# zengjianping/openpose

Measured on AMD Instinct MI355X. Metric: frames/sec whole-node, BODY_25 -1x368 @1280x720, 1/2/4/8 GPU + CPU ref, higher is better.
Workload: dtype fp16

## Files before the change

include/opk.h:

```cpp
#ifndef OPK_H
#define OPK_H

#include <stddef.h>
#include <stdint.h>

#ifdef __cplusplus
extern "C" {
#endif

#define OPK_OK 0
#define OPK_ERR_ARG 1
#define OPK_ERR_HIP 2
#define OPK_ERR_STATE 3
#define OPK_ERR_UNSUPPORTED 4

#define OPK_BODY_25 0
#define OPK_COCO_18 1
#define OPK_MPI_15 2
#define OPK_MPI_15_4 3
#define OPK_BODY_19 4
#define OPK_BODY_19_X2 5
#define OPK_BODY_19N 6
#define OPK_BODY_25E 7
#define OPK_CAR_12 8
#define OPK_BODY_25D 9
#define OPK_BODY_23 10
#define OPK_CAR_22 11
#define OPK_BODY_19E 12
#define OPK_BODY_25B 13
#define OPK_BODY_135 14

#define OPK_CONNECT_CPU 0
#define OPK_CONNECT_GPU 1

const char* opk_last_error(void);
int opk_version(void);

typedef struct opk_ctx opk_ctx;
int opk_ctx_create(int device, void* hip_stream ,
                   opk_ctx** out);
int opk_ctx_create_private_stream(int device, opk_ctx** out);
int opk_ctx_destroy(opk_ctx* ctx);
int opk_ctx_stream(opk_ctx* ctx, void** hip_stream);
int opk_sync(opk_ctx* ctx);
int opk_malloc(opk_ctx* ctx, void** dev, size_t bytes);
int opk_free(opk_ctx* ctx, void* dev);
int opk_memset(opk_ctx* ctx, void* dev, int value, size_t bytes);
int opk_memcpy_h2d(opk_ctx* ctx, void* dev_dst, const void* host_src, size_t bytes);
int opk_memcpy_d2h(opk_ctx* ctx, void* host_dst, const void* dev_src, size_t bytes);
#define OPK_F32 0
#define OPK_F64 1
#define OPK_U8 2
int opk_convert(opk_ctx* ctx, void* dst_dev, int dst_type, const void* src_dev, int src_type,
                size_t count);

int opk_resize_and_merge(opk_ctx* ctx, float* target_dev, const float* const* sources_dev,
                         int num_sources, const int target_size[4], const int* source_sizes,
                         const float* scale_ratios);

int opk_nms(opk_ctx* ctx, float* target_dev, int* kernel_scratch_dev, const float* source_dev,
            float threshold, const int target_size[4], const int source_size[4],
            float offset_x, float offset_y);

#define OPK_MAPS_CPU 0
#define OPK_MAPS_CUDA 1
int opk_resize_and_merge_semantics(opk_ctx* ctx, float* target_dev, const float* const* sources_dev,
                                   int num_sources, const int target_size[4],
                                   const int* source_sizes, const float* scale_ratios,
                                   int semantics);
int opk_nms_semantics(opk_ctx* ctx, float* target_dev, int* kernel_scratch_dev,
                      const float* source_dev, float threshold, const int target_size[4],
                      const int source_size[4], float offset_x, float offset_y, int semantics);

int opk_paf_scores(opk_ctx* ctx, float* pair_scores_dev, const float* heat_dev,
                   const float* peaks_dev, int num_frames, int pose_model, int heat_channels,
                   int heat_h, int heat_w, int max_peaks, float inter_threshold,
                   float inter_min_above_threshold, float default_nms_threshold);

int opk_connect_body_parts(opk_ctx* ctx, float* keypoints_host, float* scores_host,
                           int max_people, int* num_people, const float* heat_dev,
                           const float* peaks_dev, int pose_model, int heat_channels, int heat_h,
                           int heat_w, int max_peaks, float inter_min_above_threshold,
                           float inter_threshold, int min_subset_cnt, float min_subset_score,
                           float default_nms_threshold, float scale_factor,
                           int maximize_positives);

int opk_assemble_people(float* keypoints_host, float* scores_host, int max_people,
                        int* num_people, const float* pair_scores_host,
                        const float* peaks_host, int pose_model, int max_peaks,
                        int min_subset_cnt, float min_subset_score, float scale_factor,
                        int maximize_positives);

int opk_assemble_people_semantics(float* keypoints_host, float* scores_host, int max_people,
                                  int* num_people, const float* pair_scores_host,
                                  const float* peaks_host, int pose_model, int max_peaks,
                                  int min_subset_cnt, float min_subset_score, float scale_factor,
                                  int maximize_positives, int semantics);
int opk_connect_body_parts_semantics(opk_ctx* ctx, float* keypoints_host, float* scores_host,
                                     int max_people, int* num_people, const float* heat_dev,
                                     const float* peaks_dev, int pose_model, int heat_channels,
                                     int heat_h, int heat_w, int max_peaks,
                                     float inter_min_above_threshold, float inter_threshold,
                                     int min_subset_cnt, float min_subset_score,
                                     float default_nms_threshold, float scale_factor,
                                     int maximize_positives, int semantics);

int opk_scale_keypoints(float* keypoints_host, int people, int parts, int scale_mode,
                        double scale_input_to_output, double scale_net_to_output, int producer_w,
                        int producer_h);
int opk_keep_top_n_people(const float* keypoints_host, int people, int parts,
                          const float* scores_host, int max_people, float* out_keypoints_host,
                          int* out_index_host, int* out_people);

typedef struct opk_json_keypoints {
    const char* name;
    const float* data;
    int ndims, people, parts, dims;
} opk_json_keypoints;
int opk_people_json(const opk_json_keypoints* arrays, int n_arrays, const float* candidates_host,
                    const int* candidate_counts_host, int n_parts, int human_readable,
                    char* out_host, size_t capacity, size_t* len);
int opk_save_people_json(const char* path, const opk_json_keypoints* arrays, int n_arrays,
                         const float* candidates_host, const int* candidate_counts_host,
                         int n_parts, int human_readable);

int opk_pose_model_info(int pose_model, int* parts, int* bkg, int* npairs, int* heat_channels,
                        int* pairs, int* map_idx);
int opk_pose_default_thresholds(int pose_model, int maximize_positives, float* nms_threshold,
                                float* inter_threshold);

int opk_scale_and_size(int in_w, int in_h, int net_w, int net_h, float dynamic_behavior,
                       int scale_number, double scale_gap, double* scales, int* net_sizes);
int opk_cvmat_to_input(opk_ctx* ctx, float* input_dev, const uint8_t* frames_dev, int n, int width,
                       int height, size_t step, double scale, int net_w, int net_h, int normalize);

int opk_dev_set(const char* key, int value, int reset);

typedef struct opk_net opk_net;
int opk_net_create(opk_ctx* ctx, const char* prototxt, const char* caffemodel, opk_net** out);
int opk_net_load_caffemodel(opk_net* net, const char* caffemodel, int* convs_loaded);
int opk_caffemodel_blob(const char* caffemodel, const char* layer, int index, float* data,
                        size_t capacity, int64_t* shape, int* ndim);
int opk_net_destroy(opk_net* net);
int opk_net_num_convs(opk_net* net);
int opk_net_conv_info(opk_net* net, int index, char* name, int* cin, int* cout, int* kernel,
                      int* act);
int opk_net_set_conv(opk_net* net, const char* name, const float* weights_host,
                     const float* bias_host, const float* slope_host);
int opk_net_forward(opk_net* net, const float* input_dev, int n, int h, int w);
int opk_net_flops_per_frame(opk_net* net, int h, int w, double* flops);
#define OPK_PRECISION_FP16 0
#define OPK_PRECISION_SPLIT 1
int opk_net_set_precision(opk_net* net, int precision);
int opk_net_set_precision_schedule(opk_net* net, const int* precisions, int count);
int opk_net_conv_precision(opk_net* net, int index);
int opk_net_set_small_batch(opk_net* net, int enable);
int opk_net_small_batch(opk_net* net);
int opk_net_conv_plan(opk_net* net, int index, int n, int h, int w, int cus,
                      int* bm, int* bn, int* workgroups, int* small );
int opk_net_conv_kernels(opk_net* net, int index, int n, int h, int w, int cus,
                         char* buf, size_t size, size_t* needed);
int opk_net_set_timing(opk_net* net, int enable);
int opk_net_read_timing(opk_net* net, int* forwards, double* total_ms);
int opk_net_output(opk_net* net, float** output_dev, int shape[4]);
int opk_net_blob(opk_net* net, const char* name, int frame0, int nframes, float* host_out,
                 int shape[4]);
int opk_net_blob_planes(opk_net* net, const char* name, int frame0, int nframes, float* hi_host,
                        float* lo_host, int shape[4], int* has_lo);
int opk_net_launch_log(opk_net* net, char* buf, size_t size, size_t* needed);

typedef struct opk_pose opk_pose;
#define OPK_PROP_NMS_THRESHOLD 0
#define OPK_PROP_INTER_MIN_ABOVE_THRESHOLD 1
#define OPK_PROP_INTER_THRESHOLD 2
#define OPK_PROP_MIN_SUBSET_CNT 3
#define OPK_PROP_MIN_SUBSET_SCORE 4
int opk_pose_create(opk_ctx* ctx, opk_net* net ,
                    int maximize_positives, opk_pose** out);
int opk_pose_create_model(opk_ctx* ctx, opk_net* net, int pose_model, int maximize_positives,
                          int semantics, opk_pose** out);
int opk_pose_destroy(opk_pose* pose);
int opk_pose_set_property(opk_pose* pose, int property, double value);
int opk_pose_set_map_semantics(opk_pose* pose, int semantics);
int opk_pose_set_upsampling_ratio(opk_pose* pose, float ratio);
int opk_pose_forward(opk_pose* pose, const float* frames_dev, int n, int net_h, int net_w,
                     int producer_w, int producer_h);
int opk_pose_forward_net_output(opk_pose* pose, const float* net_output_dev, int n, int out_h,
                                int out_w, int net_h, int net_w, int producer_w, int producer_h);
int opk_pose_submit(opk_pose* pose, const float* frames_dev, int n, int net_h, int net_w,
                    int producer_w, int producer_h);
int opk_pose_submit_net_output(opk_pose* pose, const float* net_output_dev, int n, int out_h,
                               int out_w, int net_h, int net_w, int producer_w, int producer_h);
int opk_pose_collect(opk_pose* pose, int* frames);
int opk_pose_submit_multi(opk_pose* pose, const float* const* frames_dev, const int* net_hw,
                          int num_scales, int n, int producer_w, int producer_h);
int opk_pose_forward_multi(opk_pose* pose, const float* const* frames_dev, const int* net_hw,
                           int num_scales, int n, int producer_w, int producer_h);
int opk_pose_set_input(opk_pose* pose, int net_w, int net_h, float dynamic_behavior,
                       int scale_number, double scale_gap);
int opk_pose_submit_frames(opk_pose* pose, const uint8_t* frames_dev, int n, int width,
                           int height, size_t step);
int opk_pose_forward_frames(opk_pose* pose, const uint8_t* frames_dev, int n, int width,
                            int height, size_t step);
int opk_pose_net_input(opk_pose* pose, int scale, const float** input_dev, int* net_w,
                       int* net_h);
int opk_pose_pending(opk_pose* pose);
int opk_pose_set_overlay(opk_pose* pose, const float* overlay_dev);
int opk_pose_num_people(opk_pose* pose, int frame);
int opk_pose_keypoints(opk_pose* pose, int frame, float* keypoints_host, float* scores_host,
                       int max_people);
int opk_pose_set_timing(opk_pose* pose, int enable);
int opk_pose_read_timing(opk_pose* pose, int* batches, double* total_ms);
int opk_pose_read_collect_times(opk_pose* pose, int* collects, double* wait_ms, double* assembly_ms,
                                int* workers);
int opk_pose_records(opk_pose* pose, float* records_host, size_t capacity, size_t* used);
int opk_pose_heatmaps(opk_pose* pose, float** heat_dev, int shape[4]);
int opk_pose_heatmap_size(opk_pose* pose, int shape[4]);
int opk_pose_peaks(opk_pose* pose, float** peaks_dev, int shape[4]);
float opk_pose_scale_net_to_output(opk_pose* pose);
#define OPK_HEATMAP_PARTS 1
#define OPK_HEATMAP_BACKGROUND 2
#define OPK_HEATMAP_PAFS 4
int opk_pose_heatmaps_copy(opk_pose* pose, int types, int scale_mode, float* dst_dev,
                           int shape[4]);
int opk_pose_heatmaps_copy_range(opk_pose* pose, int types, int scale_mode, int frame0, int nframes,
                                 void* dst_dev, int dst_type, int shape[4]);
int opk_pose_candidates(opk_pose* pose, int frame, float* candidates_host, int* counts_host);


int opk_face_detect(int pose_model, const float* keypoints_host, int people, int parts,
                    float* rects_host);
int opk_hand_detect(int pose_model, const float* keypoints_host, int people, int parts,
                    float* rects_host);

typedef struct opk_extractor opk_extractor;
#define OPK_EXTRACT_FACE 0
#define OPK_EXTRACT_HAND 1
int opk_extractor_create(opk_ctx* ctx, opk_net* net, int kind, int net_w, int net_h,
                         opk_extractor** out);
int opk_extractor_destroy(opk_extractor* ex);
int opk_extractor_set_scales(opk_extractor* ex, int number, float range);
int opk_extractor_set_max_batch(opk_extractor* ex, int max_batch);
int opk_extractor_parts(opk_extractor* ex);
int opk_extractor_set_heatmaps(opk_extractor* ex, int scale_mode);
int opk_extractor_heatmaps(opk_extractor* ex, const float** heatmaps_dev, int shape[5]);
int opk_extractor_forward(opk_extractor* ex, const uint8_t* frames_dev, int nframes, int width,
                          int height, size_t step, const float* rects_host,
                          const int* frame_of_host, int people, float* keypoints_host);
int opk_extractor_crop_count(opk_extractor* ex);
int opk_extractor_crop(opk_extractor* ex, int i, double* matrix_host, const float** input_dev);

int opk_pose_attach_extractor(opk_pose* pose, opk_extractor* ex);
int opk_pose_detach_extractor(opk_pose* pose, int kind);
int opk_pose_part_rectangles(opk_pose* pose, int kind, int frame, float* rects_host);
int opk_pose_part_keypoints(opk_pose* pose, int kind, int frame, float* keypoints_host,
                            int max_people);
int opk_pose_read_part_times(opk_pose* pose, int kind, int* batches, int* crops, double* host_ms,
                             double* wait_ms);

int opk_probe_peaks(opk_ctx* ctx, double* mfma_random_tflops, double* mfma_zero_tflops,
                    double* hbm_read_gbs);

int opk_render_pose_keypoints(opk_ctx* ctx, float* frame_dev, int pose_model, int people,
                              unsigned width, unsigned height, const float* pose_dev,
                              float render_threshold, int googly_eyes, int blend_original,
                              float alpha);
int opk_render_face_keypoints(opk_ctx* ctx, float* frame_dev, unsigned width, unsigned height,
                              const float* face_dev, int people, float render_threshold,
                              float alpha);
int opk_render_hand_keypoints(opk_ctx* ctx, float* frame_dev, unsigned width, unsigned height,
                              const float* hands_dev, int hands, float render_threshold,
                              float alpha);
int opk_render_pose_heat_map(opk_ctx* ctx, float* frame_dev, unsigned width, unsigned height,
                             const float* heat_dev, int heat_w, int heat_h,
                             float scale_to_keep_ratio, unsigned part, float alpha);
int opk_render_pose_heat_maps(opk_ctx* ctx, float* frame_dev, int pose_model, unsigned width,
                              unsigned height, const float* heat_dev, int heat_w, int heat_h,
                              float scale_to_keep_ratio, float alpha);
int opk_render_pose_paf(opk_ctx* ctx, float* frame_dev, int pose_model, unsigned width,
                        unsigned height, const float* heat_dev, int heat_w, int heat_h,
                        float scale_to_keep_ratio, int part, float alpha);
int opk_render_pose_pafs(opk_ctx* ctx, float* frame_dev, int pose_model, unsigned width,
                         unsigned height, const float* heat_dev, int heat_w, int heat_h,
                         float scale_to_keep_ratio, float alpha);
int opk_render_pose_distance(opk_ctx* ctx, float* frame_dev, unsigned width, unsigned height,
                             const float* heat_dev, int heat_w, int heat_h,
                             float scale_to_keep_ratio, unsigned part, float alpha);

#define OPK_CAST_CPU 0
#define OPK_CAST_CUDA 1
int opk_cvmat_to_output(opk_ctx* ctx, float* output_dev, const uint8_t* frames_dev, int n,
                        int width, int height, size_t step, double scale, int out_w, int out_h);
int opk_output_to_cvmat(opk_ctx* ctx, uint8_t* dst_dev, size_t dst_step, const float* output_dev,
                        int n, int w, int h, int cast);

#define OPK_LAYER_POSE 0
#define OPK_LAYER_FACE 1
#define OPK_LAYER_HAND 2
typedef struct opk_render_layer {
    int kind;
    int pose_model;
    const float* keypoints_dev;
// ... 53 lines not shown
```

openpose_amd/_lib.py:

```python
import ctypes
import os

_HERE = os.path.dirname(os.path.abspath(__file__))
LIB_PATH = os.path.join(_HERE, "libopk_hip.so")
if os.environ.get("OPK_LIB_PATH"):
    LIB_PATH = os.environ["OPK_LIB_PATH"]

_c = ctypes
_p = _c.c_void_p
_i = _c.c_int
_f = _c.c_float
_d = _c.c_double
_ip = _c.POINTER(_c.c_int)
_fp = _c.POINTER(_c.c_float)

_SIGS = {
    "opk_last_error": (_c.c_char_p, []),
    "opk_version": (_i, []),
    "opk_dev_set": (_i, [_c.c_char_p, _i, _i]),
    "opk_ctx_create": (_i, [_i, _p, _c.POINTER(_p)]),
    "opk_ctx_create_private_stream": (_i, [_i, _c.POINTER(_p)]),
    "opk_ctx_destroy": (_i, [_p]),
    "opk_ctx_stream": (_i, [_p, _c.POINTER(_p)]),
    "opk_sync": (_i, [_p]),
    "opk_malloc": (_i, [_p, _c.POINTER(_p), _c.c_size_t]),
    "opk_free": (_i, [_p, _p]),
    "opk_memset": (_i, [_p, _p, _i, _c.c_size_t]),
    "opk_convert": (_i, [_p, _p, _i, _p, _i, _c.c_size_t]),
    "opk_memcpy_h2d": (_i, [_p, _p, _p, _c.c_size_t]),
    "opk_memcpy_d2h": (_i, [_p, _p, _p, _c.c_size_t]),
    "opk_probe_peaks": (_i, [_p, _c.POINTER(_d), _c.POINTER(_d), _c.POINTER(_d)]),
    "opk_render_pose_keypoints": (_i, [_p, _p, _i, _i, _c.c_uint, _c.c_uint, _p, _f, _i, _i, _f]),
    "opk_render_face_keypoints": (_i, [_p, _p, _c.c_uint, _c.c_uint, _p, _i, _f, _f]),
    "opk_render_hand_keypoints": (_i, [_p, _p, _c.c_uint, _c.c_uint, _p, _i, _f, _f]),
    "opk_render_pose_heat_map": (_i, [_p, _p, _c.c_uint, _c.c_uint, _p, _i, _i, _f, _c.c_uint, _f]),
    "opk_render_pose_heat_maps": (_i, [_p, _p, _i, _c.c_uint, _c.c_uint, _p, _i, _i, _f, _f]),
    "opk_render_pose_paf": (_i, [_p, _p, _i, _c.c_uint, _c.c_uint, _p, _i, _i, _f, _i, _f]),
    "opk_render_pose_pafs": (_i, [_p, _p, _i, _c.c_uint, _c.c_uint, _p, _i, _i, _f, _f]),
    "opk_render_pose_distance": (_i, [_p, _p, _c.c_uint, _c.c_uint, _p, _i, _i, _f, _c.c_uint, _f]),
    "opk_resize_and_merge": (_i, [_p, _p, _c.POINTER(_p), _i, _ip, _ip, _fp]),
    "opk_nms": (_i, [_p, _p, _p, _p, _f, _ip, _ip, _f, _f]),
    "opk_nms_semantics": (_i, [_p, _p, _p, _p, _f, _ip, _ip, _f, _f, _i]),
    "opk_pose_set_map_semantics": (_i, [_p, _i]),
    "opk_resize_and_merge_semantics": (_i, [_p, _p, _c.POINTER(_p), _i, _ip, _ip, _fp, _i]),
    "opk_paf_scores": (_i, [_p, _p, _p, _p, _i, _i, _i, _i, _i, _i, _f, _f, _f]),
    "opk_connect_body_parts": (_i, [_p, _p, _p, _i, _ip, _p, _p, _i, _i, _i, _i, _i, _f, _f, _i,
                                    _f, _f, _f, _i]),
    "opk_assemble_people": (_i, [_p, _p, _i, _ip, _p, _p, _i, _i, _i, _f, _f, _i]),
    "opk_connect_body_parts_semantics": (_i, [_p, _p, _p, _i, _ip, _p, _p, _i, _i, _i, _i, _i, _f,
                                              _f, _i, _f, _f, _f, _i, _i]),
    "opk_assemble_people_semantics": (_i, [_p, _p, _i, _ip, _p, _p, _i, _i, _i, _f, _f, _i, _i]),
    "opk_pose_model_info": (_i, [_i, _ip, _ip, _ip, _ip, _p, _p]),
    "opk_pose_default_thresholds": (_i, [_i, _i, _fp, _fp]),
    "opk_net_create": (_i, [_p, _c.c_char_p, _c.c_char_p, _c.POINTER(_p)]),
    "opk_net_destroy": (_i, [_p]),
    "opk_net_num_convs": (_i, [_p]),
    "opk_net_conv_info": (_i, [_p, _i, _c.c_char_p, _ip, _ip, _ip, _ip]),
    "opk_net_set_conv": (_i, [_p, _c.c_char_p, _p, _p, _p]),
    "opk_net_forward": (_i, [_p, _p, _i, _i, _i]),
    "opk_net_flops_per_frame": (_i, [_p, _i, _i, _c.POINTER(_d)]),
    "opk_net_output": (_i, [_p, _c.POINTER(_p), _ip]),
    "opk_net_blob": (_i, [_p, _c.c_char_p, _i, _i, _p, _ip]),
    "opk_net_launch_log": (_i, [_p, _c.c_char_p, _c.c_size_t, _c.POINTER(_c.c_size_t)]),
    "opk_pose_create": (_i, [_p, _p, _i, _c.POINTER(_p)]),
    "opk_pose_create_model": (_i, [_p, _p, _i, _i, _i, _c.POINTER(_p)]),
    "opk_pose_destroy": (_i, [_p]),
    "opk_pose_set_property": (_i, [_p, _i, _d]),
    "opk_pose_forward": (_i, [_p, _p, _i, _i, _i, _i, _i]),
    "opk_pose_forward_net_output": (_i, [_p, _p, _i, _i, _i, _i, _i, _i, _i]),
    "opk_pose_set_upsampling_ratio": (_i, [_p, _f]),
    "opk_pose_heatmap_size": (_i, [_p, _ip]),
    "opk_pose_set_overlay": (_i, [_p, _p]),
    "opk_pose_submit": (_i, [_p, _p, _i, _i, _i, _i, _i]),
    "opk_pose_submit_net_output": (_i, [_p, _p, _i, _i, _i, _i, _i, _i, _i]),
    "opk_pose_collect": (_i, [_p, _ip]),
    "opk_pose_submit_multi": (_i, [_p, _c.POINTER(_p), _ip, _i, _i, _i, _i]),
    "opk_pose_forward_multi": (_i, [_p, _c.POINTER(_p), _ip, _i, _i, _i, _i]),
    "opk_pose_pending": (_i, [_p]),
    "opk_pose_num_people": (_i, [_p, _i]),
    "opk_pose_keypoints": (_i, [_p, _i, _p, _p, _i]),
    "opk_pose_set_timing": (_i, [_p, _i]),
    "opk_pose_read_timing": (_i, [_p, _ip, _c.POINTER(_d)]),
    "opk_pose_read_collect_times": (_i, [_p, _ip, _c.POINTER(_d), _c.POINTER(_d), _ip]),
    "opk_net_set_precision": (_i, [_p, _i]),
    "opk_net_set_precision_schedule": (_i, [_p, _ip, _i]),
    "opk_net_conv_precision": (_i, [_p, _i]),
    "opk_net_blob_planes": (_i, [_p, _c.c_char_p, _i, _i, _p, _p, _ip, _ip]),
    "opk_net_set_small_batch": (_i, [_p, _i]),
    "opk_net_small_batch": (_i, [_p]),
    "opk_net_conv_plan": (_i, [_p, _i, _i, _i, _i, _i, _ip, _ip, _ip, _ip]),
    "opk_net_conv_kernels": (_i, [_p, _i, _i, _i, _i, _i, _c.c_char_p, _c.c_size_t, _c.POINTER(_c.c_size_t)]),
    "opk_pose_records":(_i, [_p, _p, _c.c_size_t, _c.POINTER(_c.c_size_t)]),
    "opk_pose_heatmaps": (_i, [_p, _c.POINTER(_p), _ip]),
    "opk_pose_peaks": (_i, [_p, _c.POINTER(_p), _ip]),
    "opk_pose_scale_net_to_output": (_f, [_p]),
    "opk_net_load_caffemodel": (_i, [_p, _c.c_char_p, _ip]),
    "opk_caffemodel_blob": (_i, [_c.c_char_p, _c.c_char_p, _i, _p, _c.c_size_t, _p, _ip]),
    "opk_net_set_timing": (_i, [_p, _i]),
    "opk_net_read_timing": (_i, [_p, _ip, _c.POINTER(_d)]),
    "opk_pose_heatmaps_copy": (_i, [_p, _i, _i, _p, _ip]),
    "opk_pose_heatmaps_copy_range": (_i, [_p, _i, _i, _i, _i, _p, _i, _ip]),
    "opk_pose_candidates": (_i, [_p, _i, _p, _ip]),
    "opk_scale_keypoints": (_i, [_p, _i, _i, _i, _d, _d, _i, _i]),
    "opk_keep_top_n_people": (_i, [_p, _i, _i, _p, _i, _p, _p, _ip]),
    "opk_people_json": (_i, [_p, _i, _p, _p, _i, _i, _p, ctypes.c_size_t, _p]),
    "opk_save_people_json": (_i, [ctypes.c_char_p, _p, _i, _p, _p, _i, _i]),
    "opk_face_detect": (_i, [_i, _p, _i, _i, _p]),
    "opk_hand_detect": (_i, [_i, _p, _i, _i, _p]),
    "opk_extractor_create": (_i, [_p, _p, _i, _i, _i, _c.POINTER(_p)]),
    "opk_extractor_destroy": (_i, [_p]),
    "opk_extractor_set_scales": (_i, [_p, _i, _f]),
    "opk_extractor_set_max_batch": (_i, [_p, _i]),
    "opk_extractor_set_heatmaps": (_i, [_p, _i]),
    "opk_extractor_heatmaps": (_i, [_p, _p, _ip]),
    "opk_extractor_parts": (_i, [_p]),
    "opk_extractor_forward": (_i, [_p, _p, _i, _i, _i, _c.c_size_t, _p, _p, _i, _p]),
    "opk_extractor_crop_count": (_i, [_p]),
    "opk_extractor_crop": (_i, [_p, _i, _p, _c.POINTER(_p)]),
    "opk_pose_attach_extractor": (_i, [_p, _p]),
    "opk_pose_detach_extractor": (_i, [_p, _i]),
    "opk_pose_part_rectangles": (_i, [_p, _i, _i, _p]),
    "opk_pose_part_keypoints": (_i, [_p, _i, _i, _p, _i]),
    "opk_pose_read_part_times": (_i, [_p, _i, _ip, _ip, _c.POINTER(_d), _c.POINTER(_d)]),
    "opk_pose_render_frames_parts": (_i, [_p, _p, _c.c_size_t, _i, _i, _p, _i, _i, _i, _c.c_size_t,
                                          _d, _f, _f, _i, _i, _i, _f, _f, _f, _f]),
    "opk_scale_and_size": (_i, [_i, _i, _i, _i, _f, _i, _d, _c.POINTER(_d), _ip]),
    "opk_cvmat_to_input": (_i, [_p, _p, _p, _i, _i, _i, _c.c_size_t, _d, _i, _i, _i]),
    "opk_pose_set_input": (_i, [_p, _i, _i, _f, _i, _d]),
    "opk_pose_submit_frames": (_i, [_p, _p, _i, _i, _i, _c.c_size_t]),
    "opk_pose_forward_frames": (_i, [_p, _p, _i, _i, _i, _c.c_size_t]),
    "opk_pose_net_input": (_i, [_p, _i, _c.POINTER(_p), _ip, _ip]),
    "opk_cvmat_to_output": (_i, [_p, _p, _p, _i, _i, _i, _c.c_size_t, _d, _i, _i]),
    "opk_output_to_cvmat": (_i, [_p, _p, _c.c_size_t, _p, _i, _i, _i, _i]),
    "opk_render_frames": (_i, [_p, _p, _c.c_size_t, _i, _i, _p, _i, _i, _i, _c.c_size_t, _d, _p, _i,
                               _i, _i]),
    "opk_pose_render_frames": (_i, [_p, _p, _c.c_size_t, _i, _i, _p, _i, _i, _i, _c.c_size_t, _d,
                                    _f, _f, _i, _i, _i]),
    "opk_render_frames_heat": (_i, [_p, _p, _c.c_size_t, _i, _i, _p, _i, _i, _i, _c.c_size_t, _d, _p,
                                    _i, _i, _i, _p]),
    "opk_render_element": (_i, [_i, _i, _ip, _ip]),
    "opk_pose_render_frames_element": (_i, [_p, _p, _c.c_size_t, _i, _i, _p, _i, _i, _i,
                                            _c.c_size_t, _d, _i, _f, _f, _f, _i, _i, _i]),
}


class RenderHeatStruct(ctypes.Structure):
    _fields_ = [("kind", _i), ("pose_model", _i), ("channel", _i), ("heat_dev", _p),
                ("channels", _i), ("heat_w", _i), ("heat_h", _i), ("scale_to_keep_ratio", _f),
                ("alpha", _f)]


class RenderLayerStruct(ctypes.Structure):
    _fields_ = [("kind", _i), ("pose_model", _i), ("keypoints_dev", _p), ("counts_host", _ip),
                ("render_threshold", _f), ("alpha", _f), ("googly_eyes", _i)]


_LIB = None


class OpkError(RuntimeError):
    pass


def load():
    global _LIB
    if _LIB is None:
        if not os.path.exists(LIB_PATH):
            raise OpkError("libopk_hip.so not built (run `python -m openpose_amd.build`); the "
                           "product has no fallback path")
        L = ctypes.CDLL(LIB_PATH)
        for name, (res, args) in _SIGS.items():
            fn = getattr(L, name, None)
            if fn is None:
                continue
            fn.restype = res
            fn.argtypes = args
        _LIB = L
    return _LIB


def exported_symbols():
    return list(_SIGS)


def check(rc):
    if rc != 0:
        raise OpkError("opk error %d: %s" % (rc, load().opk_last_error().decode()))
    return rc


def int4(v):
    return (ctypes.c_int * 4)(*[int(x) for x in v])
```

openpose_amd/api.py:

```python
import atexit
import ctypes
import weakref

import numpy as np
import torch

from . import _lib
from ._lib import OpkError, check, int4
from .pose_tables import (BODY_25, CONNECT_CPU, CONNECT_GPU, CONNECT_INTER_MIN_ABOVE_THRESHOLD,
                          CONNECT_INTER_THRESHOLD,
                          CONNECT_MIN_SUBSET_CNT, CONNECT_MIN_SUBSET_SCORE, NMS_THRESHOLD)

MAPS_CPU, MAPS_CUDA = 0, 1
PRECISION_FP16, PRECISION_SPLIT = 0, 1
CAST_CPU, CAST_CUDA = 0, 1
LAYER_POSE, LAYER_FACE, LAYER_HAND = 0, 1, 2
_LAYER_THRESHOLD = {LAYER_POSE: 0.05, LAYER_FACE: 0.4, LAYER_HAND: 0.2}


class RenderLayer:

    def __init__(self, kind, keypoints, counts, threshold=None, alpha=0.6, pose_model=BODY_25,
                 googly_eyes=False):
        self.kind, self.keypoints, self.counts = kind, keypoints, list(counts)
        self.threshold = _LAYER_THRESHOLD[kind] if threshold is None else threshold
        self.alpha, self.pose_model, self.googly_eyes = alpha, pose_model, googly_eyes


HEAT_NONE, HEAT_PART, HEAT_PARTS, HEAT_PAF, HEAT_PAFS, HEAT_DISTANCE = 0, 1, 2, 3, 4, 5


class RenderHeat:

    def __init__(self, kind, heat, scale, channel=0, alpha=0.7, pose_model=BODY_25):
        self.kind, self.heat, self.scale, self.channel = kind, heat, scale, channel
        self.alpha, self.pose_model = alpha, pose_model


def render_element(pose_model, element):
    kind, channel = ctypes.c_int(0), ctypes.c_int(0)
    check(_lib.load().opk_render_element(pose_model, element, ctypes.byref(kind),
                                         ctypes.byref(channel)))
    return kind.value, channel.value


def _row_bytes(t, n, h, w):
    assert t.dtype == torch.uint8 and t.is_contiguous() and t.shape[0] == n and t.shape[1] == h
    step = t.shape[2] * 3 if t.dim() == 4 else t.shape[2]
    assert (t.dim() == 3 or t.shape[3] == 3) and step >= w * 3
    return step


def _ptr(t):
    if t is None:
        return None
    assert t.is_cuda and t.is_contiguous(), "device tensors must be contiguous CUDA tensors"
    return ctypes.c_void_p(t.data_ptr())


_LIVE = {"pose": weakref.WeakSet(), "extractor": weakref.WeakSet(), "net": weakref.WeakSet(),
         "ctx": weakref.WeakSet()}


@atexit.register
def _close_live():
    for kind in ("pose", "extractor", "net", "ctx"):
        for obj in list(_LIVE[kind]):
            try:
                obj.close()
            except Exception:
                pass


class dev_switches:

    def __init__(self, **kv):
        self.kv = kv

    def __enter__(self):
        L = _lib.load()
        for k, v in self.kv.items():
            check(L.opk_dev_set(k.encode(), int(v), 0))
        return self

    def __exit__(self, *exc):
        L = _lib.load()
        for k in self.kv:
            L.opk_dev_set(k.encode(), 0, 1)
        return False


class Context:

    def __init__(self, device=0, stream=None):
        self.L = _lib.load()
        self.device = device
        torch.cuda.set_device(device)
        s = stream if stream is not None else torch.cuda.current_stream(device)
        self.torch_stream = s
        h = ctypes.c_void_p()
        check(self.L.opk_ctx_create(device, ctypes.c_void_p(s.cuda_stream), ctypes.byref(h)))
        self.h = h
        _LIVE["ctx"].add(self)

    def close(self):
        if self.h:
            self.L.opk_ctx_destroy(self.h)
            self.h = None

    def __del__(self):
        try:
            self.close()
        except Exception:
            pass

    def sync(self):
        check(self.L.opk_sync(self.h))

    @classmethod
    def host_only(cls):
        self = cls.__new__(cls)
        self.L = _lib.load()
        self.device = -1
        self.torch_stream = None
        h = ctypes.c_void_p()
        check(self.L.opk_ctx_create(-1, None, ctypes.byref(h)))
        self.h = h
        _LIVE["ctx"].add(self)
        return self

    def convert(self, dst, src):
        kinds = {torch.float32: 0, torch.float64: 1}
        assert dst.numel() == src.numel() and dst.dtype in kinds and src.dtype in kinds
        assert dst.is_contiguous() and src.is_contiguous()
        check(self.L.opk_convert(self.h, _ptr(dst), kinds[dst.dtype], _ptr(src), kinds[src.dtype],
                                 src.numel()))

    def resize_and_merge(self, target, sources, semantics=MAPS_CPU, scale_ratios=None):
        n = len(sources)
        ptrs = (ctypes.c_void_p * n)(*[s.data_ptr() for s in sources])
        sizes = (ctypes.c_int * (4 * n))(*[int(v) for s in sources for v in s.shape])
        ratios = None if scale_ratios is None else (ctypes.c_float * n)(*[float(r) for r in scale_ratios])
        check(self.L.opk_resize_and_merge_semantics(self.h, _ptr(target), ptrs, n,
                                                    int4(target.shape), sizes, ratios, semantics))

    def cvmat_to_input(self, net_input, frames, scale, normalize=1):
        n, h, w, c = frames.shape
        assert c == 3 and frames.dtype == torch.uint8
        assert net_input.shape[0] == n and net_input.shape[1] == 3
        check(self.L.opk_cvmat_to_input(self.h, _ptr(net_input), _ptr(frames), n, w, h, w * 3,
                                        float(scale), net_input.shape[3], net_input.shape[2],
                                        normalize))

    def nms(self, peaks, heat, threshold=NMS_THRESHOLD, offset=(0.0, 0.0), semantics=MAPS_CPU):
        check(self.L.opk_nms_semantics(self.h, _ptr(peaks), None, _ptr(heat), threshold,
                                       int4(peaks.shape), int4(heat.shape), offset[0], offset[1],
                                       semantics))

    def probe_peaks(self):
        r, z, h = ctypes.c_double(), ctypes.c_double(), ctypes.c_double()
        check(self.L.opk_probe_peaks(self.h, ctypes.byref(r), ctypes.byref(z), ctypes.byref(h)))
        return {"mfma_fp16_random_tflops": round(r.value, 1), "mfma_fp16_zero_tflops": round(z.value, 1),
                "hbm_read_gbs": round(h.value, 1)}

    def render_pose_keypoints(self, frame, pose, pose_model=BODY_25, threshold=0.05,
                              googly_eyes=False, blend_original=True, alpha=0.6):
        h, w = frame.shape[:2]
        people = 0 if pose is None else pose.shape[0]
        check(self.L.opk_render_pose_keypoints(self.h, _ptr(frame), pose_model, people, w, h,
                                               None if pose is None else _ptr(pose), threshold,
                                               int(googly_eyes), int(blend_original), alpha))

    def render_face_keypoints(self, frame, face, threshold=0.4, alpha=0.6):
        h, w = frame.shape[:2]
        check(self.L.opk_render_face_keypoints(self.h, _ptr(frame), w, h, _ptr(face), face.shape[0],
                                               threshold, alpha))

    def render_hand_keypoints(self, frame, hands, threshold=0.2, alpha=0.6):
        h, w = frame.shape[:2]
        check(self.L.opk_render_hand_keypoints(self.h, _ptr(frame), w, h, _ptr(hands),
                                               hands.shape[0], threshold, alpha))

    def render_heat_map(self, frame, heat, scale, part, alpha=0.7, distance=False):
        h, w = frame.shape[:2]
        fn = self.L.opk_render_pose_distance if distance else self.L.opk_render_pose_heat_map
        check(fn(self.h, _ptr(frame), w, h, _ptr(heat), heat.shape[-1], heat.shape[-2], scale,
                 part, alpha))

    def render_heat_maps(self, frame, heat, scale, pose_model=BODY_25, alpha=0.7):
        h, w = frame.shape[:2]
        check(self.L.opk_render_pose_heat_maps(self.h, _ptr(frame), pose_model, w, h, _ptr(heat),
                                               heat.shape[-1], heat.shape[-2], scale, alpha))

    def render_pafs(self, frame, heat, scale, part=None, pose_model=BODY_25, alpha=0.7):
        h, w = frame.shape[:2]
        if part is None:
            check(self.L.opk_render_pose_pafs(self.h, _ptr(frame), pose_model, w, h, _ptr(heat),
                                              heat.shape[-1], heat.shape[-2], scale, alpha))
        else:
            check(self.L.opk_render_pose_paf(self.h, _ptr(frame), pose_model, w, h, _ptr(heat),
                                             heat.shape[-1], heat.shape[-2], scale, part, alpha))

    def cvmat_to_output(self, frames, scale=1.0, out_size=None):
        n, h, w, c = frames.shape
        assert c == 3 and frames.dtype == torch.uint8
        ow, oh = out_size if out_size is not None else (w, h)
        out = torch.empty((n, max(oh, 0), max(ow, 0), 3), dtype=torch.float32, device=frames.device)
        check(self.L.opk_cvmat_to_output(self.h, _ptr(out), _ptr(frames), n, w, h, w * 3,
                                         float(scale), ow, oh))
        return out

    def output_to_cvmat(self, output, cast=CAST_CPU, out=None):
        n, h, w, c = output.shape
        assert c == 3 and output.dtype == torch.float32
        if out is None:
            out = torch.empty((n, h, w, 3), dtype=torch.uint8, device=output.device)
        check(self.L.opk_output_to_cvmat(self.h, _ptr(out), _row_bytes(out, n, h, w), _ptr(output),
                                         n, w, h, cast))
        return out

    def render_frames(self, frames, layers, scale=1.0, out_size=None, blend_original=True,
                      cast=CAST_CPU, out=None, heat=None):
        n, h, w, c = frames.shape
        assert c == 3 and frames.dtype == torch.uint8
        ow, oh = out_size if out_size is not None else (w, h)
        if out is None:
            out = torch.empty((n, max(oh, 0), max(ow, 0), 3), dtype=torch.uint8,
                              device=frames.device)
        arr = (_lib.RenderLayerStruct * max(len(layers), 1))()
        keep = []
        for s, l in zip(arr, layers):
            assert len(l.counts) == n, "one count per frame"
            counts = (ctypes.c_int * max(n, 1))(*[int(v) for v in l.counts])
            keep.append(counts)
            parts = {LAYER_FACE: 70, LAYER_HAND: 21}.get(l.kind)
            if parts is None and l.kind == LAYER_POSE and 0 <= l.pose_model <= 14:
                parts = pose_model_info(l.pose_model)["parts"]
            if l.keypoints is None:
                assert sum(l.counts) == 0, "keypoints missing"
            elif parts is not None:
                assert l.keypoints.dtype == torch.float32
                assert tuple(l.keypoints.shape) == (sum(l.counts), parts, 3), "keypoints shape"
            s.kind, s.pose_model = l.kind, l.pose_model
            s.keypoints_dev = None if l.keypoints is None else _ptr(l.keypoints)
            s.counts_host = counts
            s.render_threshold, s.alpha, s.googly_eyes = l.threshold, l.alpha, int(l.googly_eyes)
        if heat is None:
            check(self.L.opk_render_frames(self.h, _ptr(out), _row_bytes(out, n, oh, ow), ow, oh,
                                           _ptr(frames), n, w, h, w * 3, float(scale), arr,
                                           len(layers), int(blend_original), cast))
            return out
        hs = _lib.RenderHeatStruct()
        hs.kind, hs.pose_model, hs.channel = heat.kind, heat.pose_model, heat.channel
        if heat.heat is not None:
            assert heat.heat.dtype == torch.float32 and heat.heat.dim() == 4
            assert heat.heat.shape[0] == n, "one heat stack per frame"
            hs.heat_dev = _ptr(heat.heat)
            hs.channels, hs.heat_h, hs.heat_w = heat.heat.shape[1:]
        hs.scale_to_keep_ratio, hs.alpha = heat.scale, heat.alpha
        check(self.L.opk_render_frames_heat(self.h, _ptr(out), _row_bytes(out, n, oh, ow), ow, oh,
                                            _ptr(frames), n, w, h, w * 3, float(scale), arr,
                                            len(layers), int(blend_original), cast,
                                            ctypes.byref(hs)))
        return out

    def paf_scores(self, scores, heat, peaks, pose_model=BODY_25, inter_th=CONNECT_INTER_THRESHOLD,
                   inter_min_above=CONNECT_INTER_MIN_ABOVE_THRESHOLD, nms_th=NMS_THRESHOLD):
        n, c, h, w = heat.shape
        check(self.L.opk_paf_scores(self.h, _ptr(scores), _ptr(heat), _ptr(peaks), n, pose_model, c,
                                    h, w, peaks.shape[2] - 1, inter_th, inter_min_above, nms_th))

    def connect_body_parts(self, heat, peaks, pose_model=BODY_25, scale=1.0, max_people=512,
                           inter_min_above=CONNECT_INTER_MIN_ABOVE_THRESHOLD,
                           inter_th=CONNECT_INTER_THRESHOLD, min_subset_cnt=CONNECT_MIN_SUBSET_CNT,
                           min_subset_score=CONNECT_MIN_SUBSET_SCORE, nms_th=NMS_THRESHOLD,
                           maximize_positives=False, semantics=CONNECT_CPU):
        c, h, w = heat.shape[-3:]
        parts = peaks.shape[-3]
        kp = np.zeros((max_people, parts, 3), np.float32)
        ks = np.zeros(max_people, np.float32)
        n = ctypes.c_int()
        check(self.L.opk_connect_body_parts_semantics(
            self.h, kp.ctypes.data_as(ctypes.c_void_p), ks.ctypes.data_as(ctypes.c_void_p),
            max_people, ctypes.byref(n), _ptr(heat), _ptr(peaks), pose_model, c, h, w,
            peaks.shape[-2] - 1, inter_min_above, inter_th, min_subset_cnt, min_subset_score,
            nms_th, scale, int(maximize_positives), semantics))
        k = min(n.value, max_people)
        return kp[:k].copy(), ks[:k].copy()


def scale_and_size(input_size, net_resolution=(-1, 368), dynamic_behavior=1.0, scale_number=1,
                   scale_gap=0.25):
    L = _lib.load()
    scales = (ctypes.c_double * scale_number)()
    sizes = (ctypes.c_int * (2 * scale_number))()
    check(L.opk_scale_and_size(input_size[0], input_size[1], net_resolution[0], net_resolution[1],
                               float(dynamic_behavior), scale_number, float(scale_gap), scales,
                               sizes))
    return list(scales), [(sizes[2 * i], sizes[2 * i + 1]) for i in range(scale_number)]


def scale_keypoints(keypoints, scale_mode, scale_input_to_output=1.0, scale_net_to_output=1.0,
                    producer_size=(1, 1)):
    kp = np.ascontiguousarray(keypoints, np.float32).copy()
    check(_lib.load().opk_scale_keypoints(kp.ctypes.data_as(ctypes.c_void_p), kp.shape[0],
# ... 29 lines not shown
        a = np.ascontiguousarray(a if a is not None else np.zeros(0), np.float32)
        keep.append(a)
        shape = a.shape if a.size else ()
        if len(shape) not in (0, 1, 3):
            shape = (None,) * 2
        dims = list(shape) + [0] * (3 - len(shape))
        arr[i] = _JsonKeypoints(name.encode(), a.ctypes.data if a.size else None, len(shape),
                                dims[0] or 0, dims[1] or 0, dims[2] or 0)
    cands = candidates or []
    counts = np.array([len(c) for c in cands], np.int32)
    flat = np.ascontiguousarray(
        np.concatenate([np.asarray(c, np.float32).reshape(-1, 3) for c in cands])
        if cands and counts.sum() else np.zeros((0, 3)), np.float32)
    keep += [counts, flat]
    return arr, keep, (flat.ctypes.data if flat.size else None,
                       counts.ctypes.data if counts.size else None, len(cands))


def people_json(keypoint_vector, candidates=None, human_readable=False):
    L = _lib.load()
    arr, keep, (cp, cc, nparts) = _json_args(keypoint_vector, candidates)
    n = ctypes.c_size_t()
    check(L.opk_people_json(arr, len(keypoint_vector), cp, cc, nparts, int(human_readable), None,
                            0, ctypes.byref(n)))
    buf = ctypes.create_string_buffer(n.value + 1)
    check(L.opk_people_json(arr, len(keypoint_vector), cp, cc, nparts, int(human_readable), buf,
                            n.value + 1, ctypes.byref(n)))
    del keep
    return buf.raw[:n.value].decode()


def save_people_json(path, keypoint_vector, candidates=None, human_readable=False):
    L = _lib.load()
    arr, keep, (cp, cc, nparts) = _json_args(keypoint_vector, candidates)
    check(L.opk_save_people_json(path.encode(), arr, len(keypoint_vector), cp, cc, nparts,
                                 int(human_readable)))
    del keep


def datum_keypoint_vector(pose_keypoints, face_keypoints=None, hand_keypoints=(None, None)):
    pk = np.asarray(pose_keypoints, np.float32)
    ids = np.full(pk.shape[0], -1, np.float32) if pk.size else None
    return [(ids, "person_id"), (pk, "pose_keypoints_2d"), (face_keypoints, "face_keypoints_2d"),
            (hand_keypoints[0], "hand_left_keypoints_2d"),
            (hand_keypoints[1], "hand_right_keypoints_2d"), (None, "pose_keypoints_3d"),
            (None, "face_keypoints_3d"), (None, "hand_left_keypoints_3d"),
            (None, "hand_right_keypoints_3d")]


def caffemodel_blob(path, layer, index):
    L = _lib.load()
    shape = (ctypes.c_int64 * 8)()
    nd = ctypes.c_int()
    check(L.opk_caffemodel_blob(path.encode(), layer.encode(), index, None, 0, shape,
                                ctypes.byref(nd)))
    dims = tuple(shape[i] for i in range(nd.value))
    out = np.empty(int(np.prod(dims)) if dims else 0, np.float32)
    check(L.opk_caffemodel_blob(path.encode(), layer.encode(), index,
                                out.ctypes.data_as(ctypes.c_void_p), out.size, shape,
                                ctypes.byref(nd)))
    return dims, out.reshape(dims)


def pose_model_info(pose_model):
    L = _lib.load()
    parts, bkg, npairs, hc = (ctypes.c_int() for _ in range(4))
    check(L.opk_pose_model_info(pose_model, ctypes.byref(parts), ctypes.byref(bkg),
                                ctypes.byref(npairs), ctypes.byref(hc), None, None))
    pairs = np.zeros(2 * npairs.value, np.int32)
    nmap = hc.value - parts.value - bkg.value
    mi = np.zeros(max(nmap, 1), np.int32)
    check(L.opk_pose_model_info(pose_model, None, None, None, None,
                                pairs.ctypes.data_as(ctypes.c_void_p),
                                mi.ctypes.data_as(ctypes.c_void_p)))
    nms, inter = ctypes.c_float(), ctypes.c_float()
    check(L.opk_pose_default_thresholds(pose_model, 0, ctypes.byref(nms), ctypes.byref(inter)))
    return dict(id=pose_model, parts=parts.value, bkg=bool(bkg.value), pairs=pairs.tolist(),
                map_idx=mi[:nmap].tolist(), heat_channels=hc.value, nms_threshold=nms.value,
                inter_threshold=inter.value)


def assemble_people(pair_scores, peaks, pose_model=BODY_25, scale=1.0, max_people=512,
                    min_subset_cnt=CONNECT_MIN_SUBSET_CNT, min_subset_score=CONNECT_MIN_SUBSET_SCORE,
                    maximize_positives=False, semantics=CONNECT_CPU):
    L = _lib.load()
    pair_scores = np.ascontiguousarray(pair_scores, np.float32)
    peaks = np.ascontiguousarray(peaks, np.float32)
    parts = peaks.shape[0]
    kp = np.zeros((max_people, parts, 3), np.float32)
    ks = np.zeros(max_people, np.float32)
    n = ctypes.c_int()
    check(L.opk_assemble_people_semantics(kp.ctypes.data_as(ctypes.c_void_p),
                                          ks.ctypes.data_as(ctypes.c_void_p), max_people,
                                          ctypes.byref(n),
                                          pair_scores.ctypes.data_as(ctypes.c_void_p),
                                          peaks.ctypes.data_as(ctypes.c_void_p), pose_model,
                                          peaks.shape[1] - 1, min_subset_cnt, min_subset_score,
                                          scale, int(maximize_positives), semantics))
    k = min(n.value, max_people)
    return kp[:k].copy(), ks[:k].copy()


class Net:

    def __init__(self, ctx, prototxt="builtin:BODY_25", caffemodel=None):
        self.ctx = ctx
        self.L = ctx.L
        h = ctypes.c_void_p()
        check(self.L.opk_net_create(ctx.h, prototxt.encode(),
                                    caffemodel.encode() if caffemodel else None, ctypes.byref(h)))
        self.h = h
        _LIVE["net"].add(self)

    def close(self):
        if self.h:
            self.L.opk_net_destroy(self.h)
            self.h = None

    def __del__(self):
        try:
            self.close()
        except Exception:
            pass

    def convs(self):
        out = []
        name = ctypes.create_string_buffer(64)
        cin, cout, k, act = ctypes.c_int(), ctypes.c_int(), ctypes.c_int(), ctypes.c_int()
        for i in range(self.L.opk_net_num_convs(self.h)):
            check(self.L.opk_net_conv_info(self.h, i, name, ctypes.byref(cin), ctypes.byref(cout),
                                           ctypes.byref(k), ctypes.byref(act)))
            out.append(dict(name=name.value.decode(), cin=cin.value, num_output=cout.value,
                            kernel_size=k.value, act=act.value))
        return out

    def set_params(self, params):
        for c in self.convs():
            w, b, s = params[c["name"]]
            w = np.ascontiguousarray(w, np.float32)
            b = np.ascontiguousarray(b, np.float32)
            sp = None
            if s is not None:
                s = np.ascontiguousarray(s, np.float32)
                sp = s.ctypes.data_as(ctypes.c_void_p)
            check(self.L.opk_net_set_conv(self.h, c["name"].encode(),
                                          w.ctypes.data_as(ctypes.c_void_p),
                                          b.ctypes.data_as(ctypes.c_void_p), sp))

    def forward(self, x):
        n, c, h, w = x.shape
        check(self.L.opk_net_forward(self.h, _ptr(x), n, h, w))
        return self.output()

    def load_caffemodel(self, path):
        n = ctypes.c_int()
        check(self.L.opk_net_load_caffemodel(self.h, path.encode(), ctypes.byref(n)))
        return n.value

    def set_precision(self, precision):
        check(self.L.opk_net_set_precision(self.h, int(precision)))

    def set_precision_schedule(self, schedule):
        convs = self.convs()
        if callable(schedule):
            sched = [schedule(dict(c, index=i)) for i, c in enumerate(convs)]
        elif isinstance(schedule, dict):
            names = {c["name"] for c in convs}
            unknown = sorted(set(schedule) - names)
            if unknown:
                raise OpkError("precision schedule: no convolution named " + ", ".join(unknown))
            cur = self.precision_schedule()
            sched = [schedule.get(c["name"], cur[i]) for i, c in enumerate(convs)]
        else:
            sched = list(schedule)
        arr = (ctypes.c_int * max(1, len(sched)))(*[int(p) for p in sched])
        check(self.L.opk_net_set_precision_schedule(self.h, arr, len(sched)))

    def precision_schedule(self):
        return [self.L.opk_net_conv_precision(self.h, i)
                for i in range(self.L.opk_net_num_convs(self.h))]

    def set_small_batch(self, on=True):
        check(self.L.opk_net_set_small_batch(self.h, int(bool(on))))

    @property
    def small_batch(self):
        return self.L.opk_net_small_batch(self.h) == 1

    def conv_plan(self, index, n, h, w, cus):
        v = [ctypes.c_int() for _ in range(4)]
        check(self.L.opk_net_conv_plan(self.h, index, n, h, w, cus, *[ctypes.byref(x) for x in v]))
        return dict(bm=v[0].value, bn=v[1].value, workgroups=v[2].value, small=v[3].value)

    def conv_kernels(self, index, n, h, w, cus):
        need = ctypes.c_size_t()
        check(self.L.opk_net_conv_kernels(self.h, index, n, h, w, cus, None, 0, ctypes.byref(need)))
        buf = ctypes.create_string_buffer(need.value)
        check(self.L.opk_net_conv_kernels(self.h, index, n, h, w, cus, buf, need.value, ctypes.byref(need)))
        return buf.value.decode().splitlines()

    def set_timing(self, on=True):
        check(self.L.opk_net_set_timing(self.h, int(on)))

    def read_timing(self):
        n, ms = ctypes.c_int(), ctypes.c_double()
        check(self.L.opk_net_read_timing(self.h, ctypes.byref(n), ctypes.byref(ms)))
        return n.value, ms.value

    def flops_per_frame(self, h, w):
        f = ctypes.c_double()
        check(self.L.opk_net_flops_per_frame(self.h, h, w, ctypes.byref(f)))
        return f.value

    def output(self):
        p = ctypes.c_void_p()
        shape = (ctypes.c_int * 4)()
        check(self.L.opk_net_output(self.h, ctypes.byref(p), shape))
        return p.value, tuple(shape)

    def output_numpy(self):
        p, shape = self.output()
        out = np.empty(shape, np.float32)
        check(self.L.opk_memcpy_d2h(self.ctx.h, out.ctypes.data_as(ctypes.c_void_p),
                                    ctypes.c_void_p(p), out.nbytes))
        return out

    def blob(self, name, frames=None):
        shape = (ctypes.c_int * 4)()
        f0, nf = frames if frames is not None else (0, self.output()[1][0])
        check(self.L.opk_net_blob(self.h, name.encode(), f0, nf, None, shape))
        out = np.empty(tuple(shape), np.float32)
        check(self.L.opk_net_blob(self.h, name.encode(), f0, nf,
                                  out.ctypes.data_as(ctypes.c_void_p), shape))
        return out

    def blob_planes(self, name, frames=None):
        shape = (ctypes.c_int * 4)()
        has = ctypes.c_int()
        f0, nf = frames if frames is not None else (0, self.output()[1][0])
        check(self.L.opk_net_blob_planes(self.h, name.encode(), f0, nf, None, None, shape,
                                         ctypes.byref(has)))
        hi = np.empty(tuple(shape), np.float32)
        lo = np.empty(tuple(shape), np.float32)
        check(self.L.opk_net_blob_planes(self.h, name.encode(), f0, nf,
                                         hi.ctypes.data_as(ctypes.c_void_p),
                                         lo.ctypes.data_as(ctypes.c_void_p), shape, ctypes.byref(has)))
        return hi, lo, bool(has.value)

    def launch_log(self):
        need = ctypes.c_size_t()
        check(self.L.opk_net_launch_log(self.h, None, 0, ctypes.byref(need)))
        buf = ctypes.create_string_buffer(need.value)
        check(self.L.opk_net_launch_log(self.h, buf, need.value, ctypes.byref(need)))
        return [tuple(line.split("\t", 1)) for line in buf.value.decode().splitlines()]


class PoseExtractor:

    def __init__(self, ctx, net=None, maximize_positives=False, pose_model=BODY_25,
                 semantics=CONNECT_CPU):
        self.ctx = ctx
        self.L = ctx.L
        h = ctypes.c_void_p()
        check(self.L.opk_pose_create_model(ctx.h, net.h if net is not None else None, pose_model,
                                           int(maximize_positives), semantics, ctypes.byref(h)))
        self.h = h
        _LIVE["pose"].add(self)
        self.net = net
        self.parts = pose_model_info(pose_model)["parts"]
        self.pose_model = pose_model
        self._attached = {}

    def close(self):
        if self.h:
            self.L.opk_pose_destroy(self.h)
            self.h = None
            self._attached = {}

    def attach(self, face=None, hands=None):
        for ex, kind in ((face, FACE), (hands, HAND)):
            if ex is None:
                continue
            if ex.kind != kind:
                raise ValueError("face wants a FACE extractor, hands a HAND extractor")
            check(self.L.opk_pose_attach_extractor(self.h, ex.h))
            self._attached[kind] = ex

    def detach(self, kind):
        check(self.L.opk_pose_detach_extractor(self.h, kind))
        self._attached.pop(kind, None)

    def _part_rectangles(self, kind, frame):
        n = max(self.num_people(frame), 0)
        out = np.zeros((n, 2 if kind == HAND else 1, 4), np.float32)
        check(self.L.opk_pose_part_rectangles(self.h, kind, frame,
                                              out.ctypes.data_as(ctypes.c_void_p)))
        return out

    def _part_keypoints(self, kind, frame):
        n = max(self.num_people(frame), 0)
        parts = self._attached[kind].parts if kind in self._attached else (21 if kind == HAND else 70)
        out = np.zeros((2 if kind == HAND else 1, n, parts, 3), np.float32)
        check(self.L.opk_pose_part_keypoints(self.h, kind, frame,
                                             out.ctypes.data_as(ctypes.c_void_p), n))
        return out

# ... 352 lines not shown
```

openpose_amd/csrc/host/api_net.cpp:

```cpp
#include <cstring>
#include <memory>
#include <string>

#include "../../../include/opk.h"
#include "net.h"
#include "caffemodel.h"
#include "extract.h"
#include "input.h"
#include "pose.h"

namespace opk {
template <class F>
static int guarded_net(F&& f)
{
    try {
        f();
        return OPK_OK;
    } catch (const Error& e) {
        set_error(e.what());
        return e.code;
    } catch (const std::exception& e) {
        set_error(e.what());
        return OPK_ERR_STATE;
    }
}
}

struct opk_ctx : opk::Context {};
struct opk_net {
    opk_ctx* ctx;
    std::unique_ptr<opk::NetHip> net;
};
struct opk_pose {
    opk_ctx* ctx;
    std::unique_ptr<opk::PoseHip> pose;
};

using opk::guarded_net;

extern "C" {

int opk_net_create(opk_ctx* ctx, const char* prototxt, const char* caffemodel, opk_net** out)
{
    return guarded_net([&] {
        OPK_CHECK_ARG(ctx && prototxt && out, "NULL argument");
        const std::string p(prototxt);
        std::vector<opk::LayerDesc> layers =
            p.rfind("builtin:", 0) == 0 ? opk::builtin_graph(p) : opk::load_prototxt(p);
        auto n = std::make_unique<opk_net>(opk_net{ctx, std::make_unique<opk::NetHip>(ctx, std::move(layers))});
        if (caffemodel && caffemodel[0]) {
            OPK_CHECK_ARG(ctx->device >= 0, "weights need a device context");
            n->net->load_caffemodel(caffemodel);
        }
        *out = n.release();
    });
}

int opk_net_destroy(opk_net* net)
{
    return guarded_net([&] {
        if (!net) return;
        if (net->ctx->device >= 0) net->ctx->bind();
        delete net;
    });
}

int opk_net_num_convs(opk_net* net)
{
    if (!net) return -1;
    return (int)net->net->convs().size();
}

int opk_net_conv_info(opk_net* net, int i, char* name, int* cin, int* cout, int* k, int* act)
{
    return guarded_net([&] {
        OPK_CHECK_ARG(net && i >= 0 && i < (int)net->net->convs().size(), "bad index");
        const auto& c = net->net->convs()[i];
        if (name) {
            std::strncpy(name, c.name.c_str(), 63);
            name[63] = 0;
        }
        if (cin) *cin = c.cin;
        if (cout) *cout = c.cout;
        if (k) *k = c.k;
        if (act) *act = c.act;
    });
}

int opk_net_set_conv(opk_net* net, const char* name, const float* w, const float* b,
                     const float* slope)
{
    return guarded_net([&] {
        OPK_CHECK_ARG(net && name, "NULL argument");
        net->net->set_conv(name, w, b, slope);
    });
}

int opk_net_forward(opk_net* net, const float* input, int n, int h, int w)
{
    return guarded_net([&] {
        OPK_CHECK_ARG(net, "NULL net");
        net->net->forward(input, n, h, w);
    });
}

int opk_net_flops_per_frame(opk_net* net, int h, int w, double* flops)
{
    return guarded_net([&] {
        OPK_CHECK_ARG(net && flops && h > 0 && w > 0, "bad argument");
        *flops = net->net->flops_per_frame(h, w);
    });
}

int opk_net_output(opk_net* net, float** out, int shape[4])
{
    return guarded_net([&] {
        OPK_CHECK_ARG(net && out && shape, "NULL argument");
        *out = net->net->output();
        shape[0] = net->net->frames();
        shape[1] = net->net->out_channels();
        shape[2] = net->net->out_h();
        shape[3] = net->net->out_w();
    });
}

int opk_net_blob(opk_net* net, const char* name, int frame0, int nframes, float* host_out,
                 int shape[4])
{
    return guarded_net([&] {
        OPK_CHECK_ARG(net && name && shape, "NULL argument");
        net->net->blob(name, frame0, nframes, host_out, shape);
    });
}

int opk_net_blob_planes(opk_net* net, const char* name, int frame0, int nframes, float* hi_host,
                        float* lo_host, int shape[4], int* has_lo)
{
    return guarded_net([&] {
        OPK_CHECK_ARG(net && name && shape && has_lo, "NULL argument");
        net->net->blob_planes(name, frame0, nframes, hi_host, lo_host, shape, has_lo);
    });
}

int opk_net_launch_log(opk_net* net, char* buf, size_t size, size_t* needed)
{
    return guarded_net([&] {
        OPK_CHECK_ARG(net && needed, "NULL argument");
        std::string text;
        for (const auto& l : net->net->launches()) text += l + "\n";
        *needed = text.size() + 1;
        if (buf && size >= *needed) std::memcpy(buf, text.c_str(), text.size() + 1);
    });
}

int opk_pose_create(opk_ctx* ctx, opk_net* net, int maxpos, opk_pose** out)
{
    return guarded_net([&] {
        OPK_CHECK_ARG(ctx && out, "NULL argument");
        *out = new opk_pose{ctx, std::make_unique<opk::PoseHip>(ctx, net ? net->net.get() : nullptr,
                                                                maxpos != 0)};
    });
}

int opk_pose_create_model(opk_ctx* ctx, opk_net* net, int pose_model, int maxpos, int semantics,
                          opk_pose** out)
{
    return guarded_net([&] {
        OPK_CHECK_ARG(ctx && out, "NULL argument");
        *out = new opk_pose{ctx, std::make_unique<opk::PoseHip>(ctx, net ? net->net.get() : nullptr,
                                                                maxpos != 0, pose_model, semantics)};
    });
}

int opk_pose_destroy(opk_pose* p)
{
    return guarded_net([&] {
        if (!p) return;
        if (p->ctx->device >= 0) p->ctx->bind();
        delete p;
    });
}

int opk_pose_set_map_semantics(opk_pose* p, int semantics)
{
    return guarded_net([&] {
        OPK_CHECK_ARG(p, "NULL pose");
        p->pose->set_map_semantics(semantics);
    });
}

int opk_pose_set_property(opk_pose* p, int prop, double v)
{
    return guarded_net([&] {
        OPK_CHECK_ARG(p, "NULL pose");
        p->pose->set_property(prop, v);
    });
}

int opk_pose_forward(opk_pose* p, const float* frames, int n, int net_h, int net_w, int pw, int ph)
{
    return guarded_net([&] {
        OPK_CHECK_ARG(p, "NULL pose");
        p->pose->forward(frames, n, net_h, net_w, pw, ph);
    });
}

int opk_pose_forward_net_output(opk_pose* p, const float* out, int n, int oh, int ow, int net_h,
                                int net_w, int pw, int ph)
{
    return guarded_net([&] {
        OPK_CHECK_ARG(p, "NULL pose");
        p->pose->forward_net_output(out, n, oh, ow, net_h, net_w, pw, ph);
    });
}

int opk_pose_submit(opk_pose* p, const float* frames, int n, int net_h, int net_w, int pw, int ph)
{
    return guarded_net([&] {
        OPK_CHECK_ARG(p, "NULL pose");
        p->pose->submit(frames, n, net_h, net_w, pw, ph);
    });
}

int opk_pose_submit_multi(opk_pose* p, const float* const* frames, const int* net_hw, int nscales,
                          int n, int pw, int ph)
{
    return guarded_net([&] {
        OPK_CHECK_ARG(p, "NULL pose");
        p->pose->submit_multi(frames, net_hw, nscales, n, pw, ph);
    });
}

int opk_pose_forward_multi(opk_pose* p, const float* const* frames, const int* net_hw,
                           int nscales, int n, int pw, int ph)
{
    return guarded_net([&] {
        OPK_CHECK_ARG(p, "NULL pose");
        OPK_CHECK_ARG(p->pose->pending() == 0, "batches in flight: collect them first");
        p->pose->submit_multi(frames, net_hw, nscales, n, pw, ph);
        p->pose->collect();
    });
}

int opk_pose_submit_net_output(opk_pose* p, const float* out, int n, int oh, int ow, int net_h,
                               int net_w, int pw, int ph)
{
    return guarded_net([&] {
        OPK_CHECK_ARG(p, "NULL pose");
        p->pose->submit_net_output(out, n, oh, ow, net_h, net_w, pw, ph);
    });
}

int opk_pose_collect(opk_pose* p, int* frames)
{
    return guarded_net([&] {
        OPK_CHECK_ARG(p, "NULL pose");
// ... 89 lines not shown
    });
}

int opk_pose_heatmaps(opk_pose* p, float** heat, int shape[4])
{
    return guarded_net([&] {
        OPK_CHECK_ARG(p && heat && shape, "NULL argument");
        *heat = p->pose->heatmaps(shape);
    });
}

int opk_pose_heatmap_size(opk_pose* p, int shape[4])
{
    return guarded_net([&] {
        OPK_CHECK_ARG(p && shape, "NULL argument");
        p->pose->heatmap_size(shape);
    });
}

int opk_pose_peaks(opk_pose* p, float** peaks, int shape[4])
{
    return guarded_net([&] {
        OPK_CHECK_ARG(p && peaks && shape, "NULL argument");
        *peaks = p->pose->peaks(shape);
    });
}

int opk_net_load_caffemodel(opk_net* net, const char* caffemodel, int* loaded)
{
    return guarded_net([&] {
        OPK_CHECK_ARG(net && caffemodel, "NULL argument");
        OPK_CHECK_ARG(net->ctx->device >= 0, "weights need a device context");
        const int n = net->net->load_caffemodel(caffemodel);
        if (loaded) *loaded = n;
    });
}

int opk_caffemodel_blob(const char* caffemodel, const char* layer, int index, float* data,
                        size_t capacity, int64_t* shape, int* ndim)
{
    return guarded_net([&] {
        OPK_CHECK_ARG(caffemodel && layer && ndim, "NULL argument");
        const auto layers = opk::load_caffemodel(caffemodel);
        for (const auto& L : layers) {
            if (L.name != layer) continue;
            OPK_CHECK_ARG(index >= 0 && index < (int)L.blobs.size(), "no such blob");
            const auto& b = L.blobs[index];
            OPK_CHECK_ARG(b.shape.size() <= 8, "blob rank > 8");
            *ndim = (int)b.shape.size();
            if (shape) for (size_t i = 0; i < b.shape.size(); ++i) shape[i] = b.shape[i];
            if (data) {
                OPK_CHECK_ARG(capacity >= b.data.size(), "capacity too small");
                std::memcpy(data, b.data.data(), b.data.size() * sizeof(float));
            }
            return;
        }
        throw opk::Error(1, std::string("layer ") + layer + " has no blobs in " + caffemodel);
    });
}

int opk_net_set_precision(opk_net* net, int precision)
{
    return guarded_net([&] {
        OPK_CHECK_ARG(net, "NULL net");
        net->net->set_precision(precision);
    });
}

int opk_net_set_precision_schedule(opk_net* net, const int* precisions, int count)
{
    return guarded_net([&] {
        OPK_CHECK_ARG(net, "NULL net");
        net->net->set_precision_schedule(precisions, count);
    });
}

int opk_net_conv_precision(opk_net* net, int index)
{
    if (!net) return -1;
    return net->net->conv_precision(index);
}

int opk_net_set_small_batch(opk_net* net, int enable)
{
    return guarded_net([&] {
        OPK_CHECK_ARG(net, "NULL net");
        OPK_CHECK_ARG(enable == 0 || enable == 1, "small batch: 0 or 1");
        net->net->set_small_batch(enable == 1);
    });
}

int opk_net_small_batch(opk_net* net)
{
    if (!net) return -1;
    return net->net->small_batch() ? 1 : 0;
}

int opk_net_conv_plan(opk_net* net, int index, int n, int h, int w, int cus, int* bm, int* bn,
                      int* workgroups, int* small)
{
    return guarded_net([&] {
        OPK_CHECK_ARG(net, "NULL net");
        net->net->conv_plan(index, n, h, w, cus, bm, bn, workgroups, small);
    });
}

int opk_net_conv_kernels(opk_net* net, int index, int n, int h, int w, int cus, char* buf, size_t size,
                         size_t* needed)
{
    return guarded_net([&] {
        OPK_CHECK_ARG(net && needed, "NULL argument");
        std::string text;
        for (const auto& k : net->net->conv_kernels(index, n, h, w, cus)) text += k + "\n";
        *needed = text.size() + 1;
        if (buf && size >= *needed) std::memcpy(buf, text.c_str(), text.size() + 1);
    });
}

int opk_net_set_timing(opk_net* net, int enable)
{
    return guarded_net([&] {
        OPK_CHECK_ARG(net, "NULL net");
        net->net->set_timing(enable != 0);
    });
}

int opk_net_read_timing(opk_net* net, int* forwards, double* total_ms)
{
    return guarded_net([&] {
        OPK_CHECK_ARG(net, "NULL net");
        net->net->read_timing(forwards, total_ms);
    });
}

int opk_scale_and_size(int in_w, int in_h, int net_w, int net_h, float dynamic_behavior,
                       int scale_number, double scale_gap, double* scales, int* net_sizes)
{
    return guarded_net([&] {
        OPK_CHECK_ARG(scales && net_sizes, "NULL output");
        opk::scale_and_size(in_w, in_h, net_w, net_h, dynamic_behavior, scale_number, scale_gap,
                            scales, net_sizes);
    });
}

int opk_cvmat_to_input(opk_ctx* ctx, float* input_dev, const uint8_t* frames_dev, int n, int width,
                       int height, size_t step, double scale, int net_w, int net_h, int normalize)
{
    return guarded_net([&] {
        OPK_CHECK_ARG(ctx, "NULL context");
        OPK_CHECK_ARG(normalize == 0 || normalize == 1,
                      "normalize: 0 (none) or 1 (VGG); DenseNet (2) is not supported");
        opk::cvmat_to_input(ctx, input_dev, frames_dev, n, width, height, step, scale, net_w, net_h,
                            normalize);
    });
}

int opk_pose_set_input(opk_pose* p, int net_w, int net_h, float dynamic_behavior, int scale_number,
                       double scale_gap)
{
    return guarded_net([&] {
        OPK_CHECK_ARG(p, "NULL pose");
        p->pose->set_input(net_w, net_h, dynamic_behavior, scale_number, scale_gap);
    });
}

int opk_pose_submit_frames(opk_pose* p, const uint8_t* frames, int n, int width, int height,
                           size_t step)
{
    return guarded_net([&] {
        OPK_CHECK_ARG(p, "NULL pose");
        p->pose->submit_frames(frames, n, width, height, step);
    });
}

int opk_pose_forward_frames(opk_pose* p, const uint8_t* frames, int n, int width, int height,
                            size_t step)
{
    return guarded_net([&] {
        OPK_CHECK_ARG(p, "NULL pose");
        p->pose->forward_frames(frames, n, width, height, step);
    });
}

int opk_pose_render_frames(opk_pose* p, uint8_t* dst, size_t dst_step, int out_w, int out_h,
                           const uint8_t* frames, int n, int width, int height, size_t step,
                           double scale, float threshold, float alpha, int googly_eyes,
                           int blend_original, int cast)
{
    return guarded_net([&] {
        OPK_CHECK_ARG(p, "NULL pose");
        std::vector<int> counts;
        opk_render_layer layer{};
        const opk::PoseHip& pose = *p->pose;
        if (pose.frames() == 0) throw opk::Error(OPK_ERR_STATE, "no collected batch to render");
        if (n != pose.frames())
            throw opk::Error(OPK_ERR_STATE, "the collected batch has " +
                                                std::to_string(pose.frames()) + " frames, not " +
                                                std::to_string(n));
        const int parts = opk::pose_model(pose.model()).parts;
        std::vector<float> kp;
        for (int f = 0; f < n; ++f) {
            const int people = pose.num_people(f);
            counts.push_back(people);
            const auto& k = pose.keypoints(f);
            kp.insert(kp.end(), k.begin(), k.begin() + (size_t)people * parts * 3);
        }
        const float s = (float)scale;
        if (s != 1.f)
            for (size_t i = 0; i < kp.size(); i += 3) {
                kp[i] *= s;
                kp[i + 1] *= s;
            }
        layer.kind = OPK_LAYER_POSE;
        layer.pose_model = pose.model();
        layer.counts_host = counts.data();
        layer.render_threshold = threshold;
        layer.alpha = alpha;
        layer.googly_eyes = googly_eyes;
        opk::render_frames(p->ctx, dst, dst_step, out_w, out_h, frames, n, width, height, step,
                           scale, &layer, 1, blend_original, cast, kp.data(), kp.size());
    });
}

int opk_pose_render_frames_element(opk_pose* p, uint8_t* dst, size_t dst_step, int out_w,
                                   int out_h, const uint8_t* frames, int n, int width, int height,
                                   size_t step, double scale, int element, float threshold,
                                   float alpha_keypoint, float alpha_heatmap, int googly_eyes,
                                   int blend_original, int cast)
{
    if (element == 0)
        return opk_pose_render_frames(p, dst, dst_step, out_w, out_h, frames, n, width, height,
                                      step, scale, threshold, alpha_keypoint, googly_eyes,
                                      blend_original, cast);
    return guarded_net([&] {
        OPK_CHECK_ARG(p, "NULL pose");
        const opk::PoseHip& pose = *p->pose;
        opk_render_heat heat{};
        heat.pose_model = pose.model();
        opk::render_element(pose.model(), element, &heat.kind, &heat.channel);
        if (pose.frames() == 0) throw opk::Error(OPK_ERR_STATE, "no collected batch to render");
        if (n != pose.frames())
            throw opk::Error(OPK_ERR_STATE, "the collected batch has " +
                                                std::to_string(pose.frames()) + " frames, not " +
                                                std::to_string(n));
        const opk::HeatMap& lazy = pose.lazy_heat();
        heat.scale_to_keep_ratio = pose.scale_net_to_output() * (float)scale;
        heat.alpha = blend_original ? alpha_heatmap : 1.f;
        opk::render_frames(p->ctx, dst, dst_step, out_w, out_h, frames, n, width, height, step,
                           scale, nullptr, 0, 1, cast, nullptr, 0, &heat, &lazy);
    });
}

int opk_pose_net_input(opk_pose* p, int scale, const float** input_dev, int* net_w, int* net_h)
{
    return guarded_net([&] {
        OPK_CHECK_ARG(p && input_dev, "NULL argument");
        *input_dev = p->pose->net_input(scale, net_w, net_h);
    });
}

int opk_pose_heatmaps_copy(opk_pose* p, int types, int scale_mode, float* dst_dev, int shape[4])
{
    return guarded_net([&] {
        OPK_CHECK_ARG(p && shape, "NULL argument");
        p->pose->heatmaps_copy(types, scale_mode, dst_dev, shape);
    });
}

int opk_pose_heatmaps_copy_range(opk_pose* p, int types, int scale_mode, int frame0, int nframes,
                                 void* dst_dev, int dst_type, int shape[4])
{
    return guarded_net([&] {
        OPK_CHECK_ARG(p && shape, "NULL argument");
        p->pose->heatmaps_copy_range(types, scale_mode, frame0, nframes, dst_dev, dst_type, shape);
    });
}

int opk_pose_candidates(opk_pose* p, int frame, float* candidates_host, int* counts_host)
{
    return guarded_net([&] {
        OPK_CHECK_ARG(p, "NULL pose");
        p->pose->candidates(frame, candidates_host, counts_host);
    });
}

float opk_pose_scale_net_to_output(opk_pose* p) { return p ? p->pose->scale_net_to_output() : 0.f; }

}

struct opk_extractor {
    opk_ctx* ctx;
    std::unique_ptr<opk::KeypointExtractor> ex;
};

extern "C" {

int opk_face_detect(int pose_model, const float* keypoints, int people, int parts, float* rects)
{
    return guarded_net([&] {
        OPK_CHECK_ARG(people == 0 || rects, "NULL rectangles");
        opk::detect_faces(pose_model, keypoints, people, parts, reinterpret_cast<opk::Rect*>(rects));
    });
}

int opk_hand_detect(int pose_model, const float* keypoints, int people, int parts, float* rects)
{
// ... 212 lines not shown
```

openpose_amd/csrc/host/input.cpp:

```cpp
#include "input.h"

#include <cmath>
#include <cstring>
#include <vector>

#include "../common.h"
#include "../kernels/kernels.h"
#include "context.h"

namespace opk {

namespace {
constexpr int kInterBits = 5, kInterTab = 1 << kInterBits;
constexpr int kAbBits = 10, kAbScale = 1 << kAbBits;
constexpr int kCoefScale = 1 << 15;

int round_half_even(double v) { return (int)std::lrint(v); }
int round_half_even(float v) { return (int)std::lrintf(v); }

int positive_round(float v) { return (int)(v + 0.5f); }
int positive_round(double v) { return (int)(v + 0.5f); }
}

void scale_and_size(int in_w, int in_h, int net_w, int net_h, float dyn, int scale_number,
                    double scale_gap, double* scales, int* sizes)
{
    OPK_CHECK_ARG(in_w > 0 && in_h > 0, "Wrong input element (empty cvInputData).");
    OPK_CHECK_ARG(scale_number >= 1, "scale_number must be >= 1");
    if (net_w <= 0 || net_h <= 0) {
        OPK_CHECK_ARG(net_w > 0 || net_h > 0,
                      "Only 1 of the dimensions of net input resolution can be <= 0.");
        if (dyn > 0) {
            if (net_w <= 0)
                net_w = 16 * positive_round(1 / 16.f * std::min(net_h * dyn * 16.f / 9.f,
                                                                 net_h * in_w / (float)in_h));
            else
                net_h = 16 * positive_round(1 / 16.f * std::min(net_w * dyn * 9.f / 16.f,
                                                                 net_w * in_h / (float)in_w));
        } else {
            if (net_w <= 0)
                net_w = 16 * positive_round(1 / 16.f * net_h * in_w / (float)in_h);
            else
                net_h = 16 * positive_round(1 / 16.f * net_w * in_h / (float)in_w);
        }
    }
    for (int i = 0; i < scale_number; ++i) {
        const double cur = 1. - i * scale_gap;
        OPK_CHECK_ARG(cur >= 0. && cur <= 1.,
                      "All scales must be in the range [0, 1], i.e., 0 <= 1-scale_number*scale_gap <= 1");
        const int tw = std::min(net_w, std::max(1, positive_round(net_w * cur) / 16 * 16));
        const int th = std::min(net_h, std::max(1, positive_round(net_h * cur) / 16 * 16));
        const double rw = (tw - 1) / (double)(in_w - 1), rh = (th - 1) / (double)(in_h - 1);
        scales[i] = rw < rh ? rw : rh;
        sizes[2 * i] = tw;
        sizes[2 * i + 1] = th;
    }
}

void warp_weight_table(bool cubic, short* itab )
{
    const int k = cubic ? 4 : 2;
    float t1[kInterTab * 4];
    for (int i = 0; i < kInterTab; ++i) {
        const float x = i * (1.f / kInterTab);
        float* c = t1 + i * k;
        if (cubic) {
            const float A = -0.75f;
            c[0] = ((A * (x + 1) - 5 * A) * (x + 1) + 8 * A) * (x + 1) - 4 * A;
            c[1] = ((A + 2) * x - (A + 3)) * x * x + 1;
            c[2] = ((A + 2) * (1 - x) - (A + 3)) * (1 - x) * (1 - x) + 1;
            c[3] = 1.f - c[0] - c[1] - c[2];
        } else {
            c[0] = 1.f - x;
            c[1] = x;
        }
    }
    for (int i = 0; i < kInterTab; ++i)
        for (int j = 0; j < kInterTab; ++j) {
            short* w = itab + (i * kInterTab + j) * k * k;
            int isum = 0;
            for (int a = 0; a < k; ++a)
                for (int b = 0; b < k; ++b) {
                    const float v = t1[i * k + a] * t1[j * k + b];
                    const int r = round_half_even(v * kCoefScale);
                    w[a * k + b] = (short)std::min(32767, std::max(-32768, r));
                    isum += w[a * k + b];
                }
            if (isum == kCoefScale) continue;
            const int diff = isum - kCoefScale, h = k / 2;
            int lo = h * k + h, hi = h * k + h;
            for (int a = h; a < h + 2; ++a)
                for (int b = h; b < h + 2; ++b) {
                    const int e = a * k + b;
                    if (w[e] < w[lo]) lo = e;
                    else if (w[e] > w[hi]) hi = e;
                }
            if (diff < 0) w[hi] = (short)(w[hi] - diff);
            else w[lo] = (short)(w[lo] - diff);
        }
}

void warp_axis_table(double scale, int d, bool cubic, int* tab)
{
    double D = scale * scale;
    D = D != 0 ? 1. / D : 0;
    const double m = scale * D;
    const int x0 = round_half_even(0.0 * kAbScale) + kAbScale / kInterTab / 2;
    for (int x = 0; x < d; ++x) {
        const int X = (x0 + round_half_even(m * x * kAbScale)) >> (kAbBits - kInterBits);
        tab[2 * x] = (X >> kInterBits) - (cubic ? 1 : 0);
        tab[2 * x + 1] = X & (kInterTab - 1);
    }
}

const short* Context::warp_weight_table(bool cubic)
{
    DevBuf& b = warp_weights[cubic ? 1 : 0];
    if (!b.ptr) {
        const int k = cubic ? 4 : 2;
        std::vector<short> host((size_t)(kInterTab * kInterTab + 1) * k * k);
        opk::warp_weight_table(cubic, host.data());
        const size_t bytes = (size_t)kInterTab * kInterTab * k * k * sizeof(short);
        b.get(bytes);
        OPK_HIP(hipMemcpyAsync(b.ptr, host.data(), bytes,
                               hipMemcpyHostToDevice, stream));
        OPK_HIP(hipStreamSynchronize(stream));
    }
    return static_cast<const short*>(b.ptr);
}

const Context::WarpAxes& Context::warp_axis_tables(double scale, int dw, int dh)
{
    uint64_t bits;
    std::memcpy(&bits, &scale, sizeof bits);
    const auto key = std::make_tuple(bits, dw, dh);
    auto it = warp_axes.find(key);
    if (it != warp_axes.end()) return *it->second;
    const bool cubic = scale > 1.;
    std::vector<int> host(2 * (size_t)(dw + dh));
    warp_axis_table(scale, dw, cubic, host.data());
    warp_axis_table(scale, dh, cubic, host.data() + 2 * dw);
    auto t = std::make_unique<WarpAxes>();
    int* dev = static_cast<int*>(t->buf.get(host.size() * sizeof(int)));
    OPK_HIP(hipMemcpyAsync(dev, host.data(), host.size() * sizeof(int), hipMemcpyHostToDevice,
                           stream));
    OPK_HIP(hipStreamSynchronize(stream));
    t->x = dev;
    t->y = dev + 2 * dw;
    auto& ref = *t;
    warp_axes.emplace(key, std::move(t));
    return ref;
}

void cvmat_to_input(Context* ctx, float* dst, const uint8_t* src, int n, int sw, int sh,
                    size_t step, double scale, int dw, int dh, int normalize, hipStream_t stream)
{
    OPK_CHECK_ARG(dst && src, "NULL buffer");
    OPK_CHECK_ARG(n > 0 && sw > 0 && sh > 0 && dw > 0 && dh > 0, "empty frame or net input");
    OPK_CHECK_ARG(scale > 0 && std::isfinite(scale), "scale must be positive");
    ctx->bind();
    const bool cubic = scale > 1.;
    const short* w = ctx->warp_weight_table(cubic);
    const auto& ax = ctx->warp_axis_tables(scale, dw, dh);
    launch_cvmat_to_input(dst, src, n, sh, sw, step ? step : (size_t)sw * 3, dh, dw, ax.x, ax.y, w,
                          cubic ? 4 : 2, normalize, stream ? stream : ctx->stream);
}

}
```

openpose_amd/csrc/host/input.h:

```cpp
#pragma once
#include <hip/hip_runtime.h>
#include <cstddef>
#include <cstdint>

namespace opk {

struct Context;

void scale_and_size(int in_w, int in_h, int net_w, int net_h, float dyn, int scale_number,
                    double scale_gap, double* scales, int* sizes);

void warp_weight_table(bool cubic, short* itab);
void warp_axis_table(double scale, int d, bool cubic, int* tab );

void cvmat_to_input(Context* ctx, float* dst, const uint8_t* src, int n, int sw, int sh,
                    size_t step, double scale, int dw, int dh, int normalize, hipStream_t stream = nullptr);

}
```

openpose_amd/csrc/host/net.cpp:

```cpp
#include "net.h"

#include "caffemodel.h"

#include <algorithm>
#include <cmath>
#include <cstdlib>
#include <set>

namespace opk {

namespace {
int round_up(int v, int m) { return (v + m - 1) / m * m; }
int pick_bn(int cout)
{
    if (cout <= 32) return 32;
    if (cout <= 64) return 64;
    if (cout <= 96) return 96;
    return 128;
}
}

NetHip::NetHip(Context* ctx, std::vector<LayerDesc> layers, const std::string& output_blob)
    : ctx_(ctx), output_blob_(output_blob)
{
// ... 597 lines not shown
    S.h = h;
    S.w = w;
    const std::vector<int>& lh_ = S.lh;
    const std::vector<int>& lw_ = S.lw;
    std::vector<uint16_t*>& ptr = S.base;
    ptr.assign(bufs_.size(), nullptr);
    S.base_lo.assign(bufs_.size(), nullptr);
    for (size_t i = 0; i < bufs_.size(); ++i) {
        S.mem.push_back(std::make_unique<DevBuf>());
        S.mem_lo.push_back(std::make_unique<DevBuf>());
        if ((int)i == image_buf_) continue;
        bool head_buf = false;
        for (size_t hi = 0; hi < heads_.size(); ++hi)
            head_buf = head_buf || (S.headfused[hi] && heads_[hi].buf == (int)i);
        if (head_buf) continue;
        if (S.fused1 && ((int)i == fuse1_.abuf || (int)i == fuse1_.bbuf))
            continue;
        bool pooled_away = false;
        for (size_t q = 0; q < pools_.size(); ++q)
            pooled_away = pooled_away || (S.poolfused[q] && pools_[q].in_buf == (int)i);
        if (pooled_away) continue;
        const int L = bufs_[i].level, B = border_;
        const size_t head = (size_t)B * (lw_[L] + 2 * B) + B + 64;
        const size_t pos = head + (size_t)n * (lh_[L] + 2 * B) * (lw_[L] + 2 * B) + kConvGuardTail;
        const size_t bytes = pos * bufs_[i].cs * 2;
        OPK_CHECK_ARG(pos * bufs_[i].cs < (size_t)1 << 31, "activation buffer exceeds 2^31 elements");
        uint16_t* raw = static_cast<uint16_t*>(S.mem.back()->get(bytes));
        OPK_HIP(hipMemsetAsync(raw, 0, bytes, zero_stream ? zero_stream : ctx_->stream));
        ptr[i] = raw + head * bufs_[i].cs;
        if (S.twin[i]) {
            uint16_t* rl = static_cast<uint16_t*>(S.mem_lo.back()->get(bytes));
            OPK_HIP(hipMemsetAsync(rl, 0, bytes, zero_stream ? zero_stream : ctx_->stream));
            S.base_lo[i] = rl + head * bufs_[i].cs;
        }
    }
    const size_t out_bytes = (size_t)n * out_c_ * lh_[out_level_] * lw_[out_level_] * 4;
    S.out32 = static_cast<float*>(S.out_mem.get(out_bytes));
    void* sink = sink_.get(kConv3SinkBytes);
    S.args.assign(convs_.size(), ConvArgs{});
    S.use3.assign(convs_.size(), 0);
    for (size_t ci = 0; ci < convs_.size(); ++ci) {
        const ConvPlan& c = convs_[ci];
        ConvArgs& a = S.args[ci];
        const int H = lh_[c.level], W = lw_[c.level], Wp = W + 2 * border_;
        a.in = ptr[c.in.buf];
        a.in_cs = bufs_[c.in.buf].cs;
        a.in_coff = c.in.coff;
        a.cin_pad = c.cin_pad;
        a.ntaps = c.ntaps;
        if (a.ntaps == 9)
            for (int t = 0; t < 9; ++t) a.tapoff[t] = (t / 3) * Wp + (t % 3);
        else if (a.ntaps == 1)
            a.tapoff[0] = Wp + 1;
        a.border = border_;
        a.ksteps = c.ksteps;
        const bool use3 = !c.from_image;
        S.use3[ci] = use3;
        OPK_CHECK_ARG(use3 || c.w.ptr != nullptr, c.info.name + ": weights not set");
        if (use3) {
            a.sw = S.conv[ci].sw;
            a.nstrips = S.conv[ci].nstrips;
            a.small = S.conv[ci].family == Conv3Family::conv3s;
            a.sink = sink;
            a.cus = cus;
        }
        a.w = static_cast<const uint16_t*>(use3 ? c.w3.ptr : c.w.ptr);
        a.bias = static_cast<const float*>(c.bias.ptr);
        a.slope = static_cast<const float*>(c.slope.ptr);
        a.act = c.info.act;
        a.actmax = dev_switch("EPI_MAX", 1) != 0;
        a.frames = n;
        a.H = H;
        a.W = W;
        a.M = n * H * Wp;
        a.cout = c.info.cout;
        a.ndst = (int)c.outs.size();
        for (size_t d = 0; d < c.outs.size(); ++d) {
            a.dst[d] = ptr[c.outs[d].buf];
            a.dst_cs[d] = bufs_[c.outs[d].buf].cs;
            a.dst_coff[d] = c.outs[d].coff;
            a.dst_lo[d] = S.csplit[ci] ? S.base_lo[c.outs[d].buf] : nullptr;
        }
        a.split = S.csplit[ci] ? 1 : 0;
        a.wscale = S.csplit[ci] ? c.wscale : 1.f;
        a.in_lo = S.csplit[ci] && use3 && !S.query[ci].xhi ? S.base_lo[c.in.buf] : nullptr;
        for (size_t q = 0; q < pools_.size(); ++q)
            if (S.poolfused[q] && pool_conv_[q] == (int)ci) {
                a.pool = 1;
                a.ndst = 1;
                a.dst[0] = ptr[pools_[q].out_buf];
                a.dst_lo[0] = S.csplit[ci] ? S.base_lo[pools_[q].out_buf] : nullptr;
                a.dst_cs[0] = bufs_[pools_[q].out_buf].cs;
                a.dst_coff[0] = 0;
            }
        if (c.out32_coff >= 0) {
            OPK_CHECK_ARG(c.level == out_level_, c.info.name + ": output at another resolution");
            a.out32 = S.out32;
            a.out32_c = out_c_;
            a.out32_coff = c.out32_coff;
        }
    }
    return &S;
}

void NetHip::forward(const float* input, int n, int h, int w)
{
    forward_on(input, n, h, w, ctx_->stream, true);
}

float* NetHip::select_output(int n, int h, int w, bool alternate)
{
    OPK_CHECK_ARG(n > 0 && h > 0 && w > 0, "empty input");
    ctx_->bind();
    ShapePlan& S = *shape_plan(n, h, w, ctx_->stream);
    if (alternate) {
        if (!S.out32_alt) {
            const size_t bytes = (size_t)n * out_c_ * S.lh[out_level_] * S.lw[out_level_] * 4;
            S.out32_alt = static_cast<float*>(S.out_mem_alt.get(bytes));
        }
        S.alt = !S.alt;
    }
    return S.out();
}

void NetHip::note_reader(const float* out, hipEvent_t ev)
{
    for (auto& r : readers_)
        if (r.first == out) {
            r.second = ev;
            return;
        }
    readers_.emplace_back(out, ev);
}

void NetHip::forget_reader_events(const hipEvent_t* evs, int n)
{
    for (size_t i = readers_.size(); i-- > 0;)
        for (int k = 0; k < n; ++k)
            if (readers_[i].second == evs[k]) {
                readers_.erase(readers_.begin() + (long)i);
                break;
            }
}

void NetHip::prepare(int n, int h, int w)
{
    OPK_CHECK_ARG(n > 0 && h > 0 && w > 0, "empty input");
    ctx_->bind();
    (void)shape_plan(n, h, w, ctx_->stream);
}

void NetHip::forward_on(const float* input, int n, int h, int w, hipStream_t st, bool timed)
{
    OPK_CHECK_ARG(input && n > 0 && h > 0 && w > 0, "empty input");
    OPK_CHECK_ARG(ready(), "weights not loaded for every convolution");
    ctx_->bind();
    ShapePlan& S = *shape_plan(n, h, w, st);
    cur_ = &S;
    for (const auto& r : readers_)
        if (r.first == S.out()) OPK_HIP(hipStreamWaitEvent(st, r.second, 0));
    if (timed) timer_.begin(st);
    forward_launches(S, input, n, h, w, st);
    if (timed) timer_.end(st);
}

void NetHip::blob(const std::string& name, int f0, int nf, float* host, int shape[4]) const
{
    read_planes(name, f0, nf, nullptr, nullptr, host, shape, nullptr);
}

void NetHip::blob_planes(const std::string& name, int f0, int nf, float* hi, float* lo, int shape[4],
                         int* has_lo) const
{
    read_planes(name, f0, nf, hi, lo, nullptr, shape, has_lo);
}

void NetHip::read_planes(const std::string& name, int f0, int nf, float* hi, float* lo, float* sum,
                         int shape[4], int* has_lo) const
{
    OPK_CHECK_ARG(cur_ != nullptr, "no forward yet");
    const auto it = blob_loc_.find(name);
    OPK_CHECK_ARG(it != blob_loc_.end(), "no blob named " + name);
    const BlobLoc& L = it->second;
    const ShapePlan& S = *cur_;
    OPK_CHECK_ARG(f0 >= 0 && nf > 0 && f0 + nf <= S.n, "frames out of range");
    const int H = S.lh[L.level], W = S.lw[L.level];
    if (shape) {
        shape[0] = nf; shape[1] = L.ch; shape[2] = H; shape[3] = W;
    }
    const bool twin = !L.out32 && S.base_lo[L.buf] != nullptr;
    if (has_lo) *has_lo = twin ? 1 : 0;
    if (!hi && !lo && !sum) return;
    ctx_->bind();
    OPK_HIP(hipStreamSynchronize(ctx_->stream));
    const size_t hw = (size_t)H * W;
    if (L.out32) {
        OPK_CHECK_ARG(L.level == out_level_, name + ": not at the output resolution");
        for (float* host : {hi, sum})
            for (int f = 0; f < nf && host; ++f)
                OPK_HIP(hipMemcpy(host + (size_t)f * L.ch * hw,
                                  S.out() + ((size_t)(f0 + f) * out_c_ + L.coff) * hw,
                                  (size_t)L.ch * hw * 4, hipMemcpyDeviceToHost));
        if (lo) std::fill(lo, lo + (size_t)nf * L.ch * hw, 0.f);
        return;
    }
    OPK_CHECK_ARG(S.base[L.buf] != nullptr,
                  name + ": kept on chip by a fused kernel (not materialised at this shape)");
    const int B = border_, Wp = W + 2 * B, Hp = H + 2 * B, cs = bufs_[L.buf].cs;
    const size_t frame_elems = (size_t)Hp * Wp * cs;
    std::vector<uint16_t> raw(frame_elems * nf), rlo(twin ? frame_elems * nf : 0);
    OPK_HIP(hipMemcpy(raw.data(), S.base[L.buf] + (size_t)f0 * frame_elems, raw.size() * 2,
                      hipMemcpyDeviceToHost));
    if (twin)
        OPK_HIP(hipMemcpy(rlo.data(), S.base_lo[L.buf] + (size_t)f0 * frame_elems, rlo.size() * 2,
                          hipMemcpyDeviceToHost));
    for (int f = 0; f < nf; ++f)
        for (int y = 0; y < H; ++y)
            for (int x = 0; x < W; ++x) {
                const size_t at = f * frame_elems + ((size_t)(y + B) * Wp + x + B) * cs + L.coff;
                const uint16_t* src = raw.data() + at;
                for (int c = 0; c < L.ch; ++c) {
                    const size_t o = ((size_t)f * L.ch + c) * hw + (size_t)y * W + x;
                    const float vh = (float)__builtin_bit_cast(_Float16, src[c]);
                    const float vl = twin ? (float)__builtin_bit_cast(_Float16, rlo[at + c]) : 0.f;
                    if (hi) hi[o] = vh;
                    if (lo) lo[o] = vl;
                    if (sum) sum[o] = vh + vl;
                }
            }
}

void NetHip::forward_launches(ShapePlan& S, const float* input, int n, int h, int w, hipStream_t st)
{
    const bool logging = dev_switch("LAUNCH_LOG", 0) != 0;
    if (logging) {
        log_.lines.clear();
        attach_launch_log(&log_);
    }
    struct Detach {
        bool on;
        ~Detach() { if (on) attach_launch_log(nullptr); }
    } detach{logging};
    forward_steps(S, input, n, h, w, st);
}

static void launch_conv3_frames(const ConvArgs& a, hipStream_t st)
{
    const int B = a.border > 0 ? a.border : 1;
    Conv3Query q = conv3_query(a);
    const int run = conv3_run_frames(q);
    if (run == a.frames) {
        launch_conv3(a, st);
        return;
    }
    const size_t frame_pos = (size_t)(a.H + 2 * B) * (a.W + 2 * B);
    const size_t dst_pos = a.pool ? (size_t)(a.H / 2 + 2 * B) * (a.W / 2 + 2 * B) : frame_pos;
    for (int f0 = 0; f0 < a.frames; f0 += run) {
        ConvArgs b = a;
        b.frames = std::min(run, a.frames - f0);
        q.frames = b.frames;
        const Conv3Plan pb = conv3_plan(q);
        b.sw = pb.sw;
        b.nstrips = pb.nstrips;
        b.M = b.frames * a.H * (a.W + 2 * B);
        b.in = a.in + f0 * frame_pos * a.in_cs;
        if (a.in_lo) b.in_lo = a.in_lo + f0 * frame_pos * a.in_cs;
        for (int d = 0; d < a.ndst; ++d) {
            b.dst[d] = a.dst[d] + f0 * dst_pos * a.dst_cs[d];
            if (a.dst_lo[d]) b.dst_lo[d] = a.dst_lo[d] + f0 * dst_pos * a.dst_cs[d];
        }
        if (a.out32) b.out32 = a.out32 + (size_t)f0 * a.out32_c * a.H * a.W;
        launch_conv3(b, st);
    }
}

void NetHip::forward_steps(ShapePlan& S, const float* input, int n, int h, int w, hipStream_t st)
{
    LaunchLog* log = launch_log();
    float* const out32 = S.out();
    const std::vector<uint16_t*>& ptr = S.base;
    const std::vector<int>& lh_ = S.lh;
    const std::vector<int>& lw_ = S.lw;
    size_t first = 0;
    if (S.fused1) {
        const ConvPlan& a = convs_[fuse1_.a];
        const ConvPlan& b = convs_[fuse1_.b];
        const PoolPlan& p = pools_[fuse1_.p];
        Conv1FusedArgs fa{};
        fa.img = input;
        fa.frames = n;
        fa.H = h;
        fa.W = w;
        fa.w1 = static_cast<const uint16_t*>(a.w.ptr);
        fa.b1 = static_cast<const float*>(a.bias.ptr);
        fa.s1 = static_cast<const float*>(a.slope.ptr);
        fa.act1 = a.info.act;
        fa.w2 = static_cast<const uint16_t*>(b.w3.ptr);
        fa.b2 = static_cast<const float*>(b.bias.ptr);
        fa.s2 = static_cast<const float*>(b.slope.ptr);
        fa.act2 = b.info.act;
        fa.out = ptr[p.out_buf];
        fa.out_cs = bufs_[p.out_buf].cs;
        fa.out_coff = 0;
        fa.OH = lh_[1];
        fa.OW = lw_[1];
        fa.actmax = a.slope01 && b.slope01 && dev_switch("EPI_MAX", 1) != 0;
        if (log) log->layer = a.info.name + "+" + b.info.name + "+pool";
        launch_conv1_fused(fa, std::min(cus_, std::max(1, dev_switch("GRID_CUS", cus_))), st);
        first = 3;
    }
    for (size_t si = first; si < steps_.size(); ++si) {
        const Step& s = steps_[si];
        if (s.conv) {
            const ConvPlan& c = convs_[s.idx];
            const ConvArgs& a = S.args[s.idx];
            if (c.head >= 0 && S.headfused[c.head] && heads_[c.head].step == (int)si) {
                const FuseHead& fh = heads_[c.head];
                const ConvPlan& cb = convs_[fh.b];
                const ConvArgs& b = S.args[fh.b];
                HeadArgs h{};
                h.in = a.in;
                h.in_cs = a.in_cs;
                h.in_coff = a.in_coff;
                h.cin_pad = a.cin_pad;
                h.w6 = static_cast<const uint16_t*>(c.wh.ptr);
                h.b6 = a.bias;
                h.s6 = a.slope;
                h.act6 = a.act;
                h.actmax = a.actmax && c.slope01;
                h.w7 = static_cast<const uint16_t*>(cb.wh.ptr);
                h.b7 = b.bias;
                h.n1 = c.info.cout;
                h.n2 = cb.info.cout;
                h.frames = n;
                h.H = a.H;
                h.W = a.W;
                h.ndst = b.ndst;
                for (int d = 0; d < b.ndst; ++d) {
                    h.dst[d] = b.dst[d];
                    h.dst_cs[d] = b.dst_cs[d];
                    h.dst_coff[d] = b.dst_coff[d];
                }
                h.out32 = b.out32 ? out32 : nullptr;
                h.out32_c = b.out32_c;
                h.out32_coff = b.out32_coff;
                h.cus = dev_switch("HEAD_PERSIST", 1) != 0 ? a.cus : 0;
                if (S.csplit[s.idx]) {
                    h.split = 1;
                    h.in_lo = a.in_lo;
                    for (int d = 0; d < b.ndst; ++d) h.dst_lo[d] = b.dst_lo[d];
                    h.wscale6 = a.wscale;
                    h.wscale7 = b.wscale;
                }
                if (log) log->layer = c.info.name + "+" + cb.info.name;
                launch_conv_head(h, st);
                ++si;
                continue;
            }
            if (log) log->layer = c.info.name + (a.pool ? "+pool" : "");
            if (c.from_image) {
                ConvArgs ai = a;
                if (ai.out32) ai.out32 = out32;
                launch_conv_image(ai, input, st);
            } else {
                ConvArgs a3 = a;
                a3.actmax = a.actmax && c.slope01;
                if (a3.out32) a3.out32 = out32;
                launch_conv3_frames(a3, st);
            }
        } else {
            if (S.poolfused[s.idx]) continue;
            const PoolPlan& p = pools_[s.idx];
            const int L = p.level_in;
            if (log) log->layer = "pool";
            if (S.twin[p.in_buf])
                launch_maxpool2_split(ptr[p.out_buf], S.base_lo[p.out_buf], ptr[p.in_buf],
                                      S.base_lo[p.in_buf], n, lh_[L], lw_[L], bufs_[p.in_buf].cs,
                                      lh_[L + 1], lw_[L + 1], st, border_);
            else
                launch_maxpool2(ptr[p.out_buf], ptr[p.in_buf], n, lh_[L], lw_[L],
                                bufs_[p.in_buf].cs, lh_[L + 1], lw_[L + 1], st, border_);
        }
    }
}

int NetHip::load_caffemodel(const std::string& path)
{
    const std::vector<CaffeLayer> layers = opk::load_caffemodel(path);
    std::map<std::string, const CaffeLayer*> by_name;
    for (const auto& L : layers) by_name[L.name] = &L;
    int loaded = 0;
    for (const ConvInfo& c : info_) {
        auto it = by_name.find(c.name);
        if (it == by_name.end()) continue;
        const auto& blobs = it->second->blobs;
        OPK_CHECK_ARG(blobs.size() == 2, c.name + ": expected weights and bias blobs, got " +
                                             std::to_string(blobs.size()));
        const std::vector<int64_t> wshape{c.cout, c.cin, c.k, c.k}, bshape{c.cout};
        OPK_CHECK_ARG(blob_shape_is(blobs[0], wshape), "Cannot copy param 0 weights from layer '" +
                                                           c.name + "'; shape mismatch.");
        OPK_CHECK_ARG(blob_shape_is(blobs[1], bshape), "Cannot copy param 1 weights from layer '" +
                                                           c.name + "'; shape mismatch.");
        const float* slope = nullptr;
        if (c.act == 2) {
            auto pt = by_name.find(c.act_layer);
            OPK_CHECK_ARG(pt != by_name.end() && pt->second->blobs.size() == 1 &&
                              blob_shape_is(pt->second->blobs[0], bshape),
                          c.act_layer + ": PReLU slopes missing or of the wrong shape");
            slope = pt->second->blobs[0].data.data();
        }
        set_conv(c.name, blobs[0].data.data(), blobs[1].data.data(), slope);
        ++loaded;
    }
    return loaded;
}

NetHip::~NetHip() = default;

void NetHip::set_timing(bool on)
{
    timer_.on = on;
}

void NetHip::read_timing(int* count, double* total_ms)
{
    timer_.read(count, total_ms);
}

}
```

openpose_amd/csrc/host/net.h:

```cpp
#pragma once
#include <map>
#include <memory>
#include <string>
#include <vector>

#include "../kernels/conv.h"
#include "context.h"
#include "graph.h"

namespace opk {

class NetHip {
public:
    NetHip(Context* ctx, std::vector<LayerDesc> layers, const std::string& output_blob = "net_output");

    struct ConvInfo {
        std::string name;
        int cin, cout, k, act;
        std::string act_layer;
    };
    const std::vector<ConvInfo>& convs() const { return info_; }
    void set_conv(const std::string& name, const float* w, const float* b, const float* slope);
    static constexpr int kPrecisionFp16 = 0, kPrecisionSplit = 1;
    void set_precision(int precision);
    void set_precision_schedule(const int* precisions, int count);
    int conv_precision(int index) const;
    void set_small_batch(bool on);
    bool small_batch() const { return small_batch_; }
    void conv_plan(int index, int n, int h, int w, int cus, int* bm, int* bn, int* workgroups,
                   int* small) const;
    std::vector<std::string> conv_kernels(int index, int n, int h, int w, int cus) const;
    bool ready() const;
    int load_caffemodel(const std::string& path);

    void forward(const float* input, int n, int h, int w);
    void forward_on(const float* input, int n, int h, int w, hipStream_t stream, bool timed);
    void prepare(int n, int h, int w);
    void time_begin(hipStream_t s) { timer_.begin(s); }
    void time_end(hipStream_t s) { timer_.end(s); }
    float* output() const { return cur_ ? cur_->out() : nullptr; }
    float* select_output(int n, int h, int w, bool alternate);
    std::weak_ptr<void> liveness() const { return alive_; }
    void note_reader(const float* out, hipEvent_t ev);
    void forget_reader_events(const hipEvent_t* evs, int n);
    int out_channels() const { return out_c_; }
    int out_h() const { return cur_ ? cur_->lh[out_level_] : 0; }
    int out_w() const { return cur_ ? cur_->lw[out_level_] : 0; }
    int frames() const { return cur_ ? cur_->n : 0; }
    static constexpr int kMaxShapes = 8;
    double flops_per_frame(int h, int w) const;
    int border() const { return border_; }
    ~NetHip();

    void set_timing(bool on);
    void read_timing(int* count, double* total_ms);

    void blob(const std::string& name, int f0, int nf, float* host, int shape[4]) const;
    void blob_planes(const std::string& name, int f0, int nf, float* hi, float* lo, int shape[4],
                     int* has_lo) const;
    const std::vector<std::string>& launches() const { return log_.lines; }

private:
    struct Placement { int buf; int coff; };
    struct BufSpec { int level; int cs; };
    struct ConvPlan {
        ConvInfo info;
        std::string in_blob;
        int level = 0;
        bool from_image = false;
        Placement in{};
        int cin_pad = 0, ntaps = 9, ksteps = 0, bn = 128, cout_pad = 0;
        std::vector<Placement> outs;
        int out32_coff = -1;
        DevBuf w, bias, slope;
        DevBuf w3;
        DevBuf wh;
        int head = -1;
        bool loaded = false;
        bool slope01 = true;
        float wscale = 1.f;
        int precision = kPrecisionFp16;
        std::vector<float> hw, hb, hs;
    };
    bool fused1_at(int h, int w) const;
    void read_planes(const std::string& name, int f0, int nf, float* hi, float* lo, float* sum,
                     int shape[4], int* has_lo) const;
    void pack(ConvPlan& c);
    struct PoolPlan { int in_buf, out_buf, level_in, channels; };
    struct Step { bool conv; int idx; };

    struct Dispatch {
        std::vector<int> lh, lw;
        std::vector<char> csplit;
        std::vector<char> twin;
        bool fused1 = false;
        std::vector<char> headfused;
        std::vector<char> poolfused;
        std::vector<Conv3Query> query;
        std::vector<Conv3Plan> conv;
    };
    Dispatch dispatch(int n, int h, int w, int cus) const;

    struct ShapePlan : Dispatch {
        int n = 0, h = 0, w = 0;
        std::vector<std::unique_ptr<DevBuf>> mem;
        std::vector<uint16_t*> base;
        std::vector<std::unique_ptr<DevBuf>> mem_lo;
        std::vector<uint16_t*> base_lo;
        DevBuf out_mem, out_mem_alt;
        float* out32 = nullptr;
        float* out32_alt = nullptr;
        bool alt = false;
        float* out() const { return alt ? out32_alt : out32; }
        std::vector<ConvArgs> args;
        std::vector<char> use3;
    };

    void plan(const std::vector<LayerDesc>& layers);
    void forward_launches(ShapePlan& S, const float* input, int n, int h, int w, hipStream_t st);
    void forward_steps(ShapePlan& S, const float* input, int n, int h, int w, hipStream_t st);
    ShapePlan* shape_plan(int n, int h, int w, hipStream_t zero_stream = nullptr);

    Context* ctx_;
    std::string output_blob_;
    std::vector<ConvInfo> info_;
    std::vector<ConvPlan> convs_;
    std::map<std::string, int> conv_by_name_;
    std::vector<PoolPlan> pools_;
    std::vector<Step> steps_;
    std::vector<BufSpec> bufs_;
    int out_level_ = 0, out_c_ = 0, nlevels_ = 1;
    int image_buf_ = -1;
    struct Fuse1 { int a = -1, b = -1, p = -1, abuf = -1, bbuf = -1; };
    Fuse1 fuse1_;
    struct FuseHead { int a = -1, b = -1, step = -1, buf = -1; };
    std::vector<FuseHead> heads_;
    std::vector<int> pool_conv_;
    int cus_ = 256;
    bool small_batch_ = false;
    int border_ = 1;

    struct BlobLoc { int buf = -1, coff = 0, ch = 0, level = 0; bool out32 = false; };
    std::map<std::string, BlobLoc> blob_loc_;
    LaunchLog log_;

    std::vector<std::unique_ptr<ShapePlan>> shapes_;
    ShapePlan* cur_ = nullptr;
    std::vector<std::pair<const float*, hipEvent_t>> readers_;
    std::shared_ptr<int> alive_ = std::make_shared<int>(0);
    DevBuf sink_;
    EventTimer timer_;
};

}
```

openpose_amd/csrc/host/pose.cpp:

```cpp
#include "pose.h"

#include <sched.h>

#include <algorithm>
#include <chrono>
#include <cmath>
#include <cstring>
#include <exception>
#include <string>
#include <thread>

#include "../../../include/opk.h"
#include "input.h"
#include "maps.h"

namespace opk {

double resize_scale_factor(int iw, int ih, int tw, int th)
{
    const double rw = (tw - 1) / (double)(iw - 1);
    const double rh = (th - 1) / (double)(ih - 1);
    return rw < rh ? rw : rh;
}

// ... 181 lines not shown
{
    OPK_CHECK_ARG(last_ >= 0, "no collected batch");
    OPK_CHECK_ARG(frame >= 0 && frame < n_, "bad frame");
    const PoseModelInfo& m = pose_model(model_);
    const size_t area = (size_t)(kMaxPeaks + 1) * 3;
    const float* p = static_cast<const float*>(slots_[last_].hpeaks.ptr) + (size_t)frame * m.parts * area;
    for (int part = 0; part < m.parts; ++part) {
        const float* pp = p + part * area;
        const int count = (int)std::round(pp[0]);
        if (counts) counts[part] = count;
        if (!out) continue;
        for (int c = 0; c < count; ++c) {
            float* o = out + ((size_t)part * kMaxPeaks + c) * 3;
            o[0] = pp[3 + 3 * c] * scale_net_to_output_;
            o[1] = pp[3 + 3 * c + 1] * scale_net_to_output_;
            o[2] = pp[3 + 3 * c + 2];
        }
    }
}

float* PoseHip::peaks(int shape[4]) const
{
    OPK_CHECK_ARG(last_ >= 0, "no collected batch");
    shape[0] = n_; shape[1] = pose_model(model_).parts; shape[2] = kMaxPeaks + 1; shape[3] = 3;
    return static_cast<float*>(slots_[last_].peaks.ptr);
}

void PoseHip::forward(const float* frames, int n, int net_h, int net_w, int prod_w, int prod_h)
{
    OPK_CHECK_ARG(count_ == 0, "batches in flight: collect them first");
    submit(frames, n, net_h, net_w, prod_w, prod_h);
    collect();
}

void PoseHip::forward_net_output(const float* net_out, int n, int oh, int ow, int net_h,
                                 int net_w, int prod_w, int prod_h)
{
    OPK_CHECK_ARG(count_ == 0, "batches in flight: collect them first");
    submit_net_output(net_out, n, oh, ow, net_h, net_w, prod_w, prod_h);
    collect();
}

void PoseHip::need_frames() const
{
    if (any_attached() && !cur_raw_.ptr)
        throw Error(3, "face / hand extraction needs the frames: with an extractor attached only "
                       "submit_frames / forward_frames are accepted");
}

void PoseHip::attach_extractor(KeypointExtractor* ex)
{
    OPK_CHECK_ARG(ex != nullptr, "NULL extractor");
    OPK_CHECK_ARG(ex->context() == ctx_, "the extractor and the pose extractor must share one context");
    OPK_CHECK_ARG(ex->net() != net_, "the extractor's net must not be the pose net");
    const int kind = ex->kind();
    if (kind == KeypointExtractor::kFace) detect_faces(model_, nullptr, 0, 0, nullptr);
    else detect_hands(model_, nullptr, 0, 0, nullptr);
    if (count_ != 0) throw Error(3, "batches in flight: collect them before attaching");
    if (attached(kind))
        throw Error(3, std::string("a ") + (kind == KeypointExtractor::kFace ? "face" : "hand") +
                           " extractor is already attached: detach it first");
    part_[kind] = Part{};
    part_[kind].ex = ex;
    part_[kind].alive = ex->liveness();
    part_[kind].parts = ex->parts();
    parts_valid_ = false;
}

void PoseHip::detach_extractor(int kind)
{
    OPK_CHECK_ARG(kind == KeypointExtractor::kFace || kind == KeypointExtractor::kHand,
                  "kind: face (0) or hand (1)");
    if (count_ != 0) throw Error(3, "batches in flight: collect them before detaching");
    part_[kind] = Part{};
}

const Rect* PoseHip::part_rectangles(int kind, int f) const
{
    OPK_CHECK_ARG(kind == KeypointExtractor::kFace || kind == KeypointExtractor::kHand,
                  "kind: face (0) or hand (1)");
    if (!attached(kind)) throw Error(3, "no such extractor attached");
    if (!parts_valid_) throw Error(3, "no collected batch with face / hand results");
    OPK_CHECK_ARG(f >= 0 && f < n_, "bad frame");
    return part_[kind].rects.data() + (size_t)part_first_[f] * (kind == KeypointExtractor::kHand ? 2 : 1);
}

const float* PoseHip::part_keypoints(int kind, int f, int* first, int* total, int* parts) const
{
    (void)part_rectangles(kind, f);
    *first = part_first_[f];
    *total = part_first_[n_];
    *parts = part_[kind].parts;
    return part_[kind].kp.data();
}

void PoseHip::read_part_times(int kind, int* batches, int* crops, double* host_ms, double* wait_ms)
{
    OPK_CHECK_ARG(kind == KeypointExtractor::kFace || kind == KeypointExtractor::kHand,
                  "kind: face (0) or hand (1)");
    Part& p = part_[kind];
    if (!attached(kind)) throw Error(3, "no such extractor attached");
    if (batches) *batches = p.batches;
    if (crops) *crops = p.crops;
    if (host_ms) *host_ms = p.host_ms;
    if (wait_ms) *wait_ms = p.wait_ms;
    p.batches = p.crops = 0;
    p.host_ms = p.wait_ms = 0.;
}

void PoseHip::run_parts(const Slot& sl)
{
    parts_valid_ = false;
    if (!any_attached()) return;
    if (!sl.raw.ptr) throw Error(3, "face / hand extraction needs the frames of the collected batch");
    const int n = sl.n;
    const int parts = pose_model(model_).parts;
    part_first_.assign(n + 1, 0);
    for (int f = 0; f < n; ++f) part_first_[f + 1] = part_first_[f] + people_[f];
    const int total = part_first_[n];
    std::vector<int> frame_of(total);
    for (int f = 0; f < n; ++f)
        std::fill(frame_of.begin() + part_first_[f], frame_of.begin() + part_first_[f + 1], f);
    for (int kind = 0; kind < 2; ++kind) {
        Part& p = part_[kind];
        if (!attached(kind)) continue;
        const auto t0 = std::chrono::steady_clock::now();
        const int per = kind == KeypointExtractor::kHand ? 2 : 1;
        p.rects.assign((size_t)total * per, Rect{0.f, 0.f, 0.f, 0.f});
        for (int f = 0; f < n; ++f) {
            Rect* r = p.rects.data() + (size_t)part_first_[f] * per;
            if (kind == KeypointExtractor::kFace) detect_faces(model_, kp_[f].data(), people_[f], parts, r);
            else detect_hands(model_, kp_[f].data(), people_[f], parts, r);
        }
        p.kp.assign((size_t)per * total * p.ex->parts() * 3, 0.f);
        const double rect_ms =
            std::chrono::duration<double, std::milli>(std::chrono::steady_clock::now() - t0).count();
        p.ex->extract(sl.raw.ptr, sl.raw.n, sl.raw.w, sl.raw.h, sl.raw.step, p.rects.data(),
                      frame_of.data(), total, p.kp.data(), true);
        ++p.batches;
        p.crops += p.ex->crops();
        p.host_ms += rect_ms + p.ex->last_host_ms();
        p.wait_ms += p.ex->last_wait_ms();
    }
    parts_valid_ = true;
}

void PoseHip::submit(const float* frames, int n, int net_h, int net_w, int prod_w, int prod_h)
{
    need_frames();
    OPK_CHECK_ARG(net_ != nullptr, "no network: use forward_net_output (poseNetOutput path)");
    OPK_CHECK_ARG(count_ < 2, "two batches already in flight: collect first");
    ctx_->bind();
    next_output(n, net_h, net_w, true);
    live_net()->forward(frames, n, net_h, net_w);
    const NetOutput o{live_net()->output(), live_net()->out_h(), live_net()->out_w()};
    submit_outputs(&o, 1, n, net_h, net_w, prod_w, prod_h, true);
}

hipStream_t PoseHip::post_stream(bool own_net)
{
    if (!own_net || ctx_->device < 0 || dev_switch("POST_STREAM", 1) == 0) {
        wait_post(ctx_->stream);
        return ctx_->stream;
    }
    if (!post_) {
        OPK_HIP(hipStreamCreateWithFlags(&post_, hipStreamNonBlocking));
        OPK_HIP(hipEventCreateWithFlags(&nets_done_, hipEventDisableTiming));
        for (auto& e : post_done_) OPK_HIP(hipEventCreateWithFlags(&e, hipEventDisableTiming));
        ctx_->add_side_stream(post_);
    }
    OPK_HIP(hipEventRecord(nets_done_, ctx_->stream));
    OPK_HIP(hipStreamWaitEvent(post_, nets_done_, 0));
    return post_;
}

void PoseHip::wait_post(hipStream_t s)
{
    if (post_count_ > 0) OPK_HIP(hipStreamWaitEvent(s, post_done_[(post_count_ - 1) & 1], 0));
}

void PoseHip::next_output(int n, int h, int w, bool alternate)
{
    const bool alt = alternate && post_ != nullptr && dev_switch("NET_OUT_ALT", 1) != 0;
    (void)live_net()->select_output(n, h, w, alt);
}

void PoseHip::set_input(int net_w, int net_h, float dyn, int scale_number, double scale_gap)
{
    OPK_CHECK_ARG(net_w > 0 || net_h > 0,
                  "Only 1 of the dimensions of net input resolution can be <= 0.");
    OPK_CHECK_ARG(scale_number >= 1 && scale_number <= kMaxResizeSources, "1..8 scales");
    OPK_CHECK_ARG(1. - (scale_number - 1) * scale_gap >= 0. && scale_gap >= 0.,
                  "All scales must be in the range [0, 1], i.e., 0 <= 1-scale_number*scale_gap <= 1");
    in_net_w_ = net_w;
    in_net_h_ = net_h;
    dyn_ = dyn;
    scale_number_ = scale_number;
    scale_gap_ = scale_gap;
}

void PoseHip::submit_frames(const uint8_t* frames, int n, int w, int h, size_t step)
{
    OPK_CHECK_ARG(net_ != nullptr, "no network: raw frames need the net");
    OPK_CHECK_ARG(frames != nullptr && n > 0 && w > 0 && h > 0, "empty frames");
    OPK_CHECK_ARG(count_ < 2, "two batches already in flight: collect first");
    OPK_CHECK_ARG(model_ != 6, "BODY_19N (DenseNet normalisation) is not supported");
    double scales[kMaxResizeSources];
    scale_and_size(w, h, in_net_w_, in_net_h_, dyn_, scale_number_, scale_gap_, scales, input_hw_);
    const float* ptrs[kMaxResizeSources];
    int hw[2 * kMaxResizeSources];
    ctx_->bind();
    for (int i = 0; i < scale_number_; ++i) {
        const int nw = input_hw_[2 * i], nh = input_hw_[2 * i + 1];
        float* x = static_cast<float*>(inputs_[i].get((size_t)n * 3 * nh * nw * sizeof(float)));
        cvmat_to_input(ctx_, x, frames, n, w, h, step, scales[i], nw, nh, 1, ctx_->stream);
        ptrs[i] = x;
        hw[2 * i] = nh;
        hw[2 * i + 1] = nw;
    }
    inputs_n_ = n;
    for (int i = 0; i < scale_number_; ++i) map_ratios_[i] = (float)scales[i];
    have_ratios_ = true;
    cur_raw_ = RawFrames{frames, n, w, h, step};
    try {
        if (scale_number_ == 1)
            submit(ptrs[0], n, hw[0], hw[1], w, h);
        else
            submit_multi(ptrs, hw, scale_number_, n, w, h);
    } catch (...) {
        have_ratios_ = false;
        cur_raw_ = RawFrames{};
        throw;
    }
    have_ratios_ = false;
    cur_raw_ = RawFrames{};
}

void PoseHip::forward_frames(const uint8_t* frames, int n, int w, int h, size_t step)
{
    OPK_CHECK_ARG(count_ == 0, "batches in flight: collect them first");
    submit_frames(frames, n, w, h, step);
    collect();
}

const float* PoseHip::net_input(int i, int* w, int* h) const
{
    OPK_CHECK_ARG(i >= 0 && i < scale_number_ && inputs_n_ > 0, "no such scale");
    if (w) *w = input_hw_[2 * i];
    if (h) *h = input_hw_[2 * i + 1];
    return static_cast<const float*>(inputs_[i].ptr);
}

void PoseHip::submit_multi(const float* const* frames, const int* net_hw, int nscales, int n,
                           int prod_w, int prod_h)
{
    need_frames();
    OPK_CHECK_ARG(net_ != nullptr, "no network: multi-scale needs the net");
    OPK_CHECK_ARG(frames && net_hw && nscales >= 1 && nscales <= kMaxResizeSources,
                  "1..8 scales");
    OPK_CHECK_ARG(count_ < 2, "two batches already in flight: collect first");
    std::vector<NetOutput> outs(nscales);
    for (int i = 0; i < nscales; ++i) OPK_CHECK_ARG(frames[i] != nullptr, "NULL scale input");
    ctx_->bind();
    bool distinct = dev_switch("MULTISCALE_STREAMS", 1) != 0;
    for (int i = 0; i < nscales && distinct; ++i)
        for (int j = 0; j < i; ++j)
            distinct = distinct && !(net_hw[2 * i] == net_hw[2 * j] && net_hw[2 * i + 1] == net_hw[2 * j + 1]);
    for (int i = 0; i < nscales; ++i) next_output(n, net_hw[2 * i], net_hw[2 * i + 1], nscales == 1 || distinct);
    if (nscales == 1 || !distinct) {
        for (int i = 0; i < nscales; ++i) {
            live_net()->forward(frames[i], n, net_hw[2 * i], net_hw[2 * i + 1]);
            outs[i] = NetOutput{live_net()->output(), live_net()->out_h(), live_net()->out_w()};
        }
    } else {
        if (!fork_) {
            OPK_HIP(hipEventCreateWithFlags(&fork_, hipEventDisableTiming));
            for (int i = 0; i < kMaxResizeSources - 1; ++i) {
                OPK_HIP(hipStreamCreateWithFlags(&scale_streams_[i], hipStreamNonBlocking));
                OPK_HIP(hipEventCreateWithFlags(&join_[i], hipEventDisableTiming));
            }
        }
        for (int i = 0; i < nscales; ++i) live_net()->prepare(n, net_hw[2 * i], net_hw[2 * i + 1]);
        hipStream_t s = ctx_->stream;
        live_net()->time_begin(s);
        OPK_HIP(hipEventRecord(fork_, s));
        live_net()->forward_on(frames[0], n, net_hw[0], net_hw[1], s, false);
        outs[0] = NetOutput{live_net()->output(), live_net()->out_h(), live_net()->out_w()};
        for (int i = 1; i < nscales; ++i) {
            OPK_HIP(hipStreamWaitEvent(scale_streams_[i - 1], fork_, 0));
            live_net()->forward_on(frames[i], n, net_hw[2 * i], net_hw[2 * i + 1], scale_streams_[i - 1],
                             false);
            outs[i] = NetOutput{live_net()->output(), live_net()->out_h(), live_net()->out_w()};
            OPK_HIP(hipEventRecord(join_[i - 1], scale_streams_[i - 1]));
        }
        for (int i = 1; i < nscales; ++i) OPK_HIP(hipStreamWaitEvent(s, join_[i - 1], 0));
        live_net()->time_end(s);
    }
    submit_outputs(outs.data(), nscales, n, net_hw[0], net_hw[1], prod_w, prod_h, true);
}

void PoseHip::submit_net_output(const float* net_out, int n, int oh, int ow, int net_h,
                                int net_w, int prod_w, int prod_h)
{
    need_frames();
    const NetOutput o{net_out, oh, ow};
    submit_outputs(&o, 1, n, net_h, net_w, prod_w, prod_h, false);
}

void PoseHip::submit_outputs(const NetOutput* outs, int nscales, int n, int net_h, int net_w,
                             int prod_w, int prod_h, bool own_net)
{
    const PoseModelInfo& m = pose_model(model_);
    const int C = m.heat_channels();
    OPK_CHECK_ARG(n > 0 && nscales >= 1 && nscales <= kMaxResizeSources, "bad batch");
    for (int i = 0; i < nscales; ++i)
        OPK_CHECK_ARG(outs[i].ptr && outs[i].h > 0 && outs[i].w > 0, "empty net output");
    OPK_CHECK_ARG(count_ < 2, "two batches already in flight: collect first");
    ctx_->bind();
    Slot& sl = slots_[(head_ + count_) & 1];
    const hipStream_t s = post_stream(own_net);
    if (const int d = dev_switch("POST_DELAY_US", 0)) launch_delay(d, s);
    timer_.begin(s);
    if (overlay_) {
        const size_t out_elems = (size_t)n * C * outs[0].h * outs[0].w;
        launch_add_inplace(const_cast<float*>(outs[0].ptr), overlay_, out_elems, s);
    }

    const float dec = net_decrease_factor(model_);
    const float nf = upsampling_ > 0.f ? upsampling_ : dec;
    const int H = (int)std::round(((float)outs[0].h * nf - 1.f) * 1.f) + 1;
    const int W = (int)std::round(((float)outs[0].w * nf - 1.f) * 1.f) + 1;
    OPK_CHECK_ARG(H >= 1 && W >= 1, "upsampling ratio gives an empty heat map");
    HeatMap heat{};
    if (maps_ == kMapsCuda) {
        OPK_CHECK_ARG(nscales == 1 || have_ratios_,
                      "multi-scale CUDA map semantics needs scaleInputToNetInputs (raw-frame path)");
        const float* ptr[kMaxResizeSources];
        int hs[kMaxResizeSources], ws[kMaxResizeSources];
        for (int i = 0; i < nscales; ++i) {
            ptr[i] = outs[i].ptr;
            hs[i] = outs[i].h;
            ws[i] = outs[i].w;
        }
        heat = cuda_heat_map(ptr, hs, ws, nscales, C, H, W, have_ratios_ ? map_ratios_ : nullptr);
    } else {
        heat.channels = C;
        heat.h = H;
        heat.w = W;
        heat.nsrc = nscales;
        heat.inv_n = (float)(1. / (double)nscales);
        for (int i = 0; i < nscales; ++i) {
            const auto& t = ctx_->tables(outs[i].h, outs[i].w, H, W);
            heat.src[i] = ResizeSource{outs[i].ptr, outs[i].h, outs[i].w, t.yofs, t.ycoef, t.xofs,
                                       t.xcoef};
        }
    }

    const float ratio = upsampling_ <= 0.f ? 1.f : upsampling_ / dec;
    const int out_w = (int)(ratio * (float)net_w + 0.5f), out_h = (int)(ratio * (float)net_h + 0.5f);
    const double sp = resize_scale_factor(prod_w, prod_h, out_w, out_h);
    const int nw = (int)(sp * prod_w + 0.5f), nh = (int)(sp * prod_h + 0.5f);
    const float scale = (float)resize_scale_factor(nw, nh, prod_w, prod_h);

    const float nms_th = (float)props_[OPK_PROP_NMS_THRESHOLD];
    const float off = float(0.5 / double(scale));
    OPK_CHECK_ARG(!(nms_th < 0 || nms_th > 1.0), "threshold value invalid.");
    const int P1 = kMaxPeaks + 1;
    const size_t peak_floats = (size_t)m.parts * P1 * 3;
    float* peaks = static_cast<float*>(sl.peaks.get((size_t)n * peak_floats * 4));
    const size_t cand_bytes = nms_scratch_ints(n, m.parts) * sizeof(int);
    if (cand_bytes > cand_.bytes) {
        cand_.get(cand_bytes);
        OPK_HIP(hipMemsetAsync(cand_.ptr, 0, cand_bytes, s));
    }
    launch_nms(peaks, static_cast<int*>(cand_.ptr), heat, n, m.parts, P1, nms_th, off, off, s,
               maps_ == kMapsCuda);

    const float inter_th = (float)props_[OPK_PROP_INTER_THRESHOLD];
    const float inter_min = (float)props_[OPK_PROP_INTER_MIN_ABOVE_THRESHOLD];
    const double near = std::sqrt((double)(W * H)) / 150;
    const float reject = float(nms_th + 1e-6);
    const auto& pt = ctx_->pose_table(model_);
    const size_t rf = record_floats();
    float* rec = static_cast<float*>(sl.records.get((size_t)n * rf * 4));
    launch_paf_scores_compact(rec, (int)rf, heat, peaks, n, kMaxPeaks, pt, inter_th, inter_min,
                              reject, near, s);
    timer_.end(s);
    OPK_HIP(hipEventRecord(sl.done, s));
    if (post_ && s == post_) {
        const int k = post_count_ & 1;
        OPK_HIP(hipEventRecord(post_done_[k], post_));
        for (int i = 0; i < nscales; ++i) live_net()->note_reader(outs[i].ptr, post_done_[k]);
        ++post_count_;
    }
    sl.n = n;
    sl.H = H;
    sl.W = W;
    sl.scale = scale;
    sl.heat = heat;
    sl.raw = cur_raw_;
    ++count_;
}

int PoseHip::assembly_threads()
{
    int cpus = 0;
    cpu_set_t set;
    if (sched_getaffinity(0, sizeof set, &set) == 0) cpus = CPU_COUNT(&set);
    if (cpus <= 0) cpus = (int)std::max(1u, std::thread::hardware_concurrency());
    return std::max(1, std::min(kAssemblyThreads, cpus));
}

void PoseHip::read_collect_times(int* count, double* wait_ms, double* assembly_ms)
{
    if (count) *count = collect_count_;
    if (wait_ms) *wait_ms = collect_wait_ms_;
    if (assembly_ms) *assembly_ms = collect_assembly_ms_;
    collect_count_ = 0;
    collect_wait_ms_ = collect_assembly_ms_ = 0.;
}

int PoseHip::collect()
{
    OPK_CHECK_ARG(count_ > 0, "no batch in flight");
    ctx_->bind();
    const int si = head_;
    Slot& sl = slots_[si];
    const PoseModelInfo& m = pose_model(model_);
    const int n = sl.n;
    const int P1 = kMaxPeaks + 1;
    const size_t peak_floats = (size_t)m.parts * P1 * 3;
    const size_t rf = record_floats();
    const size_t K = std::min<size_t>(record_head_, rf);
    const int R = std::min(peak_rows_, P1);
    float* hp = static_cast<float*>(sl.hpeaks.get((size_t)n * peak_floats * 4));
    float* hr = static_cast<float*>(sl.hrecords.get((size_t)n * K * 4));
    OPK_HIP(hipStreamWaitEvent(copy_, sl.done, 0));
    OPK_HIP(hipMemcpy2DAsync(hp, (size_t)P1 * 12, sl.peaks.ptr, (size_t)P1 * 12, (size_t)R * 12,
                             (size_t)n * m.parts, hipMemcpyDeviceToHost, copy_));
    OPK_HIP(hipMemcpy2DAsync(hr, K * 4, sl.records.ptr, rf * 4, K * 4, n, hipMemcpyDeviceToHost,
                             copy_));
    auto tw0 = std::chrono::steady_clock::now();
    OPK_HIP(hipStreamSynchronize(copy_));
    double wait_ms = std::chrono::duration<double, std::milli>(std::chrono::steady_clock::now() - tw0).count();
// ... 97 lines not shown
```

openpose_amd/csrc/host/pose.h:

```cpp
#pragma once
#include <memory>
#include <vector>

#include "connector.h"
#include "context.h"
#include "extract.h"
#include "net.h"
#include "pool.h"

namespace opk {

class PoseHip {
public:
    PoseHip(Context* ctx, NetHip* net, bool maximize_positives, int pose_model = 0,
            int semantics = kConnectCpu);
    ~PoseHip();

    void set_property(int prop, double v);
    void set_map_semantics(int maps);
    int map_semantics() const { return maps_; }
    double property(int prop) const { return props_[prop]; }
    void set_overlay(const float* overlay) { overlay_ = overlay; }
    void set_upsampling_ratio(float ratio);
    float upsampling_ratio() const { return upsampling_; }

    void forward(const float* frames, int n, int net_h, int net_w, int prod_w, int prod_h);
    void forward_net_output(const float* net_out, int n, int out_h, int out_w, int net_h,
                            int net_w, int prod_w, int prod_h);
    void submit(const float* frames, int n, int net_h, int net_w, int prod_w, int prod_h);
    void submit_net_output(const float* net_out, int n, int out_h, int out_w, int net_h,
                           int net_w, int prod_w, int prod_h);
    void submit_multi(const float* const* frames, const int* net_hw, int nscales, int n,
                      int prod_w, int prod_h);
    void set_input(int net_w, int net_h, float dyn, int scale_number, double scale_gap);
    void submit_frames(const uint8_t* frames, int n, int w, int h, size_t step);
    void forward_frames(const uint8_t* frames, int n, int w, int h, size_t step);
    const float* net_input(int i, int* w, int* h) const;
    int collect();
    int pending() const { return count_; }

    int frames() const { return (int)people_.size(); }
    int num_people(int f) const { return people_.at(f); }
    const std::vector<float>& keypoints(int f) const { return kp_.at(f); }
    const std::vector<float>& scores(int f) const { return ks_.at(f); }
    float* heatmaps(int shape[4]);
    void heatmap_size(int shape[4]) const;
    const HeatMap& lazy_heat() const;
    float* peaks(int shape[4]) const;
    void heatmaps_copy(int types, int scale_mode, float* dst, int shape[4]);
    void heatmaps_copy_range(int types, int scale_mode, int frame0, int nframes, void* dst,
                             int dst_type, int shape[4]);
    void candidates(int frame, float* out, int* counts) const;
    float scale_net_to_output() const { return scale_net_to_output_; }
    void set_timing(bool on) { timer_.on = on; }
    void read_timing(int* count, double* total_ms) { timer_.read(count, total_ms); }
    void read_collect_times(int* count, double* wait_ms, double* assembly_ms);
    int assembly_workers() const { return pool_ ? pool_->workers() : assembly_threads(); }
    int model() const { return model_; }

    void attach_extractor(KeypointExtractor* ex);
    void detach_extractor(int kind);
    bool attached(int kind) const
    {
        return kind >= 0 && kind < 2 && part_[kind].ex != nullptr && !part_[kind].alive.expired();
    }
    const Rect* part_rectangles(int kind, int f) const;
    const float* part_keypoints(int kind, int f, int* first, int* total, int* parts) const;
    void read_part_times(int kind, int* batches, int* crops, double* host_ms, double* wait_ms);
    void* part_render_scratch(int kind, size_t bytes) { return part_dev_[kind & 1].get(bytes); }

    static constexpr int kMaxPeaks = kPoseMaxPeople;
    static constexpr int kRecordHead = 16384;
    static constexpr int kAssemblyThreads = 16;
    static int assembly_threads();

private:
    struct RawFrames {
        const uint8_t* ptr = nullptr;
        int n = 0, w = 0, h = 0;
        size_t step = 0;
    };
    struct Slot {
        DevBuf peaks, records;
        HostBuf hpeaks, hrecords;
        hipEvent_t done = nullptr;
        int n = 0, H = 0, W = 0;
        float scale = 1.f;
        HeatMap heat{};
        RawFrames raw{};
    };
    struct Part {
        KeypointExtractor* ex = nullptr;
        std::weak_ptr<void> alive;
        int parts = 0;
        std::vector<Rect> rects;
        std::vector<float> kp;
        int batches = 0, crops = 0;
        double host_ms = 0., wait_ms = 0.;
    };
    Part part_[2];
    DevBuf part_dev_[2];
    std::vector<int> part_first_;
    bool parts_valid_ = false;
    RawFrames cur_raw_{};
    bool any_attached() const { return attached(0) || attached(1); }
    void need_frames() const;
    void run_parts(const Slot& sl);
    struct NetOutput {
        const float* ptr;
        int h, w;
    };
    void submit_outputs(const NetOutput* outs, int nscales, int n, int net_h, int net_w,
                        int prod_w, int prod_h, bool own_net);
    size_t record_floats() const;

    Context* ctx_;
    NetHip* net_;
    std::weak_ptr<void> net_alive_;
    NetHip* live_net() const;
    int in_net_w_ = -1, in_net_h_ = 368, scale_number_ = 1;
    float dyn_ = 1.f;
    double scale_gap_ = 0.25;
    DevBuf inputs_[kMaxResizeSources];
    int input_hw_[2 * kMaxResizeSources] = {};
    int inputs_n_ = 0;
    bool maximize_positives_;
    int model_, semantics_;
    int maps_ = 0;
    float map_ratios_[kMaxResizeSources] = {};
    bool have_ratios_ = false;
    double props_[5];
    const float* overlay_ = nullptr;
    float upsampling_ = 0.f;
    hipStream_t copy_ = nullptr;
    hipStream_t post_ = nullptr;
    hipEvent_t nets_done_ = nullptr, post_done_[2] = {};
    int post_count_ = 0;
    hipStream_t post_stream(bool own_net);
    void wait_post(hipStream_t s);
    void next_output(int n, int h, int w, bool alternate);
    DevBuf cand_;
    hipStream_t scale_streams_[kMaxResizeSources - 1] = {};
    hipEvent_t fork_ = nullptr, join_[kMaxResizeSources - 1] = {};
    EventTimer timer_;

    Slot slots_[2];
    int head_ = 0, count_ = 0, last_ = -1;
    HostBuf overflow_;
    size_t record_head_ = kRecordHead;
    int peak_rows_ = kMaxPeaks + 1;
    std::unique_ptr<WorkerPool> pool_;
    int collect_count_ = 0;
    double collect_wait_ms_ = 0., collect_assembly_ms_ = 0.;
    std::vector<AssemblyScratch> scratch_;

    float scale_net_to_output_ = 1.f;
    int n_ = 0, hh_ = 0, hw_ = 0;
    bool heat_valid_ = false;
    DevBuf heat_, heat_sel_;
    std::vector<int> people_;
    std::vector<std::vector<float>> kp_, ks_;
};

double resize_scale_factor(int iw, int ih, int tw, int th);

}
```

openpose_amd/csrc/kernels/conv.h:

```cpp
#pragma once
#include <hip/hip_runtime.h>

#include <cstdint>

namespace opk {

constexpr int kConvMaxDst = 6;
constexpr int kConvBK = 64;

struct ConvArgs {
    const uint16_t* in;
    int in_cs, in_coff;
    int cin_pad;
    int ntaps;
    int tapoff[9];
    int ksteps;
    const uint16_t* w;
    const float* bias;
    const float* slope;
    int act;
    int frames, H, W;
    int M;
    int cout;
    int ndst;
    uint16_t* dst[kConvMaxDst];
    int dst_cs[kConvMaxDst], dst_coff[kConvMaxDst];
    float* out32;
    int out32_c, out32_coff;
    int sw, nstrips;
    float rcp[3];
    int wide;
    int prio;
    void* sink;
    int cus;
    int border;
    int actmax;
    int bufst;
    int pool;
    int nbx;
    int split;
    const uint16_t* in_lo;
    uint16_t* dst_lo[kConvMaxDst];
    float wscale;
    int small;
    int pbn;
};
#ifndef OPK_SPLIT_WLO_K
#define OPK_SPLIT_WLO_K 0
#endif

constexpr int kConvGuardTail = 1024;
constexpr size_t kConv3SinkBytes = (size_t)1024 * 1024 * 16;
constexpr int kConvPersistBM = 512, kConvPersistHR = 688;

constexpr long kConvMaxPositions = 1L << 24;
inline bool conv_positions_fit(long last) { return last < kConvMaxPositions; }
inline bool conv_bufst_fits(int frames, int Hp, int Wp, int cs)
{
    return ((long)frames * Hp * Wp + kConvGuardTail) * cs * 2 < (1L << 31) - 4096;
}
int conv3_pack_bn(int cout, int ks);

enum class Conv3Family { conv3, conv3p, conv3w, conv3w8, conv3s };

struct Conv3Query {
    int frames, H, W, cout, cin_pad, ntaps;
    int border;
    int ndst, dst_cs[kConvMaxDst], dst_coff[kConvMaxDst];
    bool out32;
    bool split;
    bool xhi;
    bool pool;
    bool small;
    bool sink;
    int cus;
};
Conv3Query conv3_query(const ConvArgs& a);

struct Conv3Plan {
    Conv3Family family;
    int bm, bn, hr, tapu, minb, ks, nw;
    int nb;
    int pbn;
    bool pool;
    bool split;
    bool xhi;
    int sw, nstrips, VW;
    long total;
    long grid;
    long workgroups;
    bool fits;
    float rcp[3];
    char name[64];
};
Conv3Plan conv3_plan(const Conv3Query& q, int only = -1);
int conv3_run_frames(const Conv3Query& q);
constexpr int kConv3sMaxPerCu = 4;
constexpr int kConv7sBigPerCus = 4;
ConvArgs conv3_planned_args(const ConvArgs& a, const Conv3Plan& p);

constexpr char kConvImageKernel[] = "conv_image_kernel";
constexpr char kConv1FusedKernel[] = "conv1_fused_kernel";
constexpr char kConvHeadKernel[] = "conv_head_kernel";

void launch_conv3(const ConvArgs& a, hipStream_t stream);
void launch_conv3w(const ConvArgs& a, const Conv3Plan& p, hipStream_t stream);
void launch_conv3w8(const ConvArgs& a, const Conv3Plan& p, hipStream_t stream);

struct HeadArgs {
    const uint16_t* in;
    int in_cs, in_coff, cin_pad;
    const uint16_t* w6;
    const float *b6, *s6;
    int act6;
    const uint16_t* w7;
    const float* b7;
    int n1, n2;
    int frames, H, W;
    int ndst;
    uint16_t* dst[kConvMaxDst];
    int dst_cs[kConvMaxDst], dst_coff[kConvMaxDst];
    float* out32;
    int out32_c, out32_coff;
    int cus;
    int actmax;
    int split;
    const uint16_t* in_lo;
    uint16_t* dst_lo[kConvMaxDst];
    float wscale6, wscale7;
};
bool conv_head_supported(int n1, int n2, int cin_pad);
void conv_head_pack_w7(uint16_t* dst, const uint16_t* w7 , int n1, int n2);
void launch_conv_head(const HeadArgs& a, hipStream_t stream);

void launch_conv_image(const ConvArgs& a, const float* image, hipStream_t stream);

struct Conv1FusedArgs {
    const float* img;
    int frames, H, W;
    const uint16_t* w1;
    const float *b1, *s1;
    int act1;
    const uint16_t* w2;
    const float *b2, *s2;
    int act2;
    uint16_t* out;
    int out_cs, out_coff, OH, OW;
    int actmax;
};
bool conv1_fused_supported(int H, int W, int cout1, int cout2);
void launch_conv1_fused(const Conv1FusedArgs& a, int workgroups, hipStream_t stream);

void launch_maxpool2_split(uint16_t* out, uint16_t* out_lo, const uint16_t* in, const uint16_t* in_lo,
                           int frames, int H, int W, int C, int OH, int OW, hipStream_t stream,
                           int border);
void launch_maxpool2(uint16_t* out, const uint16_t* in, int frames, int H, int W, int C, int OH,
                     int OW, hipStream_t stream, int border = 1);

}
```

openpose_amd/csrc/kernels/conv1_fused.hip:

```cpp
#include "conv.h"

#include <algorithm>

#include "../common.h"
#include "conv3_dev.h"

namespace opk {

namespace {

typedef _Float16 half8_t __attribute__((ext_vector_type(8)));
typedef _Float16 half2_t __attribute__((ext_vector_type(2)));
typedef float float4_t __attribute__((ext_vector_type(4)));
typedef float float2_t __attribute__((ext_vector_type(2)));

#ifndef OPK1_ABLATE
#define OPK1_ABLATE 0
#endif

constexpr int TR = 6, TC = 62, VW = 64;
constexpr int MT = TR * VW;
constexpr int HROWS = (TR + 2) * VW + 8;
constexpr int PR = TR + 4, PCW = TC + 4;
constexpr int PATCH = 3 * PR * PCW;
constexpr int PC = 67, PS = 683, PD = 2072;
static_assert(PC >= PCW && PS >= PR * PC && PC % 32 == 3 && PS % 32 == 11 && PD % 32 == 24, "patch layout");
constexpr int PATCH_LDS = PD + 3 * PS;
constexpr int NT = 512;
constexpr int PPL = (PATCH + NT - 1) / NT;
constexpr int TSTRIDE = 72;
constexpr int W2_PIECES = 18 * 64 * 4;
constexpr int HALO_PIECES = 2 * HROWS * 4;
constexpr int LDS_BYTES = (W2_PIECES + HALO_PIECES) * 16 + (PATCH_LDS * 4 + 15) / 16 * 16;
static_assert(MT * TSTRIDE * 2 <= HALO_PIECES * 16, "epilogue tile fits in the halo");
static_assert(LDS_BYTES <= 160 * 1024, "LDS budget");

__device__ __forceinline__ int swz64(int row, int piece) { return row * 4 + (piece ^ (((row >> 2) & 1) << 1)); }
__device__ __forceinline__ int swzh(int row, int piece) { return row * 4 + (piece ^ ((row >> 1) & 3)); }

__device__ __forceinline__ uint32_t hmax4(uint32_t a, uint32_t b, uint32_t c, uint32_t d)
{
    const half2_t m = __builtin_elementwise_max(
        __builtin_elementwise_max(__builtin_bit_cast(half2_t, a), __builtin_bit_cast(half2_t, b)),
        __builtin_elementwise_max(__builtin_bit_cast(half2_t, c), __builtin_bit_cast(half2_t, d)));
    return __builtin_bit_cast(uint32_t, m);
}

template <bool MX>
__global__ __launch_bounds__(NT, 1) void conv1_fused_kernel(const Conv1FusedArgs a)
{
    __shared__ uint4 lds[LDS_BYTES / 16];
    uint4* W2 = lds;
    uint4* HALO = lds + W2_PIECES;
    float* patch = reinterpret_cast<float*>(lds + W2_PIECES + HALO_PIECES);
    uint16_t* T = reinterpret_cast<uint16_t*>(HALO);

    const int tid = threadIdx.x, lane = tid & 63;
    const int wave = __builtin_amdgcn_readfirstlane(tid >> 6);
    const int r16 = lane & 15, q = lane >> 4;
    const int H = a.H, W = a.W;
    const int tiles_x = (W + TC - 1) / TC, tiles_y = (H + TR - 1) / TR;
    const int ntiles = a.frames * tiles_x * tiles_y;

    {
        const int lrow = lane >> 2, phys = lane & 3;
#pragma unroll
        for (int k = 0; k < W2_PIECES / NT; ++k) {
            const int inst = k * 8 + wave;
            const int row = inst * 16 + lrow;
            const int lp = phys ^ (((row >> 2) & 1) << 1);
            __builtin_amdgcn_global_load_lds((const void*)(a.w2 + (size_t)row * 32 + lp * 8),
                                             (__attribute__((address_space(3))) void*)(&W2[inst * 64]),
                                             16, 0, 0);
        }
    }
    half8_t w1f[4];
    float4_t b1[4], m1[4], b2[4], m2[4];
    const float neg1 = a.act1 == 1 ? 0.f : 1.f, neg2 = a.act2 == 1 ? 0.f : 1.f;
#pragma unroll
    for (int g = 0; g < 4; ++g) {
        w1f[g] = *reinterpret_cast<const half8_t*>(a.w1 + (size_t)(g * 16 + r16) * 64 + 8 * q);
        const int ch = g * 16 + 4 * q;
        b1[g] = *reinterpret_cast<const float4_t*>(a.b1 + ch);
        const float4_t s1 = *reinterpret_cast<const float4_t*>(a.s1 + ch);
        m1[g] = a.act1 == 2 ? s1 : float4_t{neg1, neg1, neg1, neg1};
        b2[g] = *reinterpret_cast<const float4_t*>(a.b2 + ch);
        const float4_t s2 = *reinterpret_cast<const float4_t*>(a.s2 + ch);
        m2[g] = a.act2 == 2 ? s2 : float4_t{neg2, neg2, neg2, neg2};
    }
    auto poff = [](int k) {
        const int t = k / 3, ci = k - 3 * (k / 3);
        return ci * PS + (t / 3) * PC + (t - 3 * (t / 3));
    };
    int off[8];
    unsigned kvalid = 0;
#pragma unroll
    for (int e = 0; e < 8; ++e) {
        const int k = 8 * q + e;
        off[e] = k < 27 ? poff(k) + (q & 1) * PD : poff(k - 8) + 16;
        kvalid |= (k < 27 ? 1u : 0u) << e;
    }

#define OPK1_ORIGIN(tile_, f_, y0_, x0_)                                                       \
    do {                                                                                      \
        const int tx_ = (tile_) % tiles_x;                                                    \
        const int rest_ = (tile_) / tiles_x;                                                  \
        y0_ = (rest_ % tiles_y) * TR;                                                         \
        f_ = rest_ / tiles_y;                                                                 \
        x0_ = tx_ * TC;                                                                       \
    } while (0)
    float pre[PPL];
#define OPK1_LOAD_PATCH(tile_)                                                                \
    do {                                                                                      \
        int f_, y0_, x0_;                                                                     \
        OPK1_ORIGIN(tile_, f_, y0_, x0_);                                                     \
        const float* src_ = a.img + (size_t)f_ * 3 * H * W;                                   \
        _Pragma("unroll") for (int k_ = 0; k_ < PPL; ++k_) {                                  \
            const int i_ = tid + k_ * NT;                                                     \
            float v_ = 0.f;                                                                   \
            if (i_ < PATCH && (tile_) < ntiles) {                                             \
                const int ci_ = i_ / (PR * PCW);                                              \
                const int rem_ = i_ - ci_ * (PR * PCW);                                       \
                const int r_ = rem_ / PCW, c_ = rem_ - (rem_ / PCW) * PCW;                    \
                const int y_ = y0_ - 2 + r_, x_ = x0_ - 2 + c_;                               \
                if (y_ >= 0 && y_ < H && x_ >= 0 && x_ < W)                                   \
                    v_ = src_[((size_t)ci_ * H + y_) * W + x_];                               \
            }                                                                                 \
            pre[k_] = v_;                                                                     \
        }                                                                                     \
    } while (0)

    int pool_dp, pool_cg;
    {
        const unsigned g1m = 0xF00F0FF0u;
        const int lo = lane & 31;
        const bool g1 = (g1m >> lo) & 1u;
        const unsigned same = g1 ? g1m : ~g1m;
        const int k = __popc(same & ((1u << lo) - 1u));
        pool_dp = (g1 ? 1 : 0) + 2 * (lane >> 5) + 4 * (k >> 3);
        pool_cg = k & 7;
    }

    int pli[PPL];
#pragma unroll
    for (int k = 0; k < PPL; ++k) {
        const int i = tid + k * NT;
        const int ci = i / (PR * PCW), rem = i - ci * (PR * PCW);
        const int r = rem / PCW, cc = rem - r * PCW;
        pli[k] = i < PATCH ? ci * PS + r * PC + cc : -1;
    }

    int tile = blockIdx.x;
    OPK1_LOAD_PATCH(tile);
    for (; tile < ntiles; tile += gridDim.x) {
        int f, y0, x0;
        OPK1_ORIGIN(tile, f, y0, x0);
        __syncthreads();
#pragma unroll
        for (int k = 0; k < PPL; ++k)
            if (pli[k] >= 0) {
                patch[pli[k]] = pre[k];
                patch[PD + pli[k]] = pre[k];
            }
        asm volatile("s_waitcnt vmcnt(0)" ::: "memory");
        __syncthreads();

        float xv[4][8];
#pragma unroll
        for (int gi = 0; gi < 4; ++gi) {
            const int mh = (wave * 4 + gi) * 16 + r16;
            const int base = (mh >> 6) * PC + (mh & 63);
#pragma unroll
            for (int e = 0; e < 8; ++e) xv[gi][e] = patch[off[e] + base];
        }
        float4_t c1[4][4];
#pragma unroll
        for (int gi = 0; gi < 4; ++gi) {
            half8_t xf;
#pragma unroll
            for (int e = 0; e < 8; ++e)
                xf[e] = OPK1_ABLATE == 1 ? (_Float16)0.f
                        : ((kvalid >> e) & 1u) ? (_Float16)xv[gi][e] : (_Float16)0.f;
#pragma unroll
            for (int g = 0; g < 4; ++g)
                c1[gi][g] = OPK1_ABLATE == 1 ? float4_t{(float)xf[0], 0.f, 0.f, 0.f}
                    : __builtin_amdgcn_mfma_f32_16x16x32_f16(w1f[g], xf, float4_t{0.f, 0.f, 0.f, 0.f},
                                                             0, 0, 0);
        }
#pragma unroll
        for (int gi = 0; gi < 4; ++gi) {
            const int mh = (wave * 4 + gi) * 16 + r16;
            const int hr = mh >> 6, hc = mh & 63;
            const int y = y0 - 1 + hr, x = x0 - 1 + hc;
            const bool in = y >= 0 && y < H && x >= 0 && x < W;
            uint32_t pk[4][2];
#pragma unroll
            for (int g = 0; g < 4; ++g) {
                const float4_t t = c1[gi][g] + b1[g];
                const float4_t a_ = conv3dev::act_pick4<MX>(t, t * m1[g]);
                const float4_t v = in ? a_ : float4_t{0.f, 0.f, 0.f, 0.f};
                pk[g][0] = __builtin_bit_cast(uint32_t, __builtin_convertvector(v.xy, half2_t));
                pk[g][1] = __builtin_bit_cast(uint32_t, __builtin_convertvector(v.zw, half2_t));
            }
#pragma unroll
            for (int c = 0; c < 2; ++c) {
                const auto sl = __builtin_amdgcn_permlane16_swap(pk[2 * c][0], pk[2 * c + 1][0], false, false);
                const auto sh = __builtin_amdgcn_permlane16_swap(pk[2 * c][1], pk[2 * c + 1][1], false, false);
                HALO[c * HROWS * 4 + swzh(mh, 2 * (q & 1) + (q >> 1))] = make_uint4(sl[0], sh[0], sl[1], sh[1]);
            }
        }
        __syncthreads();

        OPK1_LOAD_PATCH(tile + gridDim.x);
        float4_t acc[3][4];
#pragma unroll
        for (int i = 0; i < 3; ++i)
#pragma unroll
            for (int j = 0; j < 4; ++j) acc[i][j] = float4_t{0.f, 0.f, 0.f, 0.f};
        half8_t fa[2][3], fb[2][4];
#define OPK1_READ(buf_, st_)                                                                  \
    do {                                                                                      \
        const int c_ = (st_) / 9, tap_ = (st_) - 9 * ((st_) / 9);                             \
        const int ky_ = tap_ / 3, kx_ = tap_ - 3 * (tap_ / 3);                                \
        const uint4* As_ = HALO + c_ * HROWS * 4;                                             \
        const uint4* Bs_ = W2 + (c_ * 9 + tap_) * 256;                                        \
        _Pragma("unroll") for (int i_ = 0; i_ < 3; ++i_)                                      \
            fa[buf_][i_] = __builtin_bit_cast(                                                \
                half8_t, As_[swzh(wave * 48 + i_ * 16 + r16 + ky_ * VW + kx_, q)]);             \
        _Pragma("unroll") for (int j_ = 0; j_ < 4; ++j_)                                      \
            fb[buf_][j_] = __builtin_bit_cast(half8_t, Bs_[swz64(j_ * 16 + r16, q)]);           \
    } while (0)
        OPK1_READ(0, 0);
#pragma unroll
        for (int st = 0; st < 18; ++st) {
            const int cur = st & 1;
            if (st + 1 < 18) OPK1_READ(cur ^ 1, st + 1);
            __builtin_amdgcn_sched_barrier(0);
#pragma unroll
            for (int i = 0; i < 3; ++i)
#pragma unroll
                for (int j = 0; j < 4; ++j)
                    if (OPK1_ABLATE == 2)
                        asm volatile("; mfma skipped" : "+v"(acc[i][j]) : "v"(fb[cur][j]), "v"(fa[cur][i]));
                    else
                        acc[i][j] = __builtin_amdgcn_mfma_f32_16x16x32_f16(fb[cur][j], fa[cur][i],
                                                                           acc[i][j], 0, 0, 0);
            __builtin_amdgcn_sched_barrier(0);
        }
#undef OPK1_READ
        __syncthreads();

        if (OPK1_ABLATE == 3) {
#pragma unroll
            for (int i = 0; i < 3; ++i)
#pragma unroll
                for (int j = 0; j < 4; ++j) asm volatile("" :: "v"(acc[i][j]));
            continue;
        }
#pragma unroll
        for (int i = 0; i < 3; ++i) {
            const int m = wave * 48 + i * 16 + r16;
            uint32_t pk[4][2];
#pragma unroll
            for (int j = 0; j < 4; ++j) {
                const float4_t t = acc[i][j] + b2[j];
                const float4_t v = conv3dev::act_pick4<MX>(t, t * m2[j]);
                pk[j][0] = __builtin_bit_cast(uint32_t, __builtin_convertvector(v.xy, half2_t));
                pk[j][1] = __builtin_bit_cast(uint32_t, __builtin_convertvector(v.zw, half2_t));
            }
#pragma unroll
            for (int j = 0; j < 4; j += 2) {
                const auto sl = __builtin_amdgcn_permlane16_swap(pk[j][0], pk[j + 1][0], false, false);
                const auto sh = __builtin_amdgcn_permlane16_swap(pk[j][1], pk[j + 1][1], false, false);
                *reinterpret_cast<uint4*>(T + m * TSTRIDE + j * 16 + 16 * (q & 1) + 8 * (q >> 1)) =
                    make_uint4(sl[0], sh[0], sl[1], sh[1]);
            }
        }
        __syncthreads();

        for (int it = wave; it < (TR / 2) * 4; it += NT / 64) {
            const int slot = it * 8 + pool_dp;
            const int cg = pool_cg;
            const int pr = slot >> 5, pc = slot & 31;
            const int oy = y0 / 2 + pr, ox = x0 / 2 + pc;
            if (pc >= TC / 2 || 2 * oy + 1 >= H || 2 * ox + 1 >= W) continue;
            const int m0 = (2 * pr) * VW + 2 * pc;
            const uint16_t* s0 = T + m0 * TSTRIDE + cg * 8;
            uint4 v0 = *reinterpret_cast<const uint4*>(s0);
            const uint4 v1 = *reinterpret_cast<const uint4*>(s0 + TSTRIDE);
            const uint4 v2 = *reinterpret_cast<const uint4*>(s0 + VW * TSTRIDE);
            const uint4 v3 = *reinterpret_cast<const uint4*>(s0 + (VW + 1) * TSTRIDE);
            v0.x = hmax4(v0.x, v1.x, v2.x, v3.x);
            v0.y = hmax4(v0.y, v1.y, v2.y, v3.y);
            v0.z = hmax4(v0.z, v1.z, v2.z, v3.z);
            v0.w = hmax4(v0.w, v1.w, v2.w, v3.w);
            uint16_t* dst = a.out + (((size_t)f * (a.OH + 2) + oy + 1) * (a.OW + 2) + ox + 1) * a.out_cs +
                            a.out_coff + cg * 8;
            *reinterpret_cast<uint4*>(dst) = v0;
        }
    }
#undef OPK1_LOAD_PATCH
#undef OPK1_ORIGIN
}

}

bool conv1_fused_supported(int H, int W, int cout1, int cout2)
{
    return cout1 == 64 && cout2 == 64 && H % 2 == 0 && W % 2 == 0 && H >= 2 && W >= 2;
}

void launch_conv1_fused(const Conv1FusedArgs& a, int workgroups, hipStream_t stream)
{
    OPK_CHECK_ARG(a.img && a.w1 && a.w2 && a.out && a.b1 && a.b2 && a.s1 && a.s2, "NULL argument");
    OPK_CHECK_ARG(a.frames > 0 && conv1_fused_supported(a.H, a.W, 64, 64), "conv1 fusion: sizes");
    OPK_CHECK_ARG(a.OH == a.H / 2 && a.OW == a.W / 2, "conv1 fusion: pooled size");
    OPK_CHECK_ARG(a.out_cs % 8 == 0 && a.out_coff % 8 == 0 && a.out_coff + 64 <= a.out_cs,
                  "conv1 fusion: 16-byte aligned output slice");
    const long tiles = (long)a.frames * ((a.W + TC - 1) / TC) * ((a.H + TR - 1) / TR);
    OPK_CHECK_ARG(tiles < (1L << 31), "conv1 fusion: too many tiles");
    const int grid = (int)std::min<long>(tiles, workgroups > 0 ? workgroups : 256);
    note_launch("%s<%d>", kConv1FusedKernel, a.actmax ? 1 : 0);
    if (a.actmax) hipLaunchKernelGGL(conv1_fused_kernel<true>, dim3(grid), dim3(NT), 0, stream, a);
    else hipLaunchKernelGGL(conv1_fused_kernel<false>, dim3(grid), dim3(NT), 0, stream, a);
    OPK_LAUNCH_CHECK();
}

}
```

openpose_amd/csrc/kernels/input.hip:

```cpp
#include "kernels.h"
#include "warp_dev.h"
#include "../common.h"

namespace opk {

namespace {

template <int K>
__global__ __launch_bounds__(256) void cvmat_to_input_kernel(
    float* __restrict__ dst, const uint8_t* __restrict__ src, int sh, int sw, size_t src_step,
    size_t src_frame, int dh, int dw, const int2* __restrict__ xtab, const int2* __restrict__ ytab,
    const short* __restrict__ wtab, int normalize, const int* __restrict__ frame_of, int tab_stride)
{
    const int y = blockIdx.x % dh;
    const int f = blockIdx.x / dh;
    xtab += (size_t)f * tab_stride;
    ytab += (size_t)f * tab_stride;
    const int2 yt = ytab[y];
    const uint8_t* fsrc = src + (size_t)(frame_of ? frame_of[f] : f) * src_frame;
    const size_t plane = (size_t)dh * dw;
    float* out = dst + (size_t)f * 3 * plane + (size_t)y * dw;
    for (int x = threadIdx.x; x < dw; x += blockDim.x) {
        const int2 xt = xtab[x];
        int u[3];
        warp_pixel<K>(u, yt, xt, warp_weights<K>(wtab, yt.y, xt.y), sh, sw,
                      [&](int, int yy) { return fsrc + (size_t)yy * src_step; });
#pragma unroll
        for (int c = 0; c < 3; ++c) {
            float v = (float)u[c];
            if (normalize) v = v * (1.f / 256.f) - 0.5f;
            out[(size_t)c * plane + x] = v;
        }
    }
}

template <int K, bool A16>
__global__ __launch_bounds__(256) void cvmat_to_input_lds_kernel(
    float* __restrict__ dst, const uint8_t* __restrict__ src, int sh, int sw, size_t src_step,
    size_t src_frame, int dh, int dw, const int2* __restrict__ xtab, const int2* __restrict__ ytab,
    const short* __restrict__ wtab, int normalize, const int* __restrict__ frame_of, int tab_stride,
    int lds_row, int rows_at)
{
    extern __shared__ __attribute__((aligned(16))) uint8_t smem[];
    int2* xs = reinterpret_cast<int2*>(smem);
    short* ws = reinterpret_cast<short*>(smem + (size_t)dw * 8);
    uint8_t* rows = smem + rows_at;
    const int y = blockIdx.x % dh;
    const int f = blockIdx.x / dh;
    xtab += (size_t)f * tab_stride;
    ytab += (size_t)f * tab_stride;
    const int2 yt = ytab[y];
    const int x_a = xtab[0].x, x_b = xtab[dw - 1].x;
    for (int x = threadIdx.x; x < dw; x += blockDim.x) xs[x] = xtab[x];
    for (int i = threadIdx.x; i < 32 * K * K; i += blockDim.x) ws[i] = wtab[yt.y * 32 * K * K + i];
    const int lo = max(min(x_a, x_b), 0), hi = min(max(x_a, x_b) + K, sw);
    const uint8_t* fsrc = src + (size_t)(frame_of ? frame_of[f] : f) * src_frame;
    const int b0 = A16 ? (lo * 3) & ~15 : lo * 3;
    const int b1 = hi > lo ? hi * 3 : b0;
#pragma unroll
    for (int ky = 0; ky < K; ++ky) {
        const int yy = yt.x + ky;
        if (yy < 0 || yy >= sh) continue;
        uint8_t* l = rows + ky * lds_row;
        const uint8_t* row = fsrc + (size_t)yy * src_step;
        if (A16) {
            const int full = (b1 - b0) >> 4;
            const uint4* g = reinterpret_cast<const uint4*>(row + b0);
            uint4* d = reinterpret_cast<uint4*>(l);
            for (int i = threadIdx.x; i < full; i += blockDim.x) d[i] = g[i];
            for (int j = b0 + full * 16 + threadIdx.x; j < b1; j += blockDim.x) l[j - b0] = row[j];
        } else {
            for (int j = b0 + threadIdx.x; j < b1; j += blockDim.x) l[j - b0] = row[j];
        }
    }
    __syncthreads();
    const size_t plane = (size_t)dh * dw;
    float* out = dst + (size_t)f * 3 * plane + (size_t)y * dw;
    for (int x = threadIdx.x; x < dw; x += blockDim.x) {
        const int2 xt = xs[x];
        int u[3];
        warp_pixel<K>(u, yt, xt, warp_weights<K>(ws, 0, xt.y), sh, sw,
                      [&](int ky, int) { return rows + ky * lds_row - b0; });
#pragma unroll
        for (int c = 0; c < 3; ++c) {
            float v = (float)u[c];
            if (normalize) v = v * (1.f / 256.f) - 0.5f;
            out[(size_t)c * plane + x] = v;
        }
    }
}

}

void launch_cvmat_to_input(float* dst, const uint8_t* src, int n, int sh, int sw, size_t src_step,
                           int dh, int dw, const int* xtab, const int* ytab, const short* wtab,
                           int ksize, int normalize, hipStream_t stream, const int* frame_of,
                           int tab_stride)
{
    OPK_CHECK_ARG(n > 0 && sh > 0 && sw > 0 && dh > 0 && dw > 0, "empty frame");
    OPK_CHECK_ARG(src_step >= (size_t)sw * 3, "row step shorter than the row");
    OPK_CHECK_ARG(ksize == 2 || ksize == 4, "linear or cubic");
    OPK_CHECK_ARG((long)n * dh < (1L << 31), "too many rows");
    const dim3 grid((unsigned)(n * dh));
    const int threads = dw >= 256 ? 256 : (dw >= 128 ? 128 : 64);
    const auto* xt = reinterpret_cast<const int2*>(xtab);
    const auto* yt = reinterpret_cast<const int2*>(ytab);
    const size_t frame = src_step * sh;
    const int lds_row = ((sw * 3 + 32) + 15) & ~15;
    const size_t rows_at = ((size_t)dw * 8 + 64 * ksize * ksize + 15) & ~(size_t)15;
    const size_t lds = rows_at + (size_t)ksize * lds_row;
    if (lds <= 64 * 1024) {
        const bool a16 = ((uintptr_t)src % 16 == 0) && src_step % 16 == 0 && frame % 16 == 0;
#define OPK_WARP_LDS(K_, A_)                                                                   \
    hipLaunchKernelGGL((cvmat_to_input_lds_kernel<K_, A_>), grid, dim3(threads), lds, stream, dst, \
                       src, sh, sw, src_step, frame, dh, dw, xt, yt, wtab, normalize, frame_of,  \
                       tab_stride, lds_row, (int)rows_at)
        if (ksize == 2) {
            if (a16) OPK_WARP_LDS(2, true); else OPK_WARP_LDS(2, false);
        } else {
            if (a16) OPK_WARP_LDS(4, true); else OPK_WARP_LDS(4, false);
        }
#undef OPK_WARP_LDS
        OPK_LAUNCH_CHECK();
        return;
    }
    if (ksize == 2)
        hipLaunchKernelGGL(cvmat_to_input_kernel<2>, grid, dim3(threads), 0, stream, dst, src, sh,
                           sw, src_step, frame, dh, dw, xt, yt, wtab, normalize, frame_of,
                           tab_stride);
    else
        hipLaunchKernelGGL(cvmat_to_input_kernel<4>, grid, dim3(threads), 0, stream, dst, src, sh,
                           sw, src_step, frame, dh, dw, xt, yt, wtab, normalize, frame_of,
                           tab_stride);
    OPK_LAUNCH_CHECK();
}

}
```

openpose_amd/csrc/kernels/kernels.h:

```cpp
#pragma once
#include <hip/hip_runtime.h>

#include <cstdint>

namespace opk {

struct ResizeSource {
    const float* src;
    int sh, sw;
    const int* yofs;
    const float* ycoef;
    const int* xofs;
    const float* xcoef;
    float sx, sy;
};
constexpr int kMaxResizeSources = 8;
void launch_resize_merge(float* dst, const ResizeSource* srcs, int nsrc, int planes, int dh,
                         int dw, hipStream_t stream);

struct HeatMap {
    const float* heat;
    int channels, h, w;
    int nsrc;
    float inv_n;
    ResizeSource src[kMaxResizeSources];
    int cuda;
};
void launch_resize_merge_cuda(float* dst, const HeatMap& M, int planes, hipStream_t stream);
inline HeatMap heat_materialised(const float* heat, int channels, int h, int w)
{
    HeatMap m{};
    m.heat = heat;
    m.channels = channels;
    m.h = h;
    m.w = w;
    return m;
}

constexpr int kNmsCandidates = 1024;
size_t nms_scratch_ints(int frames, int parts);
void launch_nms(float* peaks, int* scratch, const HeatMap& heat, int frames, int parts,
                int max_peaks1, float threshold, float offx, float offy, hipStream_t stream,
                bool cuda = false);

struct PafPairTable {
    int npairs;
    int nparts;
    const int* pairs;
    const int* mapx;
    const int* mapy;
};
void launch_paf_scores(float* scores, const HeatMap& heat, const float* peaks, int frames,
                       int max_peaks, const PafPairTable& t, float inter_th,
                       float inter_min_above, float reject_score, double near_dist,
                       hipStream_t stream);
void launch_paf_scores_compact(float* records, int rec_floats, const HeatMap& heat,
                               const float* peaks, int frames, int max_peaks,
                               const PafPairTable& t, float inter_th, float inter_min_above,
                               float reject_score, double near_dist, hipStream_t stream);

void launch_cvmat_to_input(float* dst, const uint8_t* src, int n, int sh, int sw, size_t src_step,
                           int dh, int dw, const int* xtab, const int* ytab, const short* wtab,
                           int ksize, int normalize, hipStream_t stream,
                           const int* frame_of = nullptr, int tab_stride = 0);

void launch_heat_argmax(float* peaks, const HeatMap& heat, int crops, int parts, hipStream_t stream);
void launch_crop_heatmaps(float* dst, const HeatMap& heat, const int* slot_dev, int crops, int parts,
                          int scale_mode, hipStream_t stream);

constexpr int kRenderMaxPeople = 1024;
struct RenderKeypointsArgs {
    float* frame;
    int w, h;
    const float* kp;
    int people, parts;
    const unsigned* pairs;
    int npairs;
    const float* colors;
    int ncolors;
    const float* scales;
    int nscales;
    float radius, line_width, threshold, alpha;
    int blend, eye1, eye2;
    float* geom;
};
size_t render_geom_floats(int people, int parts, int npairs);
void launch_render_keypoints(const RenderKeypointsArgs& a, hipStream_t stream);
void launch_render_prep(const RenderKeypointsArgs& a, hipStream_t stream);

struct FrameWarp {
    const uint8_t* src;
    size_t src_step;
    int sw, sh;
    const int* xtab;
    const int* ytab;
    const short* wtab;
    int ksize;
};
void launch_cvmat_to_output(float* dst, int n, int w, int h, const FrameWarp& warp,
                            hipStream_t stream);
void launch_output_to_cvmat(uint8_t* dst, size_t dst_step, const float* src, int n, int w, int h,
                            int cast, hipStream_t stream);
struct RenderFramesLayer {
    const float* geom;
    const int* offsets;
    int total, parts, npairs;
    const float* colors;
    float alpha;
};
constexpr int kRenderMaxLayers = 3;
enum RenderHeatKind { kHeatNone = 0, kHeatPart, kHeatParts, kHeatPaf, kHeatPafs, kHeatDistance };
struct RenderFramesHeat {
    int kind;
    int channel;
    int count;
    float scale, alpha;
    const float* colors;
    int ncolors;
    int staged;
    HeatMap map;
};
constexpr int kRenderHeatWindow = 4096;
struct RenderFramesArgs {
    uint8_t* dst;
    size_t dst_step;
    int w, h, n;
    FrameWarp warp;
    int blend, cast, nlayers;
    int dst_aligned;
    RenderFramesLayer layer[kRenderMaxLayers];
    RenderFramesHeat heat;
};
void launch_render_frames(const RenderFramesArgs& a, hipStream_t stream);
bool render_heat_staged(int kind, float scale);
struct RenderHeatArgs {
    float* frame;
    int w, h;
    const float* heat;
    int hw, hh;
    float scale, alpha;
};
void launch_render_heat_map(const RenderHeatArgs& a, int part, bool abs_value, hipStream_t stream);
void launch_render_heat_maps(const RenderHeatArgs& a, int parts, const float* colors, int ncolors,
                             hipStream_t stream);
void launch_render_pafs(const RenderHeatArgs& a, int first, int count, hipStream_t stream);

void launch_mfma_peak(const void* operands, float* out, int blocks, int iters, hipStream_t stream);
void launch_hbm_read(const void* buf, size_t bytes, float* out, int blocks, hipStream_t stream);

void launch_add_inplace(float* dst, const float* src, size_t n, hipStream_t stream);
void launch_delay(int microseconds, hipStream_t stream);
void launch_f64_to_f32(float* dst, const double* src, size_t n, hipStream_t stream);
void launch_f32_to_f64(double* dst, const float* src, size_t n, hipStream_t stream);
void launch_heat_copy(float* dst, const float* heat, const int* sel_dev, int nsel, int frames,
                      int channels, size_t hw, int scale_mode, hipStream_t stream);

struct HeatSelection {
    int nsel;
    int dst0[3], src0[3], count[3], paf[3];
};
void launch_heat_copy_lazy(void* dst, bool u8, const HeatMap& M, const HeatSelection& sel,
                           int frame0, int nframes, int scale_mode, hipStream_t stream);

}
```

Before: 3814.

## Feed the fused first conv a u8 net image instead of float input

The resize/warp kernel can now write a pitched uint8 planar net image instead of normalized float32, and the fused conv1 layer reads that u8 image directly (img8), normalizing on load. This is on by default via NET_INPUT_U8 and cuts input write/read traffic roughly fourfold. A fallback converter kernel expands u8 to float when it is needed. The post-processing stream is also created with a priority, which can change how it competes with the network stream.

```diff
diff --git a/include/opk.h b/include/opk.h
--- a/include/opk.h
+++ b/include/opk.h
@@ -133,6 +133,10 @@
                        int scale_number, double scale_gap, double* scales, int* net_sizes);
 int opk_cvmat_to_input(opk_ctx* ctx, float* input_dev, const uint8_t* frames_dev, int n, int width,
                        int height, size_t step, double scale, int net_w, int net_h, int normalize);
+int opk_cvmat_to_input_u8(opk_ctx* ctx, uint8_t* image_dev, const uint8_t* frames_dev, int n,
+                          int width, int height, size_t step, double scale, int net_w, int net_h);
+int opk_u8_to_input(opk_ctx* ctx, float* input_dev, const uint8_t* image_dev, int n, int net_w,
+                    int net_h);
 
 int opk_dev_set(const char* key, int value, int reset);
 
@@ -148,6 +152,8 @@
 int opk_net_set_conv(opk_net* net, const char* name, const float* weights_host,
                      const float* bias_host, const float* slope_host);
 int opk_net_forward(opk_net* net, const float* input_dev, int n, int h, int w);
+int opk_net_forward_u8(opk_net* net, const uint8_t* image_dev, int n, int h, int w);
+int opk_net_takes_u8(opk_net* net, int h, int w);
 int opk_net_flops_per_frame(opk_net* net, int h, int w, double* flops);
 #define OPK_PRECISION_FP16 0
 #define OPK_PRECISION_SPLIT 1
diff --git a/openpose_amd/_lib.py b/openpose_amd/_lib.py
--- a/openpose_amd/_lib.py
+++ b/openpose_amd/_lib.py
@@ -58,6 +58,8 @@
     "opk_net_conv_info": (_i, [_p, _i, _c.c_char_p, _ip, _ip, _ip, _ip]),
     "opk_net_set_conv": (_i, [_p, _c.c_char_p, _p, _p, _p]),
     "opk_net_forward": (_i, [_p, _p, _i, _i, _i]),
+    "opk_net_forward_u8": (_i, [_p, _p, _i, _i, _i]),
+    "opk_net_takes_u8": (_i, [_p, _i, _i]),
     "opk_net_flops_per_frame": (_i, [_p, _i, _i, _c.POINTER(_d)]),
     "opk_net_output": (_i, [_p, _c.POINTER(_p), _ip]),
     "opk_net_blob": (_i, [_p, _c.c_char_p, _i, _i, _p, _ip]),
@@ -126,6 +128,8 @@
                                           _d, _f, _f, _i, _i, _i, _f, _f, _f, _f]),
     "opk_scale_and_size": (_i, [_i, _i, _i, _i, _f, _i, _d, _c.POINTER(_d), _ip]),
     "opk_cvmat_to_input": (_i, [_p, _p, _p, _i, _i, _i, _c.c_size_t, _d, _i, _i, _i]),
+    "opk_cvmat_to_input_u8": (_i, [_p, _p, _p, _i, _i, _i, _c.c_size_t, _d, _i, _i]),
+    "opk_u8_to_input": (_i, [_p, _p, _p, _i, _i, _i]),
     "opk_pose_set_input": (_i, [_p, _i, _i, _f, _i, _d]),
     "opk_pose_submit_frames": (_i, [_p, _p, _i, _i, _i, _c.c_size_t]),
     "opk_pose_forward_frames": (_i, [_p, _p, _i, _i, _i, _c.c_size_t]),
diff --git a/openpose_amd/api.py b/openpose_amd/api.py
--- a/openpose_amd/api.py
+++ b/openpose_amd/api.py
@@ -151,6 +151,18 @@
         check(self.L.opk_cvmat_to_input(self.h, _ptr(net_input), _ptr(frames), n, w, h, w * 3,
                                         float(scale), net_input.shape[3], net_input.shape[2],
                                         normalize))
+
+    def cvmat_to_input_u8(self, image, frames, scale, net_size):
+        n, h, w, c = frames.shape
+        assert c == 3 and frames.dtype == torch.uint8 and image.dtype == torch.uint8
+        assert tuple(image.shape) == (n, 3, net_size[1], (net_size[0] + 3) // 4 * 4)
+        check(self.L.opk_cvmat_to_input_u8(self.h, _ptr(image), _ptr(frames), n, w, h, w * 3,
+                                           float(scale), net_size[0], net_size[1]))
+
+    def u8_to_input(self, net_input, image):
+        n, c, h, w = net_input.shape
+        assert tuple(image.shape) == (n, 3, h, (w + 3) // 4 * 4) and image.dtype == torch.uint8
+        check(self.L.opk_u8_to_input(self.h, _ptr(net_input), _ptr(image), n, w, h))
 
     def nms(self, peaks, heat, threshold=NMS_THRESHOLD, offset=(0.0, 0.0), semantics=MAPS_CPU):
         check(self.L.opk_nms_semantics(self.h, _ptr(peaks), None, _ptr(heat), threshold,
@@ -486,6 +498,15 @@
         check(self.L.opk_net_forward(self.h, _ptr(x), n, h, w))
         return self.output()
 
+    def takes_u8(self, h, w):
+        return bool(self.L.opk_net_takes_u8(self.h, h, w))
+
+    def forward_u8(self, image, net_w):
+        n, c, h, pitch = image.shape
+        assert c == 3 and image.dtype == torch.uint8 and pitch == (net_w + 3) // 4 * 4
+        check(self.L.opk_net_forward_u8(self.h, _ptr(image), n, h, net_w))
+        return self.output()
+
     def load_caffemodel(self, path):
         n = ctypes.c_int()
         check(self.L.opk_net_load_caffemodel(self.h, path.encode(), ctypes.byref(n)))
diff --git a/openpose_amd/csrc/host/api_net.cpp b/openpose_amd/csrc/host/api_net.cpp
--- a/openpose_amd/csrc/host/api_net.cpp
+++ b/openpose_amd/csrc/host/api_net.cpp
@@ -102,6 +102,19 @@
         OPK_CHECK_ARG(net, "NULL net");
         net->net->forward(input, n, h, w);
     });
+}
+
+int opk_net_forward_u8(opk_net* net, const uint8_t* image, int n, int h, int w)
+{
+    return guarded_net([&] {
+        OPK_CHECK_ARG(net, "NULL net");
+        net->net->forward_on_u8(image, n, h, w, net->ctx->stream, true);
+    });
+}
+
+int opk_net_takes_u8(opk_net* net, int h, int w)
+{
+    return net && h > 0 && w > 0 && net->net->fused1_at(h, w) ? 1 : 0;
 }
 
 int opk_net_flops_per_frame(opk_net* net, int h, int w, double* flops)
@@ -497,6 +510,26 @@
                       "normalize: 0 (none) or 1 (VGG); DenseNet (2) is not supported");
         opk::cvmat_to_input(ctx, input_dev, frames_dev, n, width, height, step, scale, net_w, net_h,
                             normalize);
+    });
+}
+
+int opk_cvmat_to_input_u8(opk_ctx* ctx, uint8_t* image_dev, const uint8_t* frames_dev, int n,
+                          int width, int height, size_t step, double scale, int net_w, int net_h)
+{
+    return guarded_net([&] {
+        OPK_CHECK_ARG(ctx, "NULL context");
+        opk::cvmat_to_input_u8(ctx, image_dev, frames_dev, n, width, height, step, scale, net_w,
+                               net_h);
+    });
+}
+
+int opk_u8_to_input(opk_ctx* ctx, float* input_dev, const uint8_t* image_dev, int n, int net_w,
+                    int net_h)
+{
+    return guarded_net([&] {
+        OPK_CHECK_ARG(ctx, "NULL context");
+        ctx->bind();
+        opk::launch_u8_to_input(input_dev, image_dev, n, net_h, net_w, ctx->stream);
     });
 }
 
diff --git a/openpose_amd/csrc/host/input.cpp b/openpose_amd/csrc/host/input.cpp
--- a/openpose_amd/csrc/host/input.cpp
+++ b/openpose_amd/csrc/host/input.cpp
@@ -152,8 +152,10 @@
     return ref;
 }
 
-void cvmat_to_input(Context* ctx, float* dst, const uint8_t* src, int n, int sw, int sh,
-                    size_t step, double scale, int dw, int dh, int normalize, hipStream_t stream)
+namespace {
+template <class Launch>
+void warp_with_tables(Context* ctx, const void* dst, const uint8_t* src, int n, int sw, int sh,
+                      double scale, int dw, int dh, Launch launch)
 {
     OPK_CHECK_ARG(dst && src, "NULL buffer");
     OPK_CHECK_ARG(n > 0 && sw > 0 && sh > 0 && dw > 0 && dh > 0, "empty frame or net input");
@@ -162,8 +164,32 @@
     const bool cubic = scale > 1.;
     const short* w = ctx->warp_weight_table(cubic);
     const auto& ax = ctx->warp_axis_tables(scale, dw, dh);
-    launch_cvmat_to_input(dst, src, n, sh, sw, step ? step : (size_t)sw * 3, dh, dw, ax.x, ax.y, w,
-                          cubic ? 4 : 2, normalize, stream ? stream : ctx->stream);
+    launch(ax.x, ax.y, w, cubic ? 4 : 2);
+}
 }
 
+void cvmat_to_input(Context* ctx, float* dst, const uint8_t* src, int n, int sw, int sh,
+                    size_t step, double scale, int dw, int dh, int normalize, hipStream_t stream)
+{
+    warp_with_tables(ctx, dst, src, n, sw, sh, scale, dw, dh,
+                     [&](const int* x, const int* y, const short* w, int k) {
+                         launch_cvmat_to_input(dst, src, n, sh, sw, step ? step : (size_t)sw * 3, dh,
+                                               dw, x, y, w, k, normalize,
+                                               stream ? stream : ctx->stream);
+                     });
 }
+
+void cvmat_to_input_u8(Context* ctx, uint8_t* dst, const uint8_t* src, int n, int sw, int sh,
+                       size_t step, double scale, int dw, int dh, hipStream_t stream)
+{
+    warp_with_tables(ctx, dst, src, n, sw, sh, scale, dw, dh,
+                     [&](const int* x, const int* y, const short* w, int k) {
+                         launch_cvmat_to_input_u8(dst, src, n, sh, sw,
+                                                  step ? step : (size_t)sw * 3, dh, dw, x, y, w, k,
+                                                  stream ? stream : ctx->stream);
+                     });
+}
+
+size_t net_image_bytes(int n, int dw, int dh) { return (size_t)n * 3 * dh * net_image_pitch(dw); }
+
+}
diff --git a/openpose_amd/csrc/host/input.h b/openpose_amd/csrc/host/input.h
--- a/openpose_amd/csrc/host/input.h
+++ b/openpose_amd/csrc/host/input.h
@@ -15,5 +15,8 @@
 
 void cvmat_to_input(Context* ctx, float* dst, const uint8_t* src, int n, int sw, int sh,
                     size_t step, double scale, int dw, int dh, int normalize, hipStream_t stream = nullptr);
+void cvmat_to_input_u8(Context* ctx, uint8_t* dst, const uint8_t* src, int n, int sw, int sh,
+                       size_t step, double scale, int dw, int dh, hipStream_t stream = nullptr);
+size_t net_image_bytes(int n, int dw, int dh);
 
 }
diff --git a/openpose_amd/csrc/host/net.cpp b/openpose_amd/csrc/host/net.cpp
--- a/openpose_amd/csrc/host/net.cpp
+++ b/openpose_amd/csrc/host/net.cpp
@@ -773,15 +773,29 @@
 
 void NetHip::forward_on(const float* input, int n, int h, int w, hipStream_t st, bool timed)
 {
-    OPK_CHECK_ARG(input && n > 0 && h > 0 && w > 0, "empty input");
+    OPK_CHECK_ARG(input != nullptr, "empty input");
+    forward_any(input, nullptr, n, h, w, st, timed);
+}
+
+void NetHip::forward_on_u8(const uint8_t* image, int n, int h, int w, hipStream_t st, bool timed)
+{
+    OPK_CHECK_ARG(image != nullptr, "empty input");
+    forward_any(nullptr, image, n, h, w, st, timed);
+}
+
+void NetHip::forward_any(const float* input, const uint8_t* input8, int n, int h, int w,
+                         hipStream_t st, bool timed)
+{
+    OPK_CHECK_ARG(n > 0 && h > 0 && w > 0, "empty input");
     OPK_CHECK_ARG(ready(), "weights not loaded for every convolution");
     ctx_->bind();
     ShapePlan& S = *shape_plan(n, h, w, st);
+    OPK_CHECK_ARG(!input8 || S.fused1, "the u8 net image needs conv1_fused as the first layer");
     cur_ = &S;
     for (const auto& r : readers_)
         if (r.first == S.out()) OPK_HIP(hipStreamWaitEvent(st, r.second, 0));
     if (timed) timer_.begin(st);
-    forward_launches(S, input, n, h, w, st);
+    forward_launches(S, input, input8, n, h, w, st);
     if (timed) timer_.end(st);
 }
 
@@ -851,18 +865,20 @@
             }
 }
 
-void NetHip::forward_launches(ShapePlan& S, const float* input, int n, int h, int w, hipStream_t st)
+void NetHip::forward_launches(ShapePlan& S, const float* input, const uint8_t* input8, int n, int h,
+                              int w, hipStream_t st)
 {
     const bool logging = dev_switch("LAUNCH_LOG", 0) != 0;
     if (logging) {
-        log_.lines.clear();
+        log_.lines = std::move(log_head_);
         attach_launch_log(&log_);
     }
+    log_head_.clear();
     struct Detach {
         bool on;
         ~Detach() { if (on) attach_launch_log(nullptr); }
     } detach{logging};
-    forward_steps(S, input, n, h, w, st);
+    forward_steps(S, input, input8, n, h, w, st);
 }
 
 static void launch_conv3_frames(const ConvArgs& a, hipStream_t st)
@@ -895,7 +911,8 @@
     }
 }
 
-void NetHip::forward_steps(ShapePlan& S, const float* input, int n, int h, int w, hipStream_t st)
+void NetHip::forward_steps(ShapePlan& S, const float* input, const uint8_t* input8, int n, int h,
+                           int w, hipStream_t st)
 {
     LaunchLog* log = launch_log();
     float* const out32 = S.out();
@@ -909,6 +926,7 @@
         const PoolPlan& p = pools_[fuse1_.p];
         Conv1FusedArgs fa{};
         fa.img = input;
+        fa.img8 = input8;
         fa.frames = n;
         fa.H = h;
         fa.W = w;
diff --git a/openpose_amd/csrc/host/net.h b/openpose_amd/csrc/host/net.h
--- a/openpose_amd/csrc/host/net.h
+++ b/openpose_amd/csrc/host/net.h
@@ -36,6 +36,9 @@
     void forward(const float* input, int n, int h, int w);
     void forward_on(const float* input, int n, int h, int w, hipStream_t stream, bool timed);
     void prepare(int n, int h, int w);
+    bool fused1_at(int h, int w) const;
+    void forward_on_u8(const uint8_t* image, int n, int h, int w, hipStream_t stream, bool timed);
+    void note_input_launches(std::vector<std::string> lines) { log_head_ = std::move(lines); }
     void time_begin(hipStream_t s) { timer_.begin(s); }
     void time_end(hipStream_t s) { timer_.end(s); }
     float* output() const { return cur_ ? cur_->out() : nullptr; }
@@ -82,7 +85,6 @@
         int precision = kPrecisionFp16;
         std::vector<float> hw, hb, hs;
     };
-    bool fused1_at(int h, int w) const;
     void read_planes(const std::string& name, int f0, int nf, float* hi, float* lo, float* sum,
                      int shape[4], int* has_lo) const;
     void pack(ConvPlan& c);
@@ -117,8 +119,12 @@
     };
 
     void plan(const std::vector<LayerDesc>& layers);
-    void forward_launches(ShapePlan& S, const float* input, int n, int h, int w, hipStream_t st);
-    void forward_steps(ShapePlan& S, const float* input, int n, int h, int w, hipStream_t st);
+    void forward_any(const float* input, const uint8_t* input8, int n, int h, int w, hipStream_t st,
+                     bool timed);
+    void forward_launches(ShapePlan& S, const float* input, const uint8_t* input8, int n, int h,
+                          int w, hipStream_t st);
+    void forward_steps(ShapePlan& S, const float* input, const uint8_t* input8, int n, int h, int w,
+                       hipStream_t st);
     ShapePlan* shape_plan(int n, int h, int w, hipStream_t zero_stream = nullptr);
 
     Context* ctx_;
@@ -143,6 +149,7 @@
     struct BlobLoc { int buf = -1, coff = 0, ch = 0, level = 0; bool out32 = false; };
     std::map<std::string, BlobLoc> blob_loc_;
     LaunchLog log_;
+    std::vector<std::string> log_head_;
 
     std::vector<std::unique_ptr<ShapePlan>> shapes_;
     ShapePlan* cur_ = nullptr;
diff --git a/openpose_amd/csrc/host/pose.cpp b/openpose_amd/csrc/host/pose.cpp
--- a/openpose_amd/csrc/host/pose.cpp
+++ b/openpose_amd/csrc/host/pose.cpp
@@ -357,7 +357,7 @@
     OPK_CHECK_ARG(count_ < 2, "two batches already in flight: collect first");
     ctx_->bind();
     next_output(n, net_h, net_w, true);
-    live_net()->forward(frames, n, net_h, net_w);
+    run_net(0, frames, n, net_h, net_w, ctx_->stream, true);
     const NetOutput o{live_net()->output(), live_net()->out_h(), live_net()->out_w()};
     submit_outputs(&o, 1, n, net_h, net_w, prod_w, prod_h, true);
 }
@@ -369,7 +369,10 @@
         return ctx_->stream;
     }
     if (!post_) {
-        OPK_HIP(hipStreamCreateWithFlags(&post_, hipStreamNonBlocking));
+        int least = 0, greatest = 0;
+        OPK_HIP(hipDeviceGetStreamPriorityRange(&least, &greatest));
+        const int prio = dev_switch("POST_PRIORITY", 1) != 0 ? least : 0;
+        OPK_HIP(hipStreamCreateWithPriority(&post_, hipStreamNonBlocking, prio));
         OPK_HIP(hipEventCreateWithFlags(&nets_done_, hipEventDisableTiming));
         for (auto& e : post_done_) OPK_HIP(hipEventCreateWithFlags(&e, hipEventDisableTiming));
         ctx_->add_side_stream(post_);
@@ -415,15 +418,39 @@
     const float* ptrs[kMaxResizeSources];
     int hw[2 * kMaxResizeSources];
     ctx_->bind();
+    const int u8_mode = dev_switch("NET_INPUT_U8", 1);
+    const bool logging = dev_switch("LAUNCH_LOG", 0) != 0;
     for (int i = 0; i < scale_number_; ++i) {
         const int nw = input_hw_[2 * i], nh = input_hw_[2 * i + 1];
-        float* x = static_cast<float*>(inputs_[i].get((size_t)n * 3 * nh * nw * sizeof(float)));
-        cvmat_to_input(ctx_, x, frames, n, w, h, step, scales[i], nw, nh, 1, ctx_->stream);
-        ptrs[i] = x;
+        LaunchLog wl;
+        wl.layer = "input";
+        if (logging) attach_launch_log(&wl);
+        struct Detach {
+            bool on;
+            ~Detach() { if (on) attach_launch_log(nullptr); }
+        } detach{logging};
+        input_is_u8_[i] = u8_mode != 0 && (u8_mode != 2 || i == 0) && live_net()->fused1_at(nh, nw);
+        input_expanded_[i] = false;
+        if (input_is_u8_[i]) {
+            uint8_t* x = static_cast<uint8_t*>(inputs_u8_[i].get(net_image_bytes(n, nw, nh)));
+            cvmat_to_input_u8(ctx_, x, frames, n, w, h, step, scales[i], nw, nh, ctx_->stream);
+            cur_u8_[i] = x;
+            ptrs[i] = nullptr;
+        } else {
+            float* x = static_cast<float*>(inputs_[i].get((size_t)n * 3 * nh * nw * sizeof(float)));
+            cvmat_to_input(ctx_, x, frames, n, w, h, step, scales[i], nw, nh, 1, ctx_->stream);
+            cur_u8_[i] = nullptr;
+            ptrs[i] = x;
+        }
+        warp_log_[i] = std::move(wl.lines);
         hw[2 * i] = nh;
         hw[2 * i + 1] = nw;
     }
     inputs_n_ = n;
+    struct ClearU8 {
+        PoseHip* p;
+        ~ClearU8() { for (auto& u : p->cur_u8_) u = nullptr; }
+    } clear_u8{this};
     for (int i = 0; i < scale_number_; ++i) map_ratios_[i] = (float)scales[i];
     have_ratios_ = true;
     cur_raw_ = RawFrames{frames, n, w, h, step};
@@ -448,12 +475,29 @@
     collect();
 }
 
-const float* PoseHip::net_input(int i, int* w, int* h) const
+const float* PoseHip::net_input(int i, int* w, int* h)
 {
     OPK_CHECK_ARG(i >= 0 && i < scale_number_ && inputs_n_ > 0, "no such scale");
-    if (w) *w = input_hw_[2 * i];
-    if (h) *h = input_hw_[2 * i + 1];
+    const int nw = input_hw_[2 * i], nh = input_hw_[2 * i + 1];
+    if (w) *w = nw;
+    if (h) *h = nh;
+    if (input_is_u8_[i] && !input_expanded_[i]) {
+        ctx_->bind();
+        float* x = static_cast<float*>(inputs_[i].get((size_t)inputs_n_ * 3 * nh * nw * sizeof(float)));
+        launch_u8_to_input(x, static_cast<const uint8_t*>(inputs_u8_[i].ptr), inputs_n_, nh, nw,
+                           ctx_->stream);
+        input_expanded_[i] = true;
+    }
     return static_cast<const float*>(inputs_[i].ptr);
+}
+
+void PoseHip::run_net(int i, const float* frames, int n, int h, int w, hipStream_t st, bool timed)
+{
+    NetHip* net = live_net();
+    if (!warp_log_[i].empty()) net->note_input_launches(std::move(warp_log_[i]));
+    warp_log_[i].clear();
+    if (cur_u8_[i]) net->forward_on_u8(cur_u8_[i], n, h, w, st, timed);
+    else net->forward_on(frames, n, h, w, st, timed);
 }
 
 void PoseHip::submit_multi(const float* const* frames, const int* net_hw, int nscales, int n,
@@ -465,7 +509,7 @@
                   "1..8 scales");
     OPK_CHECK_ARG(count_ < 2, "two batches already in flight: collect first");
     std::vector<NetOutput> outs(nscales);
-    for (int i = 0; i < nscales; ++i) OPK_CHECK_ARG(frames[i] != nullptr, "NULL scale input");
+    for (int i = 0; i < nscales; ++i) OPK_CHECK_ARG(frames[i] != nullptr || cur_u8_[i], "NULL scale input");
     ctx_->bind();
     bool distinct = dev_switch("MULTISCALE_STREAMS", 1) != 0;
     for (int i = 0; i < nscales && distinct; ++i)
@@ -474,7 +518,7 @@
     for (int i = 0; i < nscales; ++i) next_output(n, net_hw[2 * i], net_hw[2 * i + 1], nscales == 1 || distinct);
     if (nscales == 1 || !distinct) {
         for (int i = 0; i < nscales; ++i) {
-            live_net()->forward(frames[i], n, net_hw[2 * i], net_hw[2 * i + 1]);
+            run_net(i, frames[i], n, net_hw[2 * i], net_hw[2 * i + 1], ctx_->stream, true);
             outs[i] = NetOutput{live_net()->output(), live_net()->out_h(), live_net()->out_w()};
         }
     } else {
@@ -489,12 +533,11 @@
         hipStream_t s = ctx_->stream;
         live_net()->time_begin(s);
         OPK_HIP(hipEventRecord(fork_, s));
-        live_net()->forward_on(frames[0], n, net_hw[0], net_hw[1], s, false);
+        run_net(0, frames[0], n, net_hw[0], net_hw[1], s, false);
         outs[0] = NetOutput{live_net()->output(), live_net()->out_h(), live_net()->out_w()};
         for (int i = 1; i < nscales; ++i) {
             OPK_HIP(hipStreamWaitEvent(scale_streams_[i - 1], fork_, 0));
-            live_net()->forward_on(frames[i], n, net_hw[2 * i], net_hw[2 * i + 1], scale_streams_[i - 1],
-                             false);
+            run_net(i, frames[i], n, net_hw[2 * i], net_hw[2 * i + 1], scale_streams_[i - 1], false);
             outs[i] = NetOutput{live_net()->output(), live_net()->out_h(), live_net()->out_w()};
             OPK_HIP(hipEventRecord(join_[i - 1], scale_streams_[i - 1]));
         }
diff --git a/openpose_amd/csrc/host/pose.h b/openpose_amd/csrc/host/pose.h
--- a/openpose_amd/csrc/host/pose.h
+++ b/openpose_amd/csrc/host/pose.h
@@ -35,7 +35,7 @@
     void set_input(int net_w, int net_h, float dyn, int scale_number, double scale_gap);
     void submit_frames(const uint8_t* frames, int n, int w, int h, size_t step);
     void forward_frames(const uint8_t* frames, int n, int w, int h, size_t step);
-    const float* net_input(int i, int* w, int* h) const;
+    const float* net_input(int i, int* w, int* h);
     int collect();
     int pending() const { return count_; }
 
@@ -124,6 +124,12 @@
     DevBuf inputs_[kMaxResizeSources];
     int input_hw_[2 * kMaxResizeSources] = {};
     int inputs_n_ = 0;
+    DevBuf inputs_u8_[kMaxResizeSources];
+    bool input_is_u8_[kMaxResizeSources] = {};
+    bool input_expanded_[kMaxResizeSources] = {};
+    const uint8_t* cur_u8_[kMaxResizeSources] = {};
+    std::vector<std::string> warp_log_[kMaxResizeSources];
+    void run_net(int i, const float* frames, int n, int h, int w, hipStream_t st, bool timed);
     bool maximize_positives_;
     int model_, semantics_;
     int maps_ = 0;
diff --git a/openpose_amd/csrc/kernels/conv.h b/openpose_amd/csrc/kernels/conv.h
--- a/openpose_amd/csrc/kernels/conv.h
+++ b/openpose_amd/csrc/kernels/conv.h
@@ -137,6 +137,7 @@
 
 struct Conv1FusedArgs {
     const float* img;
+    const uint8_t* img8;
     int frames, H, W;
     const uint16_t* w1;
     const float *b1, *s1;
diff --git a/openpose_amd/csrc/kernels/conv1_fused.hip b/openpose_amd/csrc/kernels/conv1_fused.hip
--- a/openpose_amd/csrc/kernels/conv1_fused.hip
+++ b/openpose_amd/csrc/kernels/conv1_fused.hip
@@ -1,6 +1,7 @@
 #include "conv.h"
 
 #include <algorithm>
+#include <type_traits>
 
 #include "../common.h"
 #include "conv3_dev.h"
@@ -46,7 +47,7 @@
     return __builtin_bit_cast(uint32_t, m);
 }
 
-template <bool MX>
+template <bool MX, bool U8>
 __global__ __launch_bounds__(NT, 1) void conv1_fused_kernel(const Conv1FusedArgs a)
 {
     __shared__ uint4 lds[LDS_BYTES / 16];
@@ -109,22 +110,30 @@
         f_ = rest_ / tiles_y;                                                                 \
         x0_ = tx_ * TC;                                                                       \
     } while (0)
-    float pre[PPL];
+    using pre_t = typename std::conditional<U8, uint32_t, float>::type;
+    using img_t = typename std::conditional<U8, uint8_t, float>::type;
+    const img_t* const img = [&] { if constexpr (U8) return a.img8; else return a.img; }();
+    const int WP = U8 ? (W + 3) & ~3 : W;
+    auto patch_value = [](pre_t v) {
+        if constexpr (U8) return (float)v * (1.f / 256.f) - 0.5f;
+        else return v;
+    };
+    pre_t pre[PPL];
 #define OPK1_LOAD_PATCH(tile_)                                                                \
     do {                                                                                      \
         int f_, y0_, x0_;                                                                     \
         OPK1_ORIGIN(tile_, f_, y0_, x0_);                                                     \
-        const float* src_ = a.img + (size_t)f_ * 3 * H * W;                                   \
+        const img_t* src_ = img + (size_t)f_ * 3 * H * WP;                                    \
         _Pragma("unroll") for (int k_ = 0; k_ < PPL; ++k_) {                                  \
             const int i_ = tid + k_ * NT;                                                     \
-            float v_ = 0.f;                                                                   \
+            pre_t v_ = U8 ? (pre_t)128 : (pre_t)0;                                            \
             if (i_ < PATCH && (tile_) < ntiles) {                                             \
                 const int ci_ = i_ / (PR * PCW);                                              \
                 const int rem_ = i_ - ci_ * (PR * PCW);                                       \
                 const int r_ = rem_ / PCW, c_ = rem_ - (rem_ / PCW) * PCW;                    \
                 const int y_ = y0_ - 2 + r_, x_ = x0_ - 2 + c_;                               \
                 if (y_ >= 0 && y_ < H && x_ >= 0 && x_ < W)                                   \
-                    v_ = src_[((size_t)ci_ * H + y_) * W + x_];                               \
+                    v_ = src_[((size_t)ci_ * H + y_) * WP + x_];                              \
             }                                                                                 \
             pre[k_] = v_;                                                                     \
         }                                                                                     \
@@ -159,8 +168,9 @@
 #pragma unroll
         for (int k = 0; k < PPL; ++k)
             if (pli[k] >= 0) {
-                patch[pli[k]] = pre[k];
-                patch[PD + pli[k]] = pre[k];
+                const float v = patch_value(pre[k]);
+                patch[pli[k]] = v;
+                patch[PD + pli[k]] = v;
             }
         asm volatile("s_waitcnt vmcnt(0)" ::: "memory");
         __syncthreads();
@@ -312,7 +322,8 @@
 
 void launch_conv1_fused(const Conv1FusedArgs& a, int workgroups, hipStream_t stream)
 {
-    OPK_CHECK_ARG(a.img && a.w1 && a.w2 && a.out && a.b1 && a.b2 && a.s1 && a.s2, "NULL argument");
+    OPK_CHECK_ARG((a.img != nullptr) != (a.img8 != nullptr), "one of the fp32 and the u8 image");
+    OPK_CHECK_ARG(a.w1 && a.w2 && a.out && a.b1 && a.b2 && a.s1 && a.s2, "NULL argument");
     OPK_CHECK_ARG(a.frames > 0 && conv1_fused_supported(a.H, a.W, 64, 64), "conv1 fusion: sizes");
     OPK_CHECK_ARG(a.OH == a.H / 2 && a.OW == a.W / 2, "conv1 fusion: pooled size");
     OPK_CHECK_ARG(a.out_cs % 8 == 0 && a.out_coff % 8 == 0 && a.out_coff + 64 <= a.out_cs,
@@ -320,9 +331,15 @@
     const long tiles = (long)a.frames * ((a.W + TC - 1) / TC) * ((a.H + TR - 1) / TR);
     OPK_CHECK_ARG(tiles < (1L << 31), "conv1 fusion: too many tiles");
     const int grid = (int)std::min<long>(tiles, workgroups > 0 ? workgroups : 256);
-    note_launch("%s<%d>", kConv1FusedKernel, a.actmax ? 1 : 0);
-    if (a.actmax) hipLaunchKernelGGL(conv1_fused_kernel<true>, dim3(grid), dim3(NT), 0, stream, a);
-    else hipLaunchKernelGGL(conv1_fused_kernel<false>, dim3(grid), dim3(NT), 0, stream, a);
+    note_launch(a.img8 ? "%s<%d,u8>" : "%s<%d>", kConv1FusedKernel, a.actmax ? 1 : 0);
+#define OPK1_LAUNCH(MX_, U8_) \
+    hipLaunchKernelGGL((conv1_fused_kernel<MX_, U8_>), dim3(grid), dim3(NT), 0, stream, a)
+    if (a.img8) {
+        if (a.actmax) OPK1_LAUNCH(true, true); else OPK1_LAUNCH(false, true);
+    } else {
+        if (a.actmax) OPK1_LAUNCH(true, false); else OPK1_LAUNCH(false, false);
+    }
+#undef OPK1_LAUNCH
     OPK_LAUNCH_CHECK();
 }
 
diff --git a/openpose_amd/csrc/kernels/input.hip b/openpose_amd/csrc/kernels/input.hip
--- a/openpose_amd/csrc/kernels/input.hip
+++ b/openpose_amd/csrc/kernels/input.hip
@@ -2,13 +2,18 @@
 #include "warp_dev.h"
 #include "../common.h"
 
+#include <algorithm>
+#include <type_traits>
+
 namespace opk {
 
 namespace {
 
-template <int K>
+template <class OUT> constexpr bool kU8 = std::is_same<OUT, uint8_t>::value;
+
+template <int K, class OUT>
 __global__ __launch_bounds__(256) void cvmat_to_input_kernel(
-    float* __restrict__ dst, const uint8_t* __restrict__ src, int sh, int sw, size_t src_step,
+    OUT* __restrict__ dst, const uint8_t* __restrict__ src, int sh, int sw, size_t src_step,
     size_t src_frame, int dh, int dw, const int2* __restrict__ xtab, const int2* __restrict__ ytab,
     const short* __restrict__ wtab, int normalize, const int* __restrict__ frame_of, int tab_stride)
 {
@@ -18,25 +23,46 @@
     ytab += (size_t)f * tab_stride;
     const int2 yt = ytab[y];
     const uint8_t* fsrc = src + (size_t)(frame_of ? frame_of[f] : f) * src_frame;
-    const size_t plane = (size_t)dh * dw;
-    float* out = dst + (size_t)f * 3 * plane + (size_t)y * dw;
-    for (int x = threadIdx.x; x < dw; x += blockDim.x) {
-        const int2 xt = xtab[x];
-        int u[3];
-        warp_pixel<K>(u, yt, xt, warp_weights<K>(wtab, yt.y, xt.y), sh, sw,
-                      [&](int, int yy) { return fsrc + (size_t)yy * src_step; });
-#pragma unroll
-        for (int c = 0; c < 3; ++c) {
-            float v = (float)u[c];
-            if (normalize) v = v * (1.f / 256.f) - 0.5f;
-            out[(size_t)c * plane + x] = v;
-        }
-    }
-}
-
-template <int K, bool A16>
+    if constexpr (kU8<OUT>) {
+        const int dp = (dw + 3) & ~3;
+        const size_t plane = (size_t)dh * dp;
+        uint8_t* out = dst + (size_t)f * 3 * plane + (size_t)y * dp;
+        for (int x0 = threadIdx.x * 4; x0 < dw; x0 += blockDim.x * 4) {
+            uint32_t pk[3] = {0u, 0u, 0u};
+#pragma unroll
+            for (int j = 0; j < 4; ++j) {
+                if (x0 + j >= dw) break;
+                const int2 xt = xtab[x0 + j];
+                int u[3];
+                warp_pixel<K>(u, yt, xt, warp_weights<K>(wtab, yt.y, xt.y), sh, sw,
+                              [&](int, int yy) { return fsrc + (size_t)yy * src_step; });
+#pragma unroll
+                for (int c = 0; c < 3; ++c) pk[c] |= (uint32_t)u[c] << (8 * j);
+            }
+#pragma unroll
+            for (int c = 0; c < 3; ++c) *reinterpret_cast<uint32_t*>(out + (size_t)c * plane + x0) = pk[c];
+        }
+    } else {
+        const size_t plane = (size_t)dh * dw;
+        float* out = dst + (size_t)f * 3 * plane + (size_t)y * dw;
+        for (int x = threadIdx.x; x < dw; x += blockDim.x) {
+            const int2 xt = xtab[x];
+            int u[3];
+            warp_pixel<K>(u, yt, xt, warp_weights<K>(wtab, yt.y, xt.y), sh, sw,
+                          [&](int, int yy) { return fsrc + (size_t)yy * src_step; });
+#pragma unroll
+            for (int c = 0; c < 3; ++c) {
+                float v = (float)u[c];
+                if (normalize) v = v * (1.f / 256.f) - 0.5f;
+                out[(size_t)c * plane + x] = v;
+            }
+        }
+    }
+}
+
+template <int K, bool A16, class OUT>
 __global__ __launch_bounds__(256) void cvmat_to_input_lds_kernel(
-    float* __restrict__ dst, const uint8_t* __restrict__ src, int sh, int sw, size_t src_step,
+    OUT* __restrict__ dst, const uint8_t* __restrict__ src, int sh, int sw, size_t src_step,
     size_t src_frame, int dh, int dw, const int2* __restrict__ xtab, const int2* __restrict__ ytab,
     const short* __restrict__ wtab, int normalize, const int* __restrict__ frame_of, int tab_stride,
     int lds_row, int rows_at)
@@ -74,33 +100,79 @@
         }
     }
     __syncthreads();
-    const size_t plane = (size_t)dh * dw;
-    float* out = dst + (size_t)f * 3 * plane + (size_t)y * dw;
-    for (int x = threadIdx.x; x < dw; x += blockDim.x) {
-        const int2 xt = xs[x];
-        int u[3];
-        warp_pixel<K>(u, yt, xt, warp_weights<K>(ws, 0, xt.y), sh, sw,
-                      [&](int ky, int) { return rows + ky * lds_row - b0; });
-#pragma unroll
-        for (int c = 0; c < 3; ++c) {
-            float v = (float)u[c];
-            if (normalize) v = v * (1.f / 256.f) - 0.5f;
-            out[(size_t)c * plane + x] = v;
-        }
-    }
-}
-
-}
-
-void launch_cvmat_to_input(float* dst, const uint8_t* src, int n, int sh, int sw, size_t src_step,
-                           int dh, int dw, const int* xtab, const int* ytab, const short* wtab,
-                           int ksize, int normalize, hipStream_t stream, const int* frame_of,
-                           int tab_stride)
+    if constexpr (kU8<OUT>) {
+        const int dp = (dw + 3) & ~3;
+        uint8_t* ob = rows + K * lds_row;
+        for (int x = threadIdx.x; x < dp; x += blockDim.x) {
+            int u[3] = {0, 0, 0};
+            if (x < dw) {
+                const int2 xt = xs[x];
+                warp_pixel<K>(u, yt, xt, warp_weights<K>(ws, 0, xt.y), sh, sw,
+                              [&](int ky, int) { return rows + ky * lds_row - b0; });
+            }
+#pragma unroll
+            for (int c = 0; c < 3; ++c) ob[c * dp + x] = (uint8_t)u[c];
+        }
+        __syncthreads();
+        const size_t plane4 = (size_t)dh * dp / 4;
+        const int rw = dp >> 2;
+        uint32_t* out = reinterpret_cast<uint32_t*>(dst) + (size_t)f * 3 * plane4 + (size_t)y * rw;
+        const uint32_t* ow = reinterpret_cast<const uint32_t*>(ob);
+        for (int i = threadIdx.x; i < 3 * rw; i += blockDim.x) {
+            const int c = i / rw;
+            out[(size_t)c * plane4 + (i - c * rw)] = ow[i];
+        }
+    } else {
+        const size_t plane = (size_t)dh * dw;
+        float* out = dst + (size_t)f * 3 * plane + (size_t)y * dw;
+        for (int x = threadIdx.x; x < dw; x += blockDim.x) {
+            const int2 xt = xs[x];
+            int u[3];
+            warp_pixel<K>(u, yt, xt, warp_weights<K>(ws, 0, xt.y), sh, sw,
+                          [&](int ky, int) { return rows + ky * lds_row - b0; });
+#pragma unroll
+            for (int c = 0; c < 3; ++c) {
+                float v = (float)u[c];
+                if (normalize) v = v * (1.f / 256.f) - 0.5f;
+                out[(size_t)c * plane + x] = v;
+            }
+        }
+    }
+}
+
+__global__ __launch_bounds__(256) void u8_to_input_kernel(float* __restrict__ dst,
+                                                          const uint8_t* __restrict__ src,
+                                                          long rows, int dw, int pitch)
+{
+    const int rw = pitch >> 2;
+    const long total = rows * rw;
+    for (long i = (long)blockIdx.x * blockDim.x + threadIdx.x; i < total;
+         i += (long)gridDim.x * blockDim.x) {
+        const long r = i / rw;
+        const int x0 = (int)(i - r * rw) * 4;
+        const uint32_t w = reinterpret_cast<const uint32_t*>(src)[i];
+        float* o = dst + r * dw + x0;
+#pragma unroll
+        for (int j = 0; j < 4; ++j)
+            if (x0 + j < dw) o[j] = (float)((w >> (8 * j)) & 255u) * (1.f / 256.f) - 0.5f;
+    }
+}
+
+}
+
+namespace {
+
+template <class OUT>
+void launch_warp(OUT* dst, const uint8_t* src, int n, int sh, int sw, size_t src_step, int dh,
+                 int dw, const int* xtab, const int* ytab, const short* wtab, int ksize,
+                 int normalize, hipStream_t stream, const int* frame_of, int tab_stride)
 {
     OPK_CHECK_ARG(n > 0 && sh > 0 && sw > 0 && dh > 0 && dw > 0, "empty frame");
     OPK_CHECK_ARG(src_step >= (size_t)sw * 3, "row step shorter than the row");
     OPK_CHECK_ARG(ksize == 2 || ksize == 4, "linear or cubic");
     OPK_CHECK_ARG((long)n * dh < (1L << 31), "too many rows");
+    constexpr bool U8 = kU8<OUT>;
+    const char* ot = U8 ? "u8" : "f32";
     const dim3 grid((unsigned)(n * dh));
     const int threads = dw >= 256 ? 256 : (dw >= 128 ? 128 : 64);
     const auto* xt = reinterpret_cast<const int2*>(xtab);
@@ -108,13 +180,14 @@
     const size_t frame = src_step * sh;
     const int lds_row = ((sw * 3 + 32) + 15) & ~15;
     const size_t rows_at = ((size_t)dw * 8 + 64 * ksize * ksize + 15) & ~(size_t)15;
-    const size_t lds = rows_at + (size_t)ksize * lds_row;
+    const size_t lds = rows_at + (size_t)ksize * lds_row + (U8 ? 3 * (size_t)net_image_pitch(dw) : 0);
     if (lds <= 64 * 1024) {
         const bool a16 = ((uintptr_t)src % 16 == 0) && src_step % 16 == 0 && frame % 16 == 0;
+        note_launch("cvmat_to_input_lds_kernel<%d,%d,%s>", ksize, (int)a16, ot);
 #define OPK_WARP_LDS(K_, A_)                                                                   \
-    hipLaunchKernelGGL((cvmat_to_input_lds_kernel<K_, A_>), grid, dim3(threads), lds, stream, dst, \
-                       src, sh, sw, src_step, frame, dh, dw, xt, yt, wtab, normalize, frame_of,  \
-                       tab_stride, lds_row, (int)rows_at)
+    hipLaunchKernelGGL((cvmat_to_input_lds_kernel<K_, A_, OUT>), grid, dim3(threads), lds, stream, \
+                       dst, src, sh, sw, src_step, frame, dh, dw, xt, yt, wtab, normalize,        \
+                       frame_of, tab_stride, lds_row, (int)rows_at)
         if (ksize == 2) {
             if (a16) OPK_WARP_LDS(2, true); else OPK_WARP_LDS(2, false);
         } else {
@@ -124,15 +197,47 @@
         OPK_LAUNCH_CHECK();
         return;
     }
+    note_launch("cvmat_to_input_kernel<%d,%s>", ksize, ot);
     if (ksize == 2)
-        hipLaunchKernelGGL(cvmat_to_input_kernel<2>, grid, dim3(threads), 0, stream, dst, src, sh,
-                           sw, src_step, frame, dh, dw, xt, yt, wtab, normalize, frame_of,
+        hipLaunchKernelGGL((cvmat_to_input_kernel<2, OUT>), grid, dim3(threads), 0, stream, dst, src,
+                           sh, sw, src_step, frame, dh, dw, xt, yt, wtab, normalize, frame_of,
                            tab_stride);
     else
-        hipLaunchKernelGGL(cvmat_to_input_kernel<4>, grid, dim3(threads), 0, stream, dst, src, sh,
-                           sw, src_step, frame, dh, dw, xt, yt, wtab, normalize, frame_of,
+        hipLaunchKernelGGL((cvmat_to_input_kernel<4, OUT>), grid, dim3(threads), 0, stream, dst, src,
+                           sh, sw, src_step, frame, dh, dw, xt, yt, wtab, normalize, frame_of,
                            tab_stride);
     OPK_LAUNCH_CHECK();
 }
 
 }
+
+void launch_cvmat_to_input(float* dst, const uint8_t* src, int n, int sh, int sw, size_t src_step,
+                           int dh, int dw, const int* xtab, const int* ytab, const short* wtab,
+                           int ksize, int normalize, hipStream_t stream, const int* frame_of,
+                           int tab_stride)
+{
+    launch_warp(dst, src, n, sh, sw, src_step, dh, dw, xtab, ytab, wtab, ksize, normalize, stream,
+                frame_of, tab_stride);
+}
+
+void launch_cvmat_to_input_u8(uint8_t* dst, const uint8_t* src, int n, int sh, int sw,
+                              size_t src_step, int dh, int dw, const int* xtab, const int* ytab,
+                              const short* wtab, int ksize, hipStream_t stream)
+{
+    OPK_CHECK_ARG((uintptr_t)dst % 4 == 0, "u8 net image: 4-byte aligned");
+    launch_warp(dst, src, n, sh, sw, src_step, dh, dw, xtab, ytab, wtab, ksize, 0, stream, nullptr, 0);
+}
+
+void launch_u8_to_input(float* dst, const uint8_t* src, int n, int dh, int dw, hipStream_t stream)
+{
+    OPK_CHECK_ARG(dst && src && n > 0 && dh > 0 && dw > 0, "empty net image");
+    OPK_CHECK_ARG((uintptr_t)src % 4 == 0, "u8 net image: 4-byte aligned");
+    const int pitch = net_image_pitch(dw);
+    const long rows = (long)n * 3 * dh, words = rows * (pitch / 4);
+    const int blocks = (int)std::min<long>((words + 255) / 256, 256 * 16);
+    hipLaunchKernelGGL(u8_to_input_kernel, dim3(blocks), dim3(256), 0, stream, dst, src, rows, dw,
+                       pitch);
+    OPK_LAUNCH_CHECK();
+}
+
+}
diff --git a/openpose_amd/csrc/kernels/kernels.h b/openpose_amd/csrc/kernels/kernels.h
--- a/openpose_amd/csrc/kernels/kernels.h
+++ b/openpose_amd/csrc/kernels/kernels.h
@@ -63,6 +63,11 @@
                            int dh, int dw, const int* xtab, const int* ytab, const short* wtab,
                            int ksize, int normalize, hipStream_t stream,
                            const int* frame_of = nullptr, int tab_stride = 0);
+inline int net_image_pitch(int dw) { return (dw + 3) & ~3; }
+void launch_cvmat_to_input_u8(uint8_t* dst, const uint8_t* src, int n, int sh, int sw,
+                              size_t src_step, int dh, int dw, const int* xtab, const int* ytab,
+                              const short* wtab, int ksize, hipStream_t stream);
+void launch_u8_to_input(float* dst, const uint8_t* src, int n, int dh, int dw, hipStream_t stream);
 
 void launch_heat_argmax(float* peaks, const HeatMap& heat, int crops, int parts, hipStream_t stream);
 void launch_crop_heatmaps(float* dst, const HeatMap& heat, const int* slot_dev, int crops, int parts,
```

Result: no change. 3812, median of 2 (-0.1%).
